# zhuduowang/Change3D

Hardware: AMD Instinct MI355X
Metric: train images/sec (256x256 pairs, X3D-L BCD) (higher is better)
Workload: dtype bf16

## Files before the change

change3d_amd/csrc/dw_bwd_fused.hip:

```cpp
#include "pw_common.h"
#include "dw_common.h"
#include "bn_fin.h"
#include "launch_hints.h"
#include "../../include/change3d_hip.h"
#include <cstdlib>
#include <type_traits>

#ifdef C3D_PW_CLOCK
constexpr int FCLK_WAVES = 16384;
__device__ unsigned long long c3d_fb_clk[FCLK_WAVES][10];
#define FCLK_DECL unsigned long long fclk_[10] = {0, 0, 0, 0, 0, 0, 0, 0, 0, 0}; unsigned long long fclk_last_ = __builtin_amdgcn_s_memtime();
#define FCLK(i) { const unsigned long long t_ = __builtin_amdgcn_s_memtime(); fclk_[i] += t_ - fclk_last_; fclk_last_ = t_; }
#define FCLK_FLUSH if ((threadIdx.x & 63) == 0) { const int w_ = (blockIdx.x * 8 + (threadIdx.x >> 6)) % FCLK_WAVES; for (int i_ = 0; i_ < 9; ++i_) c3d_fb_clk[w_][i_] += fclk_[i_]; c3d_fb_clk[w_][9] += 1ull; }
#else
#define FCLK_DECL
#define FCLK(i)
#define FCLK_FLUSH
#endif

namespace {

#ifndef C3D_FB_ROWS
#define C3D_FB_ROWS 8
#endif
constexpr int FB_TH = C3D_FB_ROWS, FB_TW = 8, FB_DH = FB_TH + 2, FB_DW = FB_TW + 2, FB_NTHR = FB_TH * FB_TW * 8;
#if C3D_FB_ROWS == 8
#define FB_KATTR __launch_bounds__(FB_NTHR)
#else
#define FB_KATTR __launch_bounds__(FB_NTHR) __attribute__((amdgpu_waves_per_eu(2, 2)))
#endif

template <typename T> struct Raw8;
template <> struct Raw8<bf16_t> {
  typedef uint4 type;
  static __device__ __forceinline__ type load(const bf16_t* p) { return *reinterpret_cast<const uint4*>(p); }
  static __device__ __forceinline__ void cvt(const type& v, float (&f)[8]) {
    f[0] = __uint_as_float(v.x << 16); f[1] = __uint_as_float(v.x & 0xffff0000u);
    f[2] = __uint_as_float(v.y << 16); f[3] = __uint_as_float(v.y & 0xffff0000u);
    f[4] = __uint_as_float(v.z << 16); f[5] = __uint_as_float(v.z & 0xffff0000u);
    f[6] = __uint_as_float(v.w << 16); f[7] = __uint_as_float(v.w & 0xffff0000u);
  }
};
template <> struct Raw8<float> {
  struct type { float4 a, b; };
  static __device__ __forceinline__ type load(const float* p) {
    type t; t.a = *reinterpret_cast<const float4*>(p); t.b = *reinterpret_cast<const float4*>(p + 4); return t;
  }
  static __device__ __forceinline__ void cvt(const type& v, float (&f)[8]) {
    f[0] = v.a.x; f[1] = v.a.y; f[2] = v.a.z; f[3] = v.a.w; f[4] = v.b.x; f[5] = v.b.y; f[6] = v.b.z; f[7] = v.b.w;
  }
};
template <typename T> struct Raw4;
template <> struct Raw4<bf16_t> {
  typedef uint2 type;
  static __device__ __forceinline__ type load(const bf16_t* p) { return *reinterpret_cast<const uint2*>(p); }
  static __device__ __forceinline__ void cvt(const type& v, float (&f)[4]) {
    f[0] = __uint_as_float(v.x << 16); f[1] = __uint_as_float(v.x & 0xffff0000u);
    f[2] = __uint_as_float(v.y << 16); f[3] = __uint_as_float(v.y & 0xffff0000u);
  }
  static __device__ __forceinline__ void store(bf16_t* p, const float (&f)[4]) {
    *reinterpret_cast<uint2*>(p) = make_uint2(pack_bf16x2(f[0], f[1]), pack_bf16x2(f[2], f[3]));
  }
};
template <> struct Raw4<float> {
  typedef float4 type;
  static __device__ __forceinline__ type load(const float* p) { return *reinterpret_cast<const float4*>(p); }
  static __device__ __forceinline__ void cvt(const type& v, float (&f)[4]) { f[0] = v.x; f[1] = v.y; f[2] = v.z; f[3] = v.w; }
  static __device__ __forceinline__ void store(float* p, const float (&f)[4]) {
    *reinterpret_cast<float4*>(p) = make_float4(f[0], f[1], f[2], f[3]);
  }
};

__device__ __forceinline__ void lds4(const float* p, float (&f)[4]) {
  const float4 a = *reinterpret_cast<const float4*>(p);
  f[0] = a.x; f[1] = a.y; f[2] = a.z; f[3] = a.w;
}

__device__ __forceinline__ void lds8(const float* p, float (&f)[8]) {
  const float4 a = *reinterpret_cast<const float4*>(p);
  const float4 b = *reinterpret_cast<const float4*>(p + 4);
  f[0] = a.x; f[1] = a.y; f[2] = a.z; f[3] = a.w; f[4] = b.x; f[5] = b.y; f[6] = b.z; f[7] = b.w;
}

template <int TT> __device__ __forceinline__ void pin_acc(f32x2_t (&a)[TT][2]);
template <> __device__ __forceinline__ void pin_acc<3>(f32x2_t (&a)[3][2]) {
  asm volatile("" : "+v"(a[0][0]), "+v"(a[0][1]), "+v"(a[1][0]), "+v"(a[1][1]), "+v"(a[2][0]), "+v"(a[2][1]) : : "memory");
}
template <> __device__ __forceinline__ void pin_acc<4>(f32x2_t (&a)[4][2]) {
  asm volatile("" : "+v"(a[0][0]), "+v"(a[0][1]), "+v"(a[1][0]), "+v"(a[1][1]), "+v"(a[2][0]), "+v"(a[2][1]), "+v"(a[3][0]),
               "+v"(a[3][1]) : : "memory");
}
template <> __device__ __forceinline__ void pin_acc<5>(f32x2_t (&a)[5][2]) {
  asm volatile("" : "+v"(a[0][0]), "+v"(a[0][1]), "+v"(a[1][0]), "+v"(a[1][1]), "+v"(a[2][0]), "+v"(a[2][1]), "+v"(a[3][0]),
               "+v"(a[3][1]), "+v"(a[4][0]), "+v"(a[4][1]) : : "memory");
}
__device__ __forceinline__ void pin_dw(f32x2_t (&a0)[2], f32x2_t (&a1)[2], f32x2_t (&a2)[2]) {
  asm volatile("" : "+v"(a0[0]), "+v"(a0[1]), "+v"(a1[0]), "+v"(a1[1]), "+v"(a2[0]), "+v"(a2[1]));
}

template <int TT, int CY, int CX>
__device__ __forceinline__ void fb_taps_s2(const float4* tp, const float* wlp, f32x2_t (&acc)[TT][2], f32x2_t (&dwa)[27][2],
                                           const f32x2_t (&ain)[TT][2]) {
#pragma unroll
  for (int ky = CY ? 0 : 1; ky < 3; ky += 2) {
#pragma unroll
    for (int kx = CX ? 0 : 1; kx < 3; kx += 2) {
      const int lyo = (CY + 1 - ky) / 2 + 1, lxo = (CX + 1 - kx) / 2 + 1;
      f32x2_t wk[3][2];
#pragma unroll
      for (int kt = 0; kt < 3; ++kt) {
        const float4 wv = *reinterpret_cast<const float4*>(wlp + (kt * 9 + ky * 3 + kx) * 32);
        wk[kt][0] = f32x2_t{wv.x, wv.y}; wk[kt][1] = f32x2_t{wv.z, wv.w};
      }
#pragma unroll
      for (int to = 0; to < TT; ++to) {
        const float4 hv = tp[((to * FB_DH + lyo) * FB_DW + lxo) * DW_CV];
        const f32x2_t v0 = {hv.x, hv.y}, v1 = {hv.z, hv.w};
#pragma unroll
        for (int kt = 0; kt < 3; ++kt) {
          const int ti = to + kt - 1;
          if (ti >= 0 && ti < TT) {
            const int k = kt * 9 + ky * 3 + kx;
            acc[ti][0] = __builtin_elementwise_fma(v0, wk[kt][0], acc[ti][0]);
            acc[ti][1] = __builtin_elementwise_fma(v1, wk[kt][1], acc[ti][1]);
            dwa[k][0] = __builtin_elementwise_fma(v0, ain[ti][0], dwa[k][0]);
            dwa[k][1] = __builtin_elementwise_fma(v1, ain[ti][1], dwa[k][1]);
          }
        }
      }
      pin_acc<TT>(acc);
      pin_dw(dwa[ky * 3 + kx], dwa[9 + ky * 3 + kx], dwa[18 + ky * 3 + kx]);
      if (CX == 0) break;
    }
    if (CY == 0) break;
  }
}

template <int TT>
__device__ __forceinline__ void fb_taps_s1(const float4* tp, const float* wlp, f32x2_t (&acc)[TT][2], f32x2_t (&dwa)[27][2],
                                           const f32x2_t (&ain)[TT][2]) {
#pragma unroll
  for (int ky = 0; ky < 3; ++ky) {
#pragma unroll
    for (int kx = 0; kx < 3; ++kx) {
      f32x2_t wk[3][2];
#pragma unroll
      for (int kt = 0; kt < 3; ++kt) {
        const float4 wv = *reinterpret_cast<const float4*>(wlp + (kt * 9 + ky * 3 + kx) * 32);
        wk[kt][0] = f32x2_t{wv.x, wv.y}; wk[kt][1] = f32x2_t{wv.z, wv.w};
      }
#pragma unroll
      for (int to = 0; to < TT; ++to) {
        const float4 hv = tp[((to * FB_DH + (2 - ky)) * FB_DW + (2 - kx)) * DW_CV];
        const f32x2_t v0 = {hv.x, hv.y}, v1 = {hv.z, hv.w};
#pragma unroll
        for (int kt = 0; kt < 3; ++kt) {
          const int ti = to + kt - 1;
          if (ti >= 0 && ti < TT) {
            const int k = kt * 9 + ky * 3 + kx;
            acc[ti][0] = __builtin_elementwise_fma(v0, wk[kt][0], acc[ti][0]);
            acc[ti][1] = __builtin_elementwise_fma(v1, wk[kt][1], acc[ti][1]);
            dwa[k][0] = __builtin_elementwise_fma(v0, ain[ti][0], dwa[k][0]);
            dwa[k][1] = __builtin_elementwise_fma(v1, ain[ti][1], dwa[k][1]);
          }
        }
      }
      pin_acc<TT>(acc);
      pin_dw(dwa[ky * 3 + kx], dwa[9 + ky * 3 + kx], dwa[18 + ky * 3 + kx]);
    }
  }
}

__device__ __forceinline__ void fb_flush(void* scratch, const float (&S1)[4], const float (&S2)[4], const f32x2_t (&dwa)[27][2],
                                         double* __restrict__ dsums, float* __restrict__ dw, const DwGeom& g, const int c0) {
  const int tid = threadIdx.x;
  const int lane = tid & 63, wave = tid >> 6;
  double* red64 = reinterpret_cast<double*>(scratch);
  __syncthreads();
  double D1[4], D2[4];
#pragma unroll
  for (int j = 0; j < 4; ++j) {
    D1[j] = (double)S1[j]; D2[j] = (double)S2[j];
#pragma unroll
    for (int o = 2 * DW_CV; o < 64; o <<= 1) {
      D1[j] += __shfl_xor(D1[j], o, 64);
      D2[j] += __shfl_xor(D2[j], o, 64);
    }
  }
  if (lane < 2 * DW_CV) {
#pragma unroll
    for (int j = 0; j < 4; ++j) {
      red64[(wave * 2 * DW_CV + lane) * 8 + j] = D1[j];
      red64[(wave * 2 * DW_CV + lane) * 8 + 4 + j] = D2[j];
    }
  }
  __syncthreads();
  if (tid < 64) {
    const int v = tid >> 4, r = tid & 15;
    const int hh = r >> 3, which = (r >> 2) & 1, j = r & 3;
    double sacc = 0.0;
    for (int wv = 0; wv < FB_NTHR / 64; ++wv) sacc += red64[(wv * 2 * DW_CV + hh * DW_CV + v) * 8 + which * 4 + j];
    const int c = c0 + v * 8 + hh * 4 + j;
    if (c < g.C) atomicAdd(dsums + (size_t)which * g.C + c, sacc);
  }
  if (dw == nullptr) return;
  constexpr int FB_DUMP_LD = FB_NTHR + 48, FB_DUMP_PT = FB_NTHR / 2 + 8;
  float* dump = reinterpret_cast<float*>(scratch);
  const int dslot = tid + (FB_DUMP_PT - FB_NTHR / 2) * (tid / (FB_NTHR / 2));
#pragma unroll
  for (int j = 0; j < 4; ++j) {
    __syncthreads();
#pragma unroll
    for (int k = 0; k < 27; ++k) dump[k * FB_DUMP_LD + dslot] = dwa[k][j >> 1][j & 1];
    __syncthreads();
    for (int t2 = tid; t2 < 27 * 8 * 2; t2 += FB_NTHR) {
      const int o = t2 >> 1, part = t2 & 1;
      const int tap = o >> 3, v = o & 3, hh = (o >> 2) & 1;
      const float* src = dump + tap * FB_DUMP_LD + part * FB_DUMP_PT + hh * DW_CV + v;
      float s = 0.f;
#pragma unroll 8
      for (int k = 0; k < FB_NTHR / 16; ++k) s += src[k * 2 * DW_CV];
      s += __shfl_xor(s, 1, 64);
      const int c = c0 + v * 8 + hh * 4 + j;
      if (part == 0 && c < g.C) atomicAdd(dw + (size_t)c * 27 + tap, s);
    }
  }
}

template <typename T, int TT, int S>
__global__ FB_KATTR void dw_bwd_fused_kernel(
    const T* __restrict__ t1, const T* __restrict__ bb, const float* __restrict__ coefA,
    const float* __restrict__ coefB, const float* __restrict__ coefC, const float* __restrict__ w,
    const T* __restrict__ a, const float* __restrict__ ss_a, const float* __restrict__ mr_a, T* __restrict__ t2,
    double* __restrict__ dsums, float* __restrict__ dw, const DwGeom g, const int tiles_per_wg, const c3d_bn_fin fin) {
  typedef Raw8<T> R8;
  typedef Raw4<T> R4;
  constexpr int NI = TT * FB_DH * FB_DW * DW_CV;
  constexpr int SL = (NI + FB_NTHR - 1) / FB_NTHR;
  extern __shared__ __attribute__((aligned(16))) unsigned char smem[];
  float* wl = reinterpret_cast<float*>(smem);
  float* cf = wl + 27 * 32;
  float4* tile = reinterpret_cast<float4*>(cf + 7 * 32);

  const int tid = threadIdx.x;
  FCLK_DECL
  const int h = (tid >> 2) & 1;
  const int cv = tid & (DW_CV - 1);
  const int pix = tid >> 3;
  const int px = pix & (FB_TW - 1), py = pix >> 3;

  const int tiles_x = (g.W + FB_TW * S - 1) / (FB_TW * S), tiles_y = (g.H + FB_TH * S - 1) / (FB_TH * S);
  const int ntiles = tiles_x * tiles_y;
  const int gx = (ntiles + tiles_per_wg - 1) / tiles_per_wg;
  const ChunkOrder co = chunk_order((g.Cp + DW_CV * 8 - 1) / (DW_CV * 8), gx * g.B);
  if (co.group < 0) return;
  const int b = co.group / gx, tg = co.group % gx;
  const int c0 = co.chunk * DW_CV * 8;
  const int cb8 = c0 + cv * 8;
  const int cb4 = cb8 + h * 4;
  const bool c_ok = cb8 < g.Cp;

  for (int i = tid; i < 27 * 32; i += FB_NTHR) {
    const int tap = i >> 5, c = c0 + (i & 31);
    wl[i] = (c < g.C) ? w[(size_t)c * 27 + tap] : 0.f;
  }
  if (fin.sums) {
    if (tid < 128) {
      float cA, cB, cC;
      c3dfin::bn_b_bwd_coef_nc(fin, g.C, g.Cp, c0 + (tid >> 2), tid & 3, co.group == 0, cA, cB, cC);
      if ((tid & 3) == 0) { cf[tid >> 2] = cA; cf[32 + (tid >> 2)] = cB; cf[64 + (tid >> 2)] = cC; }
    }
  }
  for (int i = tid + (fin.sums ? 3 * 32 : 0); i < 7 * 32; i += FB_NTHR) {
    const int k = i >> 5, c = c0 + (i & 31);
    float v = 0.f;
    if (c < g.Cp) {
      v = k == 0 ? coefA[c] : k == 1 ? coefB[(size_t)b * g.Cp + c] : k == 2 ? coefC[c] : k == 3 ? ss_a[c]
        : k == 4 ? ss_a[g.Cp + c] : k == 5 ? mr_a[c] : mr_a[g.Cp + c];
    }
    cf[i] = v;
  }

  float S1[4], S2[4];
#pragma unroll
  for (int j = 0; j < 4; ++j) { S1[j] = 0.f; S2[j] = 0.f; }
  f32x2_t dwa[27][2];
#pragma unroll
  for (int k = 0; k < 27; ++k) { dwa[k][0] = f32x2_t{0.f, 0.f}; dwa[k][1] = f32x2_t{0.f, 0.f}; }

  typename R8::type r1[SL], r2[SL];
  typename R4::type ar[TT];
  unsigned vmask = 0;
  int rel[SL], yx[SL];
#pragma unroll
  for (int sl = 0; sl < SL; ++sl) {
    const int i_ = tid + sl * FB_NTHR;
    const int p_ = i_ / DW_CV;
    const int ix_ = p_ % FB_DW, q_ = p_ / FB_DW;
    const int iy_ = q_ % FB_DH, t_ = q_ / FB_DH;
    const bool use_ = i_ < NI && c_ok && t_ < g.T;
    rel[sl] = ((t_ * g.Ho + iy_) * g.Wo + ix_) * g.Cp + cb8;
    yx[sl] = use_ ? (iy_ | (ix_ << 16)) : 0x7fff7fff;
  }
  const int orel = (S * py * g.W + S * px) * g.Cp + cb4, ofr = g.H * g.W * g.Cp;
#define FB_ISSUE_RAW(TL)                                                                          \
  {                                                                                               \
    const int tx_ = (TL) % tiles_x, ty_ = (TL) / tiles_x;                                         \
    const int dy0_ = ty_ * FB_TH - 1, dx0_ = tx_ * FB_TW - 1;                                     \
    const int64_t tb_ = ((((int64_t)b * g.T) * g.Ho + dy0_) * g.Wo + dx0_) * g.Cp;   \
    const T* t1b_ = t1 + tb_;                                                                     \
    const T* bbb_ = bb + tb_;                                                                     \
    vmask = 0;                                                                                    \
    _Pragma("unroll") for (int sl = 0; sl < SL; ++sl) {                                           \
      const unsigned gy_ = (unsigned)(dy0_ + (yx[sl] & 0xffff));                                  \
      const unsigned gx_ = (unsigned)(dx0_ + (yx[sl] >> 16));                                     \
      if (gy_ < (unsigned)g.Ho && gx_ < (unsigned)g.Wo) {                                         \
        r1[sl] = R8::load(t1b_ + rel[sl]);                                                        \
        r2[sl] = R8::load(bbb_ + rel[sl]);                                                        \
        vmask |= 1u << sl;                                                                        \
      }                                                                                           \
    }                                                                                             \
  }
#define FB_ISSUE_A(TL, CY, CX)                                                                    \
  {                                                                                               \
    const int tx_ = (TL) % tiles_x, ty_ = (TL) / tiles_x;                                         \
    if (c_ok && ty_ * FB_TH * S + S * py + (CY) < g.H && tx_ * FB_TW * S + S * px + (CX) < g.W) { \
      const T* ab_ = a + ((((int64_t)b * g.T) * g.H + ty_ * FB_TH * S + (CY)) * g.W + tx_ * FB_TW * S + (CX)) * g.Cp; \
      _Pragma("unroll") for (int t = 0; t < TT; ++t)                                              \
        if (t < g.T) ar[t] = R4::load(ab_ + (orel + t * ofr));                                    \
    }                                                                                             \
  }
#define FB_ISSUE(TL) { FB_ISSUE_RAW(TL) FB_ISSUE_A(TL, 0, 0) }

  const int tl0 = tg * tiles_per_wg;
  int tl1 = tl0 + tiles_per_wg;
  if (tl1 > ntiles) tl1 = ntiles;
  if (tl0 < tl1) FB_ISSUE(tl0)
  __syncthreads();
  FCLK(0)

  for (int tl = tl0; tl < tl1; ++tl) {
    const int tx = tl % tiles_x, ty = tl / tiles_x;
    const int y0 = ty * FB_TH * S, x0 = tx * FB_TW * S;
    float4* tb = tile + (size_t)((tl - tl0) & 1) * 2 * NI;
    {
      float cA[8], cB[8], cC[8];
      lds8(cf + 0 * 32 + cv * 8, cA);
      lds8(cf + 1 * 32 + cv * 8, cB);
      lds8(cf + 2 * 32 + cv * 8, cC);
#pragma unroll
      for (int sl = 0; sl < SL; ++sl) {
        const int i = tid + sl * FB_NTHR;
        if (i < NI) {
          float f[8];
          if ((vmask >> sl) & 1u) {
            float f2[8];
            R8::cvt(r1[sl], f);
            R8::cvt(r2[sl], f2);
#pragma unroll
            for (int j = 0; j < 8; ++j) f[j] = fmaf(cA[j], f[j], fmaf(cC[j], f2[j], cB[j]));
          } else {
#pragma unroll
            for (int j = 0; j < 8; ++j) f[j] = 0.f;
          }
          tb[i] = make_float4(f[0], f[1], f[2], f[3]);
          tb[NI + i] = make_float4(f[4], f[5], f[6], f[7]);
        }
      }
    }
    FCLK(1)
    typename R4::type arc[TT];
    f32x2_t ain[TT][2];
    f32x2_t acc[TT][2];
    bool p_ok;
    float sa[4], sb[4];
    lds4(cf + 3 * 32 + cv * 8 + h * 4, sa);
    lds4(cf + 4 * 32 + cv * 8 + h * 4, sb);
#define FB_PRE(CY, CX)                                                                                            \
  {                                                                                                               \
    p_ok = c_ok && y0 + S * py + (CY) < g.H && x0 + S * px + (CX) < g.W;                                          \
    _Pragma("unroll") for (int t = 0; t < TT; ++t) {                                                             \
      if (p_ok && t < g.T) {                                                                                      \
        arc[t] = ar[t];                                                                                           \
        float av[4];                                                                                              \
        R4::cvt(arc[t], av);                                                                                      \
        ain[t][0] = f32x2_t{fmaxf(fmaf(av[0], sa[0], sb[0]), 0.f), fmaxf(fmaf(av[1], sa[1], sb[1]), 0.f)};        \
        ain[t][1] = f32x2_t{fmaxf(fmaf(av[2], sa[2], sb[2]), 0.f), fmaxf(fmaf(av[3], sa[3], sb[3]), 0.f)};        \
      } else {                                                                                                    \
        ain[t][0] = f32x2_t{0.f, 0.f}; ain[t][1] = f32x2_t{0.f, 0.f};                                             \
      }                                                                                                           \
      acc[t][0] = f32x2_t{0.f, 0.f}; acc[t][1] = f32x2_t{0.f, 0.f};                                               \
    }                                                                                                             \
  }
#define FB_EPI(CY, CX)                                                                                            \
  if (p_ok) {                                                                                                     \
    float ma[4], ra[4];                                                                                           \
    lds4(cf + 5 * 32 + cv * 8 + h * 4, ma);                                                                       \
    lds4(cf + 6 * 32 + cv * 8 + h * 4, ra);                                                                       \
    T* ob = t2 + ((((int64_t)b * g.T) * g.H + y0 + (CY)) * g.W + x0 + (CX)) * g.Cp;                               \
    _Pragma("unroll") for (int t = 0; t < TT; ++t) {                                                             \
      if (t < g.T) {                                                                                              \
        float av[4], o[4];                                                                                        \
        R4::cvt(arc[t], av);                                                                                      \
        _Pragma("unroll") for (int j = 0; j < 4; ++j) {                                                          \
          const float d = round_as<T>(ain[t][j >> 1][j & 1] > 0.f ? acc[t][j >> 1][j & 1] : 0.f);                 \
          o[j] = d;                                                                                               \
          S1[j] += d; S2[j] += d * ((av[j] - ma[j]) * ra[j]);                                                     \
        }                                                                                                         \
        R4::store(ob + (orel + t * ofr), o);                                                                      \
      }                                                                                                           \
    }                                                                                                             \
  }
    FB_PRE(0, 0)
    if constexpr (S == 2) {
      FB_ISSUE_A(tl, 1, 0)
      if (tl + 1 < tl1) FB_ISSUE_RAW(tl + 1)
      FCLK(2)
      __syncthreads();
      FCLK(3)
      const float4* tp = tb + (size_t)h * NI + (py * FB_DW + px) * DW_CV + cv;
      const float* wlp = wl + cv * 8 + h * 4;
      fb_taps_s2<TT, 0, 0>(tp, wlp, acc, dwa, ain);
      FCLK(4)
      FB_EPI(0, 0)
      FCLK(5)
      FB_PRE(1, 0)
      FB_ISSUE_A(tl, 0, 1)
      FCLK(2)
      fb_taps_s2<TT, 1, 0>(tp, wlp, acc, dwa, ain);
      FCLK(4)
      FB_EPI(1, 0)
      FCLK(5)
      FB_PRE(0, 1)
      FB_ISSUE_A(tl, 1, 1)
      FCLK(2)
      fb_taps_s2<TT, 0, 1>(tp, wlp, acc, dwa, ain);
      FCLK(4)
      FB_EPI(0, 1)
      FCLK(5)
      FB_PRE(1, 1)
      if (tl + 1 < tl1) FB_ISSUE_A(tl + 1, 0, 0)
      FCLK(2)
      fb_taps_s2<TT, 1, 1>(tp, wlp, acc, dwa, ain);
      FCLK(4)
      FB_EPI(1, 1)
      FCLK(5)
      continue;
    }
    if (tl + 1 < tl1) FB_ISSUE(tl + 1)
    FCLK(2)
    __syncthreads();
    FCLK(3)

    const float4* tp = tb + (size_t)h * NI + (py * FB_DW + px) * DW_CV + cv;
    float4 wq[2][3], hq[2][TT];
#define FB_LOAD(S, SLOT)                                                                                          \
  {                                                                                                               \
    constexpr int ky_ = (S) / 3, kx_ = (S) % 3;                                                                   \
    _Pragma("unroll") for (int kt = 0; kt < 3; ++kt)                                                             \
      wq[SLOT][kt] = *reinterpret_cast<const float4*>(wl + (kt * 9 + (S)) * 32 + cv * 8 + h * 4);                \
    _Pragma("unroll") for (int to = 0; to < TT; ++to)                                                            \
      hq[SLOT][to] = tp[((to * FB_DH + (2 - ky_)) * FB_DW + (2 - kx_)) * DW_CV];                                 \
  }
#define FB_STEP(S, SLOT)                                                                                          \
  {                                                                                                               \
    _Pragma("unroll") for (int to = 0; to < TT; ++to) {                                                          \
      const f32x2_t v0 = {hq[SLOT][to].x, hq[SLOT][to].y}, v1 = {hq[SLOT][to].z, hq[SLOT][to].w};                 \
      _Pragma("unroll") for (int kt = 0; kt < 3; ++kt) {                                                         \
        const int ti = to + kt - 1;                               \
        if (ti >= 0 && ti < TT) {                                                                                 \
          const f32x2_t w0 = {wq[SLOT][kt].x, wq[SLOT][kt].y}, w1 = {wq[SLOT][kt].z, wq[SLOT][kt].w};             \
          acc[ti][0] = __builtin_elementwise_fma(v0, w0, acc[ti][0]);                                             \
          acc[ti][1] = __builtin_elementwise_fma(v1, w1, acc[ti][1]);                                             \
          dwa[kt * 9 + (S)][0] = __builtin_elementwise_fma(v0, ain[ti][0], dwa[kt * 9 + (S)][0]);                 \
          dwa[kt * 9 + (S)][1] = __builtin_elementwise_fma(v1, ain[ti][1], dwa[kt * 9 + (S)][1]);                 \
        }                                                                                                         \
      }                                                                                                           \
    }                                                                                                             \
                                                          \
    pin_acc<TT>(acc);                                                                                             \
    pin_dw(dwa[(S)], dwa[9 + (S)], dwa[18 + (S)]);                                                                \
  }
    if constexpr (TT <= 3) {
      FB_LOAD(0, 0)
      FB_LOAD(1, 1) FB_STEP(0, 0)
      FB_LOAD(2, 0) FB_STEP(1, 1)
      FB_LOAD(3, 1) FB_STEP(2, 0)
      FB_LOAD(4, 0) FB_STEP(3, 1)
      FB_LOAD(5, 1) FB_STEP(4, 0)
      FB_LOAD(6, 0) FB_STEP(5, 1)
      FB_LOAD(7, 1) FB_STEP(6, 0)
      FB_LOAD(8, 0) FB_STEP(7, 1)
      FB_STEP(8, 0)
    } else {
      fb_taps_s1<TT>(tp, wl + cv * 8 + h * 4, acc, dwa, ain);
    }
#undef FB_LOAD
#undef FB_STEP
    FCLK(4)
    FB_EPI(0, 0)
    FCLK(5)
  }
#undef FB_PRE
#undef FB_EPI
#undef FB_ISSUE
#undef FB_ISSUE_RAW
#undef FB_ISSUE_A

  fb_flush(tile, S1, S2, dwa, dsums, dw, g, c0);
  FCLK(7)
  FCLK_FLUSH
}

__device__ __forceinline__ void fb_glds16(const void* gsrc, const uint32_t lds_dst) {
  unsigned keep;
  asm volatile("s_mov_b32 %0, m0\n\ts_mov_b32 m0, %2\n\ts_nop 0\n\tglobal_load_lds_dwordx4 %1, off\n\ts_mov_b32 m0, %0"
               : "=&s"(keep) : "v"(gsrc), "s"(lds_dst) : "memory");
}
__device__ __forceinline__ void fb_wait_vm(const int n) {
  switch (n) {
    case 0: asm volatile("s_waitcnt vmcnt(0)" ::: "memory"); break;
    case 1: asm volatile("s_waitcnt vmcnt(1)" ::: "memory"); break;
    case 2: asm volatile("s_waitcnt vmcnt(2)" ::: "memory"); break;
    case 3: asm volatile("s_waitcnt vmcnt(3)" ::: "memory"); break;
    case 4: asm volatile("s_waitcnt vmcnt(4)" ::: "memory"); break;
    case 5: asm volatile("s_waitcnt vmcnt(5)" ::: "memory"); break;
    case 6: asm volatile("s_waitcnt vmcnt(6)" ::: "memory"); break;
    case 7: asm volatile("s_waitcnt vmcnt(7)" ::: "memory"); break;
    case 8: asm volatile("s_waitcnt vmcnt(8)" ::: "memory"); break;
    case 9: asm volatile("s_waitcnt vmcnt(9)" ::: "memory"); break;
    case 10: asm volatile("s_waitcnt vmcnt(10)" ::: "memory"); break;
    case 11: asm volatile("s_waitcnt vmcnt(11)" ::: "memory"); break;
    case 12: asm volatile("s_waitcnt vmcnt(12)" ::: "memory"); break;
    default: asm volatile("s_waitcnt vmcnt(0)" ::: "memory"); break;
  }
}
typedef __attribute__((address_space(3))) unsigned char* fb_lds_ptr_t;

template <int TT>
struct RingPlan {
  static constexpr int NI = TT * FB_DH * FB_DW * DW_CV;
  static constexpr int NP = (NI + 63) / 64;
  static constexpr int NPL = NP * 64;
  static constexpr int SL = (NP + 7) / 8;
  static constexpr bool A_LDS = TT <= 4;
  static constexpr int NA = A_LDS ? (TT * 8 * DW_CV + 63) / 64 : 0;
  static constexpr int A_WAVE_BYTES = TT * 8 * DW_CV * 16;
  static constexpr int A_BYTES = A_LDS ? 8 * A_WAVE_BYTES : 0;
  static constexpr int SLOT_BYTES = 2 * NPL * 16 + A_BYTES;
  static constexpr int R = TT <= 3 ? 3 : 2;
  static constexpr int AHEAD = R - 1;
  static constexpr int HEAD_BYTES = (27 * 32 + 7 * 32) * 4;
  static constexpr int LDS_BYTES = HEAD_BYTES + R * SLOT_BYTES;
};

template <int TT, bool SPREAD>
__global__ __launch_bounds__(FB_NTHR) void dw_bwd_ring_kernel(
    const bf16_t* __restrict__ t1, const bf16_t* __restrict__ bb, const float* __restrict__ coefA,
    const float* __restrict__ coefB, const float* __restrict__ coefC, const float* __restrict__ w,
    const bf16_t* __restrict__ a, const float* __restrict__ ss_a, const float* __restrict__ mr_a, bf16_t* __restrict__ t2,
    double* __restrict__ dsums, float* __restrict__ dw, const DwGeom g, const int tiles_per_wg, const c3d_bn_fin fin) {
  typedef bf16_t T;
  typedef Raw4<T> R4;
  typedef RingPlan<TT> P;
  constexpr int NI = P::NI, NP = P::NP, NPL = P::NPL, SL = P::SL, NA = P::NA, AHEAD = P::AHEAD;
  constexpr bool A_LDS = P::A_LDS;
  extern __shared__ __attribute__((aligned(16))) unsigned char smem[];
  float* wl = reinterpret_cast<float*>(smem);
  float* cf = wl + 27 * 32;
  unsigned char* ring = smem + P::HEAD_BYTES;
  const uint32_t ring_lds = (uint32_t)(uintptr_t)(fb_lds_ptr_t)ring;

  const int tid = threadIdx.x;
  FCLK_DECL
  const int lane = tid & 63;
  const int wave = __builtin_amdgcn_readfirstlane(tid >> 6);
  const int h = (tid >> 2) & 1;
  const int cv = tid & (DW_CV - 1);
  const int pix = tid >> 3;
  const int px = pix & (FB_TW - 1), py = pix >> 3;

  const int tiles_x = (g.W + FB_TW - 1) / FB_TW, tiles_y = (g.H + FB_TH - 1) / FB_TH;
  const int ntiles = tiles_x * tiles_y;
  const int gx = (ntiles + tiles_per_wg - 1) / tiles_per_wg;
  const ChunkOrder co = chunk_order((g.Cp + DW_CV * 8 - 1) / (DW_CV * 8), gx * g.B);
  if (co.group < 0) return;
  const int b = co.group / gx, tg = co.group % gx;
  const int c0 = co.chunk * DW_CV * 8;
  const int cb8 = c0 + cv * 8;
  const int cb4 = cb8 + h * 4;
  const bool c_ok = cb8 < g.Cp;

  for (int i = tid; i < 27 * 32; i += FB_NTHR) {
    const int tap = i >> 5, c = c0 + (i & 31);
    wl[i] = (c < g.C) ? w[(size_t)c * 27 + tap] : 0.f;
  }
  if (fin.sums) {
    if (tid < 128) {
      float cA, cB, cC;
      c3dfin::bn_b_bwd_coef_nc(fin, g.C, g.Cp, c0 + (tid >> 2), tid & 3, co.group == 0, cA, cB, cC);
      if ((tid & 3) == 0) { cf[tid >> 2] = cA; cf[32 + (tid >> 2)] = cB; cf[64 + (tid >> 2)] = cC; }
    }
  }
  for (int i = tid + (fin.sums ? 3 * 32 : 0); i < 7 * 32; i += FB_NTHR) {
    const int k = i >> 5, c = c0 + (i & 31);
    float v = 0.f;
    if (c < g.Cp) {
      v = k == 0 ? coefA[c] : k == 1 ? coefB[(size_t)b * g.Cp + c] : k == 2 ? coefC[c] : k == 3 ? ss_a[c]
        : k == 4 ? ss_a[g.Cp + c] : k == 5 ? mr_a[c] : mr_a[g.Cp + c];
    }
    cf[i] = v;
  }

  float S1[4], S2[4];
#pragma unroll
  for (int j = 0; j < 4; ++j) { S1[j] = 0.f; S2[j] = 0.f; }
  f32x2_t dwa[27][2];
#pragma unroll
  for (int k = 0; k < 27; ++k) { dwa[k][0] = f32x2_t{0.f, 0.f}; dwa[k][1] = f32x2_t{0.f, 0.f}; }

  int rel[SL], yx[SL];
#pragma unroll
  for (int sl = 0; sl < SL; ++sl) {
    const int i_ = tid + sl * FB_NTHR;
    const int p_ = i_ / DW_CV;
    const int ix_ = p_ % FB_DW, q_ = p_ / FB_DW;
    const int iy_ = q_ % FB_DH, t_ = q_ / FB_DH;
    const bool use_ = i_ < NI && c_ok && t_ < g.T;
    rel[sl] = ((t_ * g.Ho + iy_) * g.Wo + ix_) * g.Cp + cb8;
    yx[sl] = use_ ? (iy_ | (ix_ << 16)) : 0x7fff7fff;
  }
  const int rel_safe = (g.Wo + 1) * g.Cp + c0;
  int arel[NA > 0 ? NA : 1];
  unsigned aok = 0;
  int apx[NA > 0 ? NA : 1];
#pragma unroll
  for (int j = 0; j < NA; ++j) {
    const int idx = j * 64 + lane;
    const int vec = idx & (DW_CV - 1), combo = idx >> 2;
    const int p_ = combo & 7, t_ = combo >> 3;
    arel[j] = ((t_ * g.H + wave) * g.W + p_) * g.Cp + c0 + vec * 8;
    apx[j] = p_;
    if (t_ < TT && t_ < g.T && c0 + vec * 8 < g.Cp) aok |= 1u << j;
  }
  typename R4::type ar[A_LDS ? 1 : TT];
  const int orel = (py * g.W + px) * g.Cp + cb4, ofr = g.H * g.W * g.Cp;
  const int n_raw = (NP - 1 - wave) / 8 + 1;
  const int n_dma = 2 * n_raw + NA;

  int64_t ri_tb = 0, ri_ab = 0;
  uint32_t ri_sb = 0;
  int ri_dy0 = 0, ri_dx0 = 0;
  bool ri_row_ok = false, ri_on = false;
#define RB_BASES(TL, SIDX)                                                                        \
  {                                                                                               \
    const int tx_ = (TL) % tiles_x, ty_ = (TL) / tiles_x;                                         \
    ri_dy0 = ty_ * FB_TH - 1; ri_dx0 = tx_ * FB_TW - 1;                                           \
    ri_tb = ((((int64_t)b * g.T) * g.Ho + ri_dy0) * g.Wo + ri_dx0) * g.Cp;      \
    ri_sb = ring_lds + (uint32_t)(SIDX) * P::SLOT_BYTES;                                          \
    ri_ab = ((((int64_t)b * g.T) * g.H + ty_ * FB_TH) * g.W + tx_ * FB_TW) * g.Cp;                \
    ri_row_ok = ty_ * FB_TH + wave < g.H;                                                         \
  }
#define RB_ISSUE_Q(Q)                                                                             \
  if (ri_on) {                                                                                    \
    if constexpr ((Q) < 2 * SL) {                                                                 \
      constexpr int sl_ = (Q) >> 1;                                                               \
      if (wave + 8 * sl_ < NP) {                                                                  \
        const unsigned gy_ = (unsigned)(ri_dy0 + (yx[sl_] & 0xffff));                             \
        const unsigned gx_ = (unsigned)(ri_dx0 + (yx[sl_] >> 16));                                \
        const int off_ = (gy_ < (unsigned)g.Ho && gx_ < (unsigned)g.Wo) ? rel[sl_] : rel_safe;    \
        fb_glds16((((Q) & 1) ? bb : t1) + ri_tb + off_,                                           \
                  ri_sb + (uint32_t)(((Q) & 1) * NPL * 16) + (uint32_t)(wave + 8 * sl_) * 1024u); \
      }                                                                                           \
    } else if constexpr ((Q) < 2 * SL + NA) {                                                     \
      constexpr int j_ = (Q) - 2 * SL;                                                            \
      if (j_ * 64 + lane < TT * 8 * DW_CV) {                                                      \
        const int ax0_ = ri_dx0 + 1;                                                              \
        const int off_ = (ri_row_ok && ((aok >> j_) & 1u) && ax0_ + apx[j_] < g.W) ? arel[j_] : c0; \
        fb_glds16(a + ri_ab + off_, ri_sb + (uint32_t)(2 * NPL * 16) + (uint32_t)wave * (uint32_t)P::A_WAVE_BYTES + (uint32_t)j_ * 1024u); \
      }                                                                                           \
    }                                                                                             \
  }
#define RB_ISSUE_ALL                                                                              \
  { RB_ISSUE_Q(0) RB_ISSUE_Q(1) RB_ISSUE_Q(2) RB_ISSUE_Q(3) RB_ISSUE_Q(4) RB_ISSUE_Q(5) RB_ISSUE_Q(6) RB_ISSUE_Q(7) RB_ISSUE_Q(8) RB_ISSUE_Q(9) }
  static_assert(2 * SL + NA <= 10, "RB_ISSUE_ALL covers ten request indices");
#define RB_ISSUE_A(TL)                                                                            \
  if constexpr (!A_LDS) {                                                                         \
    const int tx_ = (TL) % tiles_x, ty_ = (TL) / tiles_x;                                         \
    if (c_ok && ty_ * FB_TH + py < g.H && tx_ * FB_TW + px < g.W) {                               \
      const T* ab_ = a + ((((int64_t)b * g.T) * g.H + ty_ * FB_TH) * g.W + tx_ * FB_TW) * g.Cp;   \
      _Pragma("unroll") for (int t = 0; t < TT; ++t)                                              \
        if (t < g.T) ar[t] = R4::load(ab_ + (orel + t * ofr));                                    \
    }                                                                                             \
  }
#define RB_CONVERT(TL, SIDX)                                                                      \
  {                                                                                               \
    const int tx_ = (TL) % tiles_x, ty_ = (TL) / tiles_x;                                         \
    const int dy0_ = ty_ * FB_TH - 1, dx0_ = tx_ * FB_TW - 1;                                     \
    uint4* p0_ = reinterpret_cast<uint4*>(ring + (size_t)(SIDX) * P::SLOT_BYTES);                 \
    float cA[8], cB[8], cC[8];                                                                    \
    lds8(cf + 0 * 32 + cv * 8, cA);                                                               \
    lds8(cf + 1 * 32 + cv * 8, cB);                                                               \
    lds8(cf + 2 * 32 + cv * 8, cC);                                                               \
    _Pragma("unroll") for (int sl = 0; sl < SL; ++sl) {                                           \
      if (wave + 8 * sl < NP) {                                                                   \
        const int i = tid + sl * FB_NTHR;                                                         \
        const unsigned gy_ = (unsigned)(dy0_ + (yx[sl] & 0xffff));                                \
        const unsigned gx_ = (unsigned)(dx0_ + (yx[sl] >> 16));                                   \
        float f[8];                                                                               \
        if (gy_ < (unsigned)g.Ho && gx_ < (unsigned)g.Wo) {                                       \
          float f2[8];                                                                            \
          Raw8<T>::cvt(p0_[i], f);                                                                \
          Raw8<T>::cvt(p0_[NPL + i], f2);                                                         \
          _Pragma("unroll") for (int j = 0; j < 8; ++j) f[j] = fmaf(cA[j], f[j], fmaf(cC[j], f2[j], cB[j])); \
        } else {                                                                                  \
          _Pragma("unroll") for (int j = 0; j < 8; ++j) f[j] = 0.f;                               \
        }                                                                                         \
        reinterpret_cast<float4*>(p0_)[i] = make_float4(f[0], f[1], f[2], f[3]);                  \
        reinterpret_cast<float4*>(p0_)[NPL + i] = make_float4(f[4], f[5], f[6], f[7]);            \
      }                                                                                           \
    }                                                                                             \
  }

  const int tl0 = tg * tiles_per_wg;
  int tl1 = tl0 + tiles_per_wg;
  if (tl1 > ntiles) tl1 = ntiles;
  ri_on = true;
#pragma unroll
  for (int d = 0; d < AHEAD; ++d)
    if (tl0 + d < tl1) { RB_BASES(tl0 + d, d) RB_ISSUE_ALL }
  if (tl0 < tl1) RB_ISSUE_A(tl0)
  __syncthreads();
  if (tl0 < tl1) {
    const int younger = tl1 - tl0 - 1 < AHEAD - 1 ? tl1 - tl0 - 1 : AHEAD - 1;
    fb_wait_vm(A_LDS ? younger * n_dma : 0);
    RB_CONVERT(tl0, 0)
  }
  FCLK(0)

  int slot = 0;
  for (int tl = tl0; tl < tl1; ++tl) {
    const int tx = tl % tiles_x, ty = tl / tiles_x;
    const int y0 = ty * FB_TH, x0 = tx * FB_TW;
    const int slot1 = slot + 1 == P::R ? 0 : slot + 1;
    const int slotn = slot + AHEAD >= P::R ? slot + AHEAD - P::R : slot + AHEAD;
    const float4* tb = reinterpret_cast<const float4*>(ring + (size_t)slot * P::SLOT_BYTES);
    typename R4::type arc[TT];
    f32x2_t ain[TT][2];
    f32x2_t acc[TT][2];
    float sa[4], sb[4];
    const bool p_ok = c_ok && y0 + py < g.H && x0 + px < g.W;
    if constexpr (A_LDS) {
      const uint2* ab = reinterpret_cast<const uint2*>(ring + (size_t)slot * P::SLOT_BYTES + 2 * NPL * 16 + wave * P::A_WAVE_BYTES) + (px * DW_CV + cv) * 2 + h;
#pragma unroll
      for (int t = 0; t < TT; ++t) arc[t] = ab[t * 8 * DW_CV * 2];
    } else {
#pragma unroll
      for (int t = 0; t < TT; ++t) arc[t] = ar[t];
    }
    lds4(cf + 3 * 32 + cv * 8 + h * 4, sa);
    lds4(cf + 4 * 32 + cv * 8 + h * 4, sb);
    __syncthreads();
    FCLK(3)
    ri_on = tl + AHEAD < tl1;
    if (ri_on) RB_BASES(tl + AHEAD, slotn)
    if constexpr (!SPREAD) RB_ISSUE_ALL
    if (tl + 1 < tl1) RB_ISSUE_A(tl + 1)
    FCLK(2)
#pragma unroll
    for (int t = 0; t < TT; ++t) {
      if (p_ok && t < g.T) {
        float av[4];
        R4::cvt(arc[t], av);
        ain[t][0] = f32x2_t{fmaxf(fmaf(av[0], sa[0], sb[0]), 0.f), fmaxf(fmaf(av[1], sa[1], sb[1]), 0.f)};
        ain[t][1] = f32x2_t{fmaxf(fmaf(av[2], sa[2], sb[2]), 0.f), fmaxf(fmaf(av[3], sa[3], sb[3]), 0.f)};
      } else {
        ain[t][0] = f32x2_t{0.f, 0.f}; ain[t][1] = f32x2_t{0.f, 0.f};
      }
      acc[t][0] = f32x2_t{0.f, 0.f}; acc[t][1] = f32x2_t{0.f, 0.f};
    }
    FCLK(1)
    const float4* tp = tb + (size_t)h * NPL + (py * FB_DW + px) * DW_CV + cv;
    if constexpr (TT <= 3) {
      float4 wq[2][3], hq[2][TT];
#define FB_LOAD(S, SLOT)                                                                                          \
  {                                                                                                               \
    constexpr int ky_ = (S) / 3, kx_ = (S) % 3;                                                                   \
    _Pragma("unroll") for (int kt = 0; kt < 3; ++kt)                                                             \
      wq[SLOT][kt] = *reinterpret_cast<const float4*>(wl + (kt * 9 + (S)) * 32 + cv * 8 + h * 4);                \
    _Pragma("unroll") for (int to = 0; to < TT; ++to)                                                            \
      hq[SLOT][to] = tp[((to * FB_DH + (2 - ky_)) * FB_DW + (2 - kx_)) * DW_CV];                                 \
  }
#define FB_STEP(S, SLOT)                                                                                          \
  {                                                                                                               \
    _Pragma("unroll") for (int to = 0; to < TT; ++to) {                                                          \
      const f32x2_t v0 = {hq[SLOT][to].x, hq[SLOT][to].y}, v1 = {hq[SLOT][to].z, hq[SLOT][to].w};                 \
      _Pragma("unroll") for (int kt = 0; kt < 3; ++kt) {                                                         \
        const int ti = to + kt - 1;                                                                               \
        if (ti >= 0 && ti < TT) {                                                                                 \
          const f32x2_t w0 = {wq[SLOT][kt].x, wq[SLOT][kt].y}, w1 = {wq[SLOT][kt].z, wq[SLOT][kt].w};             \
          acc[ti][0] = __builtin_elementwise_fma(v0, w0, acc[ti][0]);                                             \
          acc[ti][1] = __builtin_elementwise_fma(v1, w1, acc[ti][1]);                                             \
          dwa[kt * 9 + (S)][0] = __builtin_elementwise_fma(v0, ain[ti][0], dwa[kt * 9 + (S)][0]);                 \
          dwa[kt * 9 + (S)][1] = __builtin_elementwise_fma(v1, ain[ti][1], dwa[kt * 9 + (S)][1]);                 \
        }                                                                                                         \
      }                                                                                                           \
    }                                                                                                             \
    pin_acc<TT>(acc);                                                                                             \
    pin_dw(dwa[(S)], dwa[9 + (S)], dwa[18 + (S)]);                                                                \
    if constexpr (SPREAD) { RB_ISSUE_Q(S) if constexpr ((S) == 8) { RB_ISSUE_Q(9) } }                             \
  }
      FB_LOAD(0, 0)
      FB_LOAD(1, 1) FB_STEP(0, 0)
      FB_LOAD(2, 0) FB_STEP(1, 1)
      FB_LOAD(3, 1) FB_STEP(2, 0)
      FB_LOAD(4, 0) FB_STEP(3, 1)
      FB_LOAD(5, 1) FB_STEP(4, 0)
      FB_LOAD(6, 0) FB_STEP(5, 1)
      FB_LOAD(7, 1) FB_STEP(6, 0)
      FB_LOAD(8, 0) FB_STEP(7, 1)
      FB_STEP(8, 0)
#undef FB_LOAD
#undef FB_STEP
    } else {
      fb_taps_s1<TT>(tp, wl + cv * 8 + h * 4, acc, dwa, ain);
      if constexpr (SPREAD) RB_ISSUE_ALL
    }
    FCLK(4)
    if (tl + 1 < tl1) {
      const int younger = tl1 - tl - 2 < AHEAD - 1 ? tl1 - tl - 2 : AHEAD - 1;
      fb_wait_vm(A_LDS ? younger * n_dma : 0);
    }
    FCLK(6)
    if (p_ok) {
      float ma[4], ra[4];
      lds4(cf + 5 * 32 + cv * 8 + h * 4, ma);
      lds4(cf + 6 * 32 + cv * 8 + h * 4, ra);
      T* ob = t2 + ((((int64_t)b * g.T) * g.H + y0) * g.W + x0) * g.Cp;
#pragma unroll
      for (int t = 0; t < TT; ++t) {
        if (t < g.T) {
          float av[4], o[4];
          R4::cvt(arc[t], av);
#pragma unroll
          for (int j = 0; j < 4; ++j) {
            const float d = round_as<T>(ain[t][j >> 1][j & 1] > 0.f ? acc[t][j >> 1][j & 1] : 0.f);
            o[j] = d;
            S1[j] += d; S2[j] += d * ((av[j] - ma[j]) * ra[j]);
          }
          R4::store(ob + (orel + t * ofr), o);
        }
      }
    }
    FCLK(5)
    if (tl + 1 < tl1) RB_CONVERT(tl + 1, slot1)
    FCLK(8)
    slot = slot1;
  }
#undef RB_BASES
#undef RB_ISSUE_Q
#undef RB_ISSUE_ALL
#undef RB_ISSUE_A
#undef RB_CONVERT

  fb_flush(ring, S1, S2, dwa, dsums, dw, g, c0);
  FCLK(7)
  FCLK_FLUSH
}

template <int TT, bool SPREAD>
int launch_ring_t(const void* t1, const void* bb, const float* cA, const float* cB, const float* cC, const float* w,
                  const void* a, const float* ss_a, const float* mr_a, void* t2, double* dsums, float* dw,
                  const DwGeom& g, hipStream_t stream, const c3d_bn_fin& fin) {
  typedef RingPlan<TT> P;
  static_assert(P::LDS_BYTES <= 160 * 1024, "ring does not fit");
  static_assert((size_t)P::R * P::SLOT_BYTES >= (size_t)27 * (FB_NTHR + 48) * sizeof(float), "dump region");
  static_assert((P::AHEAD - 1) * (2 * P::SL + P::NA) <= 12, "fb_wait_vm covers counts up to 12");
  static bool attr_set = false;
  if (!attr_set) {
    hipError_t e = hipFuncSetAttribute(reinterpret_cast<const void*>(&dw_bwd_ring_kernel<TT, SPREAD>),
                                       hipFuncAttributeMaxDynamicSharedMemorySize, 160 * 1024);
    if (e != hipSuccess) return (int)e;
    attr_set = true;
  }
  const int ntiles = ((g.W + FB_TW - 1) / FB_TW) * ((g.H + FB_TH - 1) / FB_TH);
  const int chunks = (g.Cp + DW_CV * 8 - 1) / (DW_CV * 8);
  static const int env_tpw = c3d_env("C3D_DWBF_TPW") ? atoi(c3d_env("C3D_DWBF_TPW")) : 0;
  static const int env_max = c3d_env("C3D_DWBF_MAX") ? atoi(c3d_env("C3D_DWBF_MAX")) : 64;
  int tpw = env_max;
  while (tpw > 4 && (long)((ntiles + tpw - 1) / tpw) * chunks * g.B < 85L * device_cus() / 100) tpw >>= 1;
  if (env_tpw > 0) tpw = env_tpw;
  if (tpw > ntiles) tpw = ntiles;
  dim3 grid(chunk_order_grid(chunks, (long)((ntiles + tpw - 1) / tpw) * g.B));
  dw_bwd_ring_kernel<TT, SPREAD><<<grid, dim3(FB_NTHR), P::LDS_BYTES, stream>>>(
      reinterpret_cast<const bf16_t*>(t1), reinterpret_cast<const bf16_t*>(bb), cA, cB, cC, w, reinterpret_cast<const bf16_t*>(a),
      ss_a, mr_a, reinterpret_cast<bf16_t*>(t2), dsums, dw, g, tpw, fin);
  C3D_CHECK_LAUNCH();
  return 0;
}

template <typename T, int TT, int S>
int launch_fused_t(const void* t1, const void* bb, const float* cA, const float* cB, const float* cC, const float* w,
                   const void* a, const float* ss_a, const float* mr_a, void* t2, double* dsums, float* dw,
                   const DwGeom& g, hipStream_t stream, const c3d_bn_fin& fin) {
  constexpr int NI = TT * FB_DH * FB_DW * DW_CV;
  const size_t lds = (27 * 32 + 7 * 32) * sizeof(float) + (size_t)2 * 2 * NI * sizeof(float4);
  static_assert((size_t)2 * 2 * NI * sizeof(float4) >= (size_t)27 * (FB_NTHR + 48) * sizeof(float), "dump region");
  if (lds > 160 * 1024) return C3D_E_UNSUPPORTED;
  static bool attr_set = false;
  if (!attr_set) {
    hipError_t e = hipFuncSetAttribute(reinterpret_cast<const void*>(&dw_bwd_fused_kernel<T, TT, S>),
                                       hipFuncAttributeMaxDynamicSharedMemorySize, 160 * 1024);
    if (e != hipSuccess) return (int)e;
    attr_set = true;
  }
  const int ntiles = ((g.W + FB_TW * S - 1) / (FB_TW * S)) * ((g.H + FB_TH * S - 1) / (FB_TH * S));
  const int chunks = (g.Cp + DW_CV * 8 - 1) / (DW_CV * 8);
  static const int env_tpw = c3d_env("C3D_DWBF_TPW") ? atoi(c3d_env("C3D_DWBF_TPW")) : 0;
  static const int env_max = c3d_env("C3D_DWBF_MAX") ? atoi(c3d_env("C3D_DWBF_MAX")) : 64;
  int tpw = env_max / (S * S) * (8 / FB_TH);
  constexpr int WGC = 512 / FB_NTHR;
  while (tpw > 4 && (long)((ntiles + tpw - 1) / tpw) * chunks * g.B < 85L * WGC * device_cus() / 100) tpw >>= 1;
  if (env_tpw > 0) tpw = env_tpw;
  if (tpw > ntiles) tpw = ntiles;
  dim3 grid(chunk_order_grid(chunks, (long)((ntiles + tpw - 1) / tpw) * g.B));
  dw_bwd_fused_kernel<T, TT, S><<<grid, dim3(FB_NTHR), lds, stream>>>(
      reinterpret_cast<const T*>(t1), reinterpret_cast<const T*>(bb), cA, cB, cC, w, reinterpret_cast<const T*>(a),
      ss_a, mr_a, reinterpret_cast<T*>(t2), dsums, dw, g, tpw, fin);
  C3D_CHECK_LAUNCH();
  return 0;
}

}

namespace {
int dispatch_fused(const void* t1, const void* b, const float* coefA, const float* coefB, const float* coefC, const float* w,
                   const void* a, const float* ss_a, const float* mr_a, void* t2, double* dsums, float* dw, const DwGeom& g,
                   int dtype, hipStream_t s, const c3d_bn_fin& fin) {
  const int tt = dw_frames(g.T);
#define FB_DISPATCH(TY, S_)                                                                                         \
  return tt == 3 ? launch_fused_t<TY, 3, S_>(t1, b, coefA, coefB, coefC, w, a, ss_a, mr_a, t2, dsums, dw, g, s, fin)   \
       : tt == 4 ? launch_fused_t<TY, 4, S_>(t1, b, coefA, coefB, coefC, w, a, ss_a, mr_a, t2, dsums, dw, g, s, fin)   \
                 : launch_fused_t<TY, 5, S_>(t1, b, coefA, coefB, coefC, w, a, ss_a, mr_a, t2, dsums, dw, g, s, fin);
  if (dtype == C3D_DT_F32) {
    if (g.stride == 1) { FB_DISPATCH(float, 1) }
    FB_DISPATCH(float, 2)
  }
  if (dtype == C3D_DT_BF16) {
    if (C3D_FB_ROWS == 8 && g.stride == 1 && (c3d_option_dw_ring & 1) && ((c3d_option_dw_ring & 8) || g.T > 3 || (long)g.H * g.W >= 64 * 64)) {
      if (tt == 3) {
        if (c3d_option_dw_ring & 4) return launch_ring_t<3, true>(t1, b, coefA, coefB, coefC, w, a, ss_a, mr_a, t2, dsums, dw, g, s, fin);
        return launch_ring_t<3, false>(t1, b, coefA, coefB, coefC, w, a, ss_a, mr_a, t2, dsums, dw, g, s, fin);
      }
      if (tt == 4) {
        if (c3d_option_dw_ring & 4) return launch_ring_t<4, true>(t1, b, coefA, coefB, coefC, w, a, ss_a, mr_a, t2, dsums, dw, g, s, fin);
        return launch_ring_t<4, false>(t1, b, coefA, coefB, coefC, w, a, ss_a, mr_a, t2, dsums, dw, g, s, fin);
      }
      if (c3d_option_dw_ring & 4) return launch_ring_t<5, true>(t1, b, coefA, coefB, coefC, w, a, ss_a, mr_a, t2, dsums, dw, g, s, fin);
      return launch_ring_t<5, false>(t1, b, coefA, coefB, coefC, w, a, ss_a, mr_a, t2, dsums, dw, g, s, fin);
    }
    if (g.stride == 1) { FB_DISPATCH(bf16_t, 1) }
    FB_DISPATCH(bf16_t, 2)
  }
#undef FB_DISPATCH
  return C3D_E_BADARG;
}
}

extern "C" int c3d_dw333_bwd_fused(const void* t1, const void* b, const float* coefA, const float* coefB,
                                   const float* coefC, const float* w, const void* a, const float* ss_a,
                                   const float* mr_a, void* t2, double* dsums, float* dw, int32_t B, int32_t T,
                                   int32_t H, int32_t W, int32_t C, int32_t Cp, int32_t stride, int32_t dtype, void* stream) {
  if (stride != 1 && stride != 2) return C3D_E_UNSUPPORTED;
  DwGeom g{B, T, H, W, (H - 1) / stride + 1, (W - 1) / stride + 1, C, Cp, stride};
  if (!t1 || !b || !coefA || !coefB || !coefC || !w || !a || !ss_a || !mr_a || !t2 || !dsums || !dw || !geom_ok(g))
    return C3D_E_BADARG;
  return dispatch_fused(t1, b, coefA, coefB, coefC, w, a, ss_a, mr_a, t2, dsums, dw, g, dtype,
                        reinterpret_cast<hipStream_t>(stream), c3d_bn_fin{});
}

extern "C" int c3d_dw333_bwd_fused_fin(const void* t1, const void* b, const c3d_bn_fin* fin_b, const float* w, const void* a,
                                       const float* ss_a, const float* mr_a, void* t2, double* dsums, float* dw, int32_t B,
                                       int32_t T, int32_t H, int32_t W, int32_t C, int32_t Cp, int32_t stride, int32_t dtype,
                                       void* stream) {
  if (stride != 1 && stride != 2) return C3D_E_UNSUPPORTED;
  DwGeom g{B, T, H, W, (H - 1) / stride + 1, (W - 1) / stride + 1, C, Cp, stride};
  if (!t1 || !b || !w || !a || !ss_a || !mr_a || !t2 || !dsums || !dw || !geom_ok(g)) return C3D_E_BADARG;
  if (!fin_b || !fin_b->sums || fin_b->batch != B || !fin_b->gamma || !fin_b->mr || !(fin_b->count > 0)) return C3D_E_BADARG;
  return dispatch_fused(t1, b, nullptr, nullptr, nullptr, w, a, ss_a, mr_a, t2, dsums, dw, g, dtype,
                        reinterpret_cast<hipStream_t>(stream), *fin_b);
}

#ifdef C3D_PW_CLOCK
extern "C" int c3d_debug_fb_clock(unsigned long long* out, int reset) {
  hipError_t e = hipMemcpyFromSymbol(out, HIP_SYMBOL(c3d_fb_clk), sizeof(unsigned long long) * FCLK_WAVES * 10);
  if (e != hipSuccess) return (int)e;
  if (reset) {
    void* p = nullptr;
    e = hipGetSymbolAddress(&p, HIP_SYMBOL(c3d_fb_clk));
    if (e == hipSuccess) e = hipMemset(p, 0, sizeof(unsigned long long) * FCLK_WAVES * 10);
  }
  return (int)e;
}
#endif
```

change3d_amd/csrc/launch_hints.h:

```cpp
#pragma once
#include <cstdint>
#include <hip/hip_runtime.h>
#include "../../include/change3d_hip.h"

extern thread_local int c3d_side_launch;

extern int c3d_option_stem_mfma;
extern int c3d_option_convt_mfma;
extern int c3d_option_dw_ring;
extern int c3d_option_dw_fwd_hv;
extern int c3d_option_dw_t4;
extern int c3d_option_pw_cfwd;
extern int c3d_option_pw_cdg;
int c3d_detail_pw_cdg_a(const c3d_pw_args* args, void* stream);
bool c3d_detail_pw_cdg_a_supported(int Kp, int Np, int64_t M);
int c3d_detail_pw_cdg_c(const c3d_pw_args* args, void* stream);
bool c3d_detail_pw_cdg_c_supported(int Kp, int Np, int64_t M, int64_t rows_per_sample);
extern thread_local int c3d_cdg_defer_reduce, c3d_cdg_parts;
int c3d_detail_pw_wgrad_reduce(const float* ws, float* dw, int N, int K, int parts, int sn, int sk, hipStream_t stream);
extern int c3d_option_pw_wgrad_v2;
void c3d_detail_pw_wgrad_v2_drop();
```

change3d_amd/csrc/pw_cdgrad.hip:

```cpp
#include "common.h"
#include "../../include/change3d_hip.h"
#include "pw_common.h"
#include "launch_hints.h"
#include "bn_fin.h"
#include <cstdlib>
#include <cstring>

thread_local int c3d_cdg_defer_reduce = 0, c3d_cdg_parts = 0;

#ifdef C3D_CD_CLOCK
__device__ unsigned long long c3d_cd_clk[1024][8];
#define CDCLK(i) { if (threadIdx.x == 0) c3d_cd_clk[blockIdx.x & 1023][i] = __builtin_amdgcn_s_memtime(); }
extern "C" int c3d_debug_cd_clock(unsigned long long* out) {
  return (int)hipMemcpyFromSymbol(out, HIP_SYMBOL(c3d_cd_clk), sizeof(c3d_cd_clk));
}
#else
#define CDCLK(i)
#endif

namespace {

constexpr int CD_THREADS = 512;
constexpr uint32_t CD_OOB = 0x80000000u;
constexpr int CD_MAX_PARTS = 512;

struct CdPlan {
  int MT, WR, WC;
  int QG;
  int tiles_per_wg;
  int KL, QL;
  int img_rows;
  int w_off, a_off, a_bytes, q_off, q_bytes;
  int os_off, os_wave;
  int par_off, dump_off;
};

typedef uint32_t cd_u32x4_t __attribute__((ext_vector_type(4)));
typedef __attribute__((address_space(3))) void* cd_lds_ptr_t;
typedef const __attribute__((address_space(1))) void* cd_glb_ptr_t;
typedef short cd_s16x4_t __attribute__((ext_vector_type(4)));
typedef __attribute__((address_space(3))) cd_s16x4_t* cd_lds_s16x4_ptr_t;

__device__ __forceinline__ __amdgpu_buffer_rsrc_t cd_rsrc(const void* p, uint32_t bytes) {
  return __builtin_amdgcn_make_buffer_rsrc(const_cast<void*>(p), 0, p ? (int)bytes : 0, 0x00020000);
}
__device__ __forceinline__ uint4 cd_load(__amdgpu_buffer_rsrc_t r, uint32_t off) {
  const cd_u32x4_t v = __builtin_amdgcn_raw_buffer_load_b128(r, off, 0, 0);
  return make_uint4(v[0], v[1], v[2], v[3]);
}
__device__ __forceinline__ void cd_cvt(const uint4& v, float (&f)[8]) {
  f[0] = __uint_as_float(v.x << 16); f[1] = __uint_as_float(v.x & 0xffff0000u);
  f[2] = __uint_as_float(v.y << 16); f[3] = __uint_as_float(v.y & 0xffff0000u);
  f[4] = __uint_as_float(v.z << 16); f[5] = __uint_as_float(v.z & 0xffff0000u);
  f[6] = __uint_as_float(v.w << 16); f[7] = __uint_as_float(v.w & 0xffff0000u);
}
__device__ __forceinline__ void cd_ld8(const float* p, float (&f)[8]) {
  const float4 a = *reinterpret_cast<const float4*>(p);
  const float4 b = *reinterpret_cast<const float4*>(p + 4);
  f[0] = a.x; f[1] = a.y; f[2] = a.z; f[3] = a.w; f[4] = b.x; f[5] = b.y; f[6] = b.z; f[7] = b.w;
}

template <int KS, int NTW, int NPW, int NQW, int RP, int RQ, int K2>
__global__ __launch_bounds__(CD_THREADS) void pw_cdg_a_kernel(const c3d_pw_args a, const CdPlan L) {
  extern __shared__ __attribute__((aligned(16))) unsigned char smem[];
  const int tid = threadIdx.x, lane = tid & 63;
  const int wave = __builtin_amdgcn_readfirstlane(tid >> 6);
  const int Kp = a.Kp, Np = a.Np, Gq = Kp >> 3, Gn = Np >> 3, MT = L.MT, KL = L.KL, QL = L.QL;
  bf16_t* const Ws = reinterpret_cast<bf16_t*>(smem + L.w_off);
  float* const Pp = reinterpret_cast<float*>(smem + L.par_off);
  float* const Ep = Pp + 3 * Kp;
  bf16_t* const dump = reinterpret_cast<bf16_t*>(smem + L.dump_off) + tid * 8;

  const int M32 = (int)a.M;
  const int tiles = (M32 + MT - 1) / MT;
  int t0 = (int)blockIdx.x * L.tiles_per_wg;
  if (t0 > tiles) t0 = tiles;
  int t1 = t0 + L.tiles_per_wg;
  if (t1 > tiles) t1 = tiles;
  const uint32_t row_hi = (uint32_t)(t1 * MT < M32 ? t1 * MT : M32);
  const __amdgpu_buffer_rsrc_t rX = cd_rsrc(a.x, row_hi * (uint32_t)Kp * 2u);
  const __amdgpu_buffer_rsrc_t rX2 = cd_rsrc(a.x2, row_hi * (uint32_t)Kp * 2u);
  const __amdgpu_buffer_rsrc_t rQ = cd_rsrc(a.wg_x3, row_hi * (uint32_t)Np * 2u);
  const __amdgpu_buffer_rsrc_t rE1 = cd_rsrc(a.e1, (uint32_t)M32 * (uint32_t)Np * 2u);
  const __amdgpu_buffer_rsrc_t rC1 = cd_rsrc(a.add_sums ? a.add_c : nullptr, (uint32_t)M32 * (uint32_t)Np * 2u);
  const __amdgpu_buffer_rsrc_t rY = cd_rsrc(a.y, (uint32_t)M32 * (uint32_t)Np * 2u);

  int p_desc[RP], q_desc[RQ];
  uint32_t p_go[RP], q_go[RQ];
  {
    const float invG = 1.0f / (float)Gq, invN = 1.0f / (float)Gn;
#pragma unroll
    for (int r = 0; r < RP; ++r) {
      const int i = tid + CD_THREADS * r;
      const int row = __float2int_rz(((float)i + 0.5f) * invG);
      const bool ok = i < MT * Gq;
      p_desc[r] = ok ? (row << 5) | (i - row * Gq) : 0;
      p_go[r] = ok ? (uint32_t)i * 16u : CD_OOB;
    }
#pragma unroll
    for (int r = 0; r < RQ; ++r) {
      const int i = tid + CD_THREADS * r;
      const int row = __float2int_rz(((float)i + 0.5f) * invN);
      const bool ok = i < MT * Gn;
      q_desc[r] = ok ? (row << 5) | (i - row * Gn) : 0;
      q_go[r] = ok ? (uint32_t)i * 16u : CD_OOB;
    }
  }
  const bool p_last = (wave * 64 + CD_THREADS * (RP - 1)) < MT * Gq;
  const bool q_last = (wave * 64 + CD_THREADS * (RQ - 1)) < MT * Gn;
  uint4 rawp[RP], rawp2[RP], rawq[RQ];
  const uint32_t tbp = (uint32_t)(MT * Kp * 2), tbq = (uint32_t)(MT * Np * 2);
  {
    const uint32_t bp = (uint32_t)t0 * tbp, bq = (uint32_t)t0 * tbq;
#pragma unroll
    for (int r = 0; r < RP; ++r) { rawp[r] = cd_load(rX, p_go[r] + bp); rawp2[r] = cd_load(rX2, p_go[r] + bp); }
#pragma unroll
    for (int r = 0; r < RQ; ++r) rawq[r] = cd_load(rQ, q_go[r] + bq);
  }

  const int wr = wave % L.WR, wc = wave / L.WR;
  const int nt0 = wc * NTW;
  constexpr int NLW = NTW * 16 + 8;
  bf16_t* const Os = reinterpret_cast<bf16_t*>(smem + L.os_off + wave * L.os_wave);
  constexpr int GOW = NTW * 2, RPO = 64 / GOW, NPASS = (16 + RPO - 1) / RPO;
  const int rr_o = lane / GOW, v_o = lane - rr_o * GOW;
  const int cvec = nt0 * 2 + v_o;
  const bool act_o = lane < GOW * RPO && cvec * 8 < Np;
  uint4 e1r[NPASS], c1r[NPASS];
#define CD_EOFF(TILE, P) ((act_o && (P) * RPO + rr_o < 16 && (TILE) * MT + wr * 16 + (P) * RPO + rr_o < M32)                        \
                              ? ((uint32_t)((TILE) * MT + wr * 16 + (P) * RPO + rr_o) * (uint32_t)Np + (uint32_t)cvec * 8u) * 2u : CD_OOB)
#pragma unroll
  for (int p = 0; p < NPASS; ++p) { const uint32_t o = t0 < t1 ? CD_EOFF(t0, p) : CD_OOB; e1r[p] = cd_load(rE1, o); c1r[p] = cd_load(rC1, o); }

  {
    const int wbytes = (KS * 4) * L.img_rows * 16;
    const int nchunk = (wbytes + 1023) >> 10;
    const unsigned char* src = reinterpret_cast<const unsigned char*>(a.w_img);
    const int rot = (int)blockIdx.x % nchunk;
    for (int c = wave; c < nchunk; c += 8) {
      int r = c + rot;
      if (r >= nchunk) r -= nchunk;
      const int off = r * 1024 + lane * 16;
      if (off < wbytes)
        __builtin_amdgcn_global_load_lds((cd_glb_ptr_t)(src + off), (cd_lds_ptr_t)(smem + L.w_off + r * 1024), 16, 0, 0);
    }
  }
  for (int i = tid * 16; i < 2 * L.a_bytes; i += CD_THREADS * 16) *reinterpret_cast<uint4*>(smem + L.a_off + i) = make_uint4(0u, 0u, 0u, 0u);
  for (int i = tid * 16; i < 2 * L.q_bytes; i += CD_THREADS * 16) *reinterpret_cast<uint4*>(smem + L.q_off + i) = make_uint4(0u, 0u, 0u, 0u);

  if (a.fin.sums) {
    for (int c = tid; c < Kp; c += CD_THREADS) {
      float cA, cB, cC;
      c3dfin::bn_bwd_coef_consume(a.fin, a.K, Kp, c, blockIdx.x == 0, cA, cB, cC);
      Pp[c] = cA; Pp[Kp + c] = cB; Pp[2 * Kp + c] = cC;
    }
  } else {
    for (int i = tid; i < 3 * Kp; i += CD_THREADS) Pp[i] = a.pro_p[i];
  }
  for (int i = tid; i < 2 * Np; i += CD_THREADS) Ep[i] = a.add_sums ? a.add_mr[i] : 0.f;
  asm volatile("s_waitcnt vmcnt(0)" ::: "memory");
  __syncthreads();

  float s0[8], s1[8];
#pragma unroll
  for (int j = 0; j < 8; ++j) { s0[j] = 0.f; s1[j] = 0.f; }
  const uint32_t mask_on = a.wg_mask_out ? 0xffffffffu : 0u;
  const uint32_t sums_on = a.add_sums ? 0xffffffffu : 0u;
  const bf16_t* const wfrag = Ws + ((size_t)(lane >> 4) * L.img_rows + nt0 * 16 + (lane & 15)) * 8;
  const int xfrag = (wr * 16 + (lane & 15)) * KL + (lane >> 4) * 8;

  const int qg = wave % L.QG, pg = wave / L.QG;
  const int g4 = lane >> 4, li = lane & 15;
  const int pl = (4 * g4 + (li >> 2)) * KL + 4 * (li & 3) + pg * NPW * 16;
  const int ql = (4 * g4 + (li >> 2)) * QL + 4 * (li & 3) + qg * NQW * 16;
  f32x4_t dacc[NPW][NQW];
#pragma unroll
  for (int i = 0; i < NPW; ++i)
#pragma unroll
    for (int j = 0; j < NQW; ++j) dacc[i][j] = f32x4_t{0.f, 0.f, 0.f, 0.f};

#define CD_CONVERT(TILE, CP, CQ)                                                                                    \
  {                                                                                                                 \
    const int rowg0_ = (TILE) * MT;                                                                                 \
    const uint32_t bpn_ = (uint32_t)((TILE) + 1) * tbp, bqn_ = (uint32_t)((TILE) + 1) * tbq;                        \
    _Pragma("unroll") for (int r = 0; r < RP; ++r) {                                                                \
      if (r == RP - 1 && !p_last) continue;                                                                         \
      const int row = p_desc[r] >> 5, v = p_desc[r] & 31;                                                           \
      bf16_t* dst = p_go[r] != CD_OOB ? (CP) + row * KL + v * 8 : dump;                                             \
      float f[8], f2[8], cA[8], cB[8], cC[8];                                                                       \
      cd_cvt(rawp[r], f); cd_cvt(rawp2[r], f2);                                                                     \
      cd_ld8(Pp + v * 8, cA); cd_ld8(Pp + Kp + v * 8, cB); cd_ld8(Pp + 2 * Kp + v * 8, cC);                         \
       \
      const uint32_t keep = rowg0_ + row < M32 ? 0xffffffffu : 0u;                                                  \
      _Pragma("unroll") for (int e = 0; e < 8; ++e)                                                                 \
        f[e] = __uint_as_float(__float_as_uint(fmaf(cA[e], f[e], fmaf(cC[e], f2[e], cB[e]))) & keep);               \
      Vec8<bf16_t>::store(dst, f);                                                                                  \
      rawp[r] = cd_load(rX, p_go[r] + bpn_);          \
      rawp2[r] = cd_load(rX2, p_go[r] + bpn_);                                                                      \
    }                                                                                                               \
    _Pragma("unroll") for (int r = 0; r < RQ; ++r) {                                                                \
      if (r == RQ - 1 && !q_last) continue;                                                                         \
      const int row = q_desc[r] >> 5, v = q_desc[r] & 31;                                                           \
      bf16_t* dst = q_go[r] != CD_OOB ? (CQ) + row * QL + v * 8 : dump;                                             \
      *reinterpret_cast<uint4*>(dst) = rawq[r];                                                                     \
      rawq[r] = cd_load(rQ, q_go[r] + bqn_);                                                                        \
    }                                                                                                               \
  }
#define CD_MULT(CA)                                                                                                 \
  {                                                                                                                 \
    _Pragma("unroll") for (int ks = 0; ks < KS; ++ks) {                                                             \
      const uint4 xb = *reinterpret_cast<const uint4*>((CA) + xfrag + ks * 32);                                     \
      _Pragma("unroll") for (int t = 0; t < NTW; ++t) {                                                             \
        const uint4 wa = *reinterpret_cast<const uint4*>(wfrag + ((size_t)ks * 4 * L.img_rows + t * 16) * 8);       \
        acc[t] = __builtin_amdgcn_mfma_f32_16x16x32_bf16(__builtin_bit_cast(bf16x8_t, wa), __builtin_bit_cast(bf16x8_t, xb), acc[t], 0, 0, 0); \
      }                                                                                                             \
    }                                                                                                               \
  }
#define CD_WGRAD(CA, CQ)                                                                                            \
  {                                                                                                                 \
    _Pragma("unroll") for (int k2 = 0; k2 < K2; ++k2) {                                                             \
      uint4 pa[NPW], qb[NQW];                                                                                       \
      const bf16_t* pb_ = (CA) + k2 * 32 * KL + pl;                                                                 \
      const bf16_t* qb_ = (CQ) + k2 * 32 * QL + ql;                                                                 \
      _Pragma("unroll") for (int i = 0; i < NPW; ++i) {                                                             \
        const cd_s16x4_t lo_ = __builtin_amdgcn_ds_read_tr16_b64_v4i16((cd_lds_s16x4_ptr_t)(pb_ + i * 16));        \
        const cd_s16x4_t hi_ = __builtin_amdgcn_ds_read_tr16_b64_v4i16((cd_lds_s16x4_ptr_t)(pb_ + 16 * KL + i * 16)); \
        pa[i] = __builtin_bit_cast(uint4, __builtin_shufflevector(lo_, hi_, 0, 1, 2, 3, 4, 5, 6, 7));               \
      }                                                                                                             \
      _Pragma("unroll") for (int j = 0; j < NQW; ++j) {                                                             \
        const cd_s16x4_t lo_ = __builtin_amdgcn_ds_read_tr16_b64_v4i16((cd_lds_s16x4_ptr_t)(qb_ + j * 16));        \
        const cd_s16x4_t hi_ = __builtin_amdgcn_ds_read_tr16_b64_v4i16((cd_lds_s16x4_ptr_t)(qb_ + 16 * QL + j * 16)); \
        qb[j] = __builtin_bit_cast(uint4, __builtin_shufflevector(lo_, hi_, 0, 1, 2, 3, 4, 5, 6, 7));               \
      }                                                                                                             \
      _Pragma("unroll") for (int i = 0; i < NPW; ++i)                                                               \
        _Pragma("unroll") for (int j = 0; j < NQW; ++j)                                                             \
          dacc[i][j] = __builtin_amdgcn_mfma_f32_16x16x32_bf16(__builtin_bit_cast(bf16x8_t, pa[i]), __builtin_bit_cast(bf16x8_t, qb[j]), \
                                                               dacc[i][j], 0, 0, 0);                               \
    }                                                                                                               \
  }
#define CD_EPI(TILE, CQ, NEXT_ON)                                                                                   \
  {                                                                                                                 \
    _Pragma("unroll") for (int t = 0; t < NTW; ++t)                                                                 \
      *reinterpret_cast<uint2*>(Os + (lane & 15) * NLW + t * 16 + (lane >> 4) * 4) =                                \
          make_uint2(pack_bf16x2(acc[t][0], acc[t][1]), pack_bf16x2(acc[t][2], acc[t][3]));                         \
    const int row0_ = (TILE) * MT + wr * 16;                                                                        \
    _Pragma("unroll") for (int p = 0; p < NPASS; ++p) {                                                             \
      const int row = p * RPO + rr_o;                                                                               \
      const int rowc = row < 16 ? row : 0;                                                                          \
      const int m = row0_ + row;                                                                                    \
      const bool ok = act_o && row < 16 && m < M32;                                                                 \
      const uint32_t keep = ok ? 0xffffffffu : 0u;                                                                  \
      const uint4 rawo = *reinterpret_cast<const uint4*>(Os + rowc * NLW + v_o * 8);                                \
      const uint4 x3 = *reinterpret_cast<const uint4*>((CQ) + (wr * 16 + rowc) * QL + (act_o ? cvec : 0) * 8);      \
      float f[8], rv[8], cv[8], eM[8], eR[8];                                                                       \
      cd_cvt(rawo, f); cd_cvt(e1r[p], rv); cd_cvt(c1r[p], cv);                                                      \
      cd_ld8(Ep + (act_o ? cvec : 0) * 8, eM); cd_ld8(Ep + Np + (act_o ? cvec : 0) * 8, eR);                        \
      const uint32_t xw[4] = {x3.x, x3.y, x3.z, x3.w};                                                              \
      _Pragma("unroll") for (int j = 0; j < 8; ++j) {                                                               \
        const uint32_t hx = (xw[j >> 1] >> ((j & 1) * 16)) & 0xffffu;                                               \
              \
        const uint32_t pass = ((hx & 0x7fffu) != 0u && !(hx & 0x8000u)) ? 0xffffffffu : ~mask_on;                   \
        const float d = __uint_as_float(__float_as_uint(f[j] + rv[j]) & pass);                                      \
        f[j] = d;                                                                                                   \
        const float gq = __uint_as_float(__float_as_uint(round_as<bf16_t>(d)) & keep & sums_on);                    \
        s0[j] += gq; s1[j] = fmaf(gq, (cv[j] - eM[j]) * eR[j], s1[j]);                                              \
      }                                                                                                             \
      const uint4 pk = make_uint4(pack_bf16x2(f[0], f[1]), pack_bf16x2(f[2], f[3]), pack_bf16x2(f[4], f[5]), pack_bf16x2(f[6], f[7])); \
      __builtin_amdgcn_raw_buffer_store_b128(cd_u32x4_t{pk.x, pk.y, pk.z, pk.w}, rY,                                \
                                             ok ? ((uint32_t)m * (uint32_t)Np + (uint32_t)cvec * 8u) * 2u : CD_OOB, 0, 0); \
      const uint32_t no_ = (NEXT_ON) ? CD_EOFF((TILE) + 1, p) : CD_OOB;                                             \
      e1r[p] = cd_load(rE1, no_); c1r[p] = cd_load(rC1, no_);                                                       \
    }                                                                                                               \
  }

  bf16_t* const bufP0 = reinterpret_cast<bf16_t*>(smem + L.a_off);
  bf16_t* const bufP1 = reinterpret_cast<bf16_t*>(smem + L.a_off + L.a_bytes);
  bf16_t* const bufQ0 = reinterpret_cast<bf16_t*>(smem + L.q_off);
  bf16_t* const bufQ1 = reinterpret_cast<bf16_t*>(smem + L.q_off + L.q_bytes);
  if (t0 < t1) CD_CONVERT(t0, bufP0, bufQ0)
  int cur = 0;
  for (int tile = t0; tile < t1; ++tile, cur ^= 1) {
    bf16_t* const curP = cur ? bufP1 : bufP0;
    bf16_t* const nxtP = cur ? bufP0 : bufP1;
    bf16_t* const curQ = cur ? bufQ1 : bufQ0;
    bf16_t* const nxtQ = cur ? bufQ0 : bufQ1;
    __syncthreads();
    f32x4_t acc[NTW];
#pragma unroll
    for (int t = 0; t < NTW; ++t) acc[t] = f32x4_t{0.f, 0.f, 0.f, 0.f};
    if (tile + 1 < t1) {
      CD_MULT(curP)
      CD_WGRAD(curP, curQ)
      CD_CONVERT(tile + 1, nxtP, nxtQ)
      CD_EPI(tile, curQ, true)
#ifndef CD_VPM
#define CD_VPM 10
#endif
#ifndef CD_SCHED
#define CD_SCHED 0
#endif
#pragma unroll
      for (int i = 0; i < (CD_SCHED ? NTW * KS + K2 * NPW * NQW : 0); ++i) {
        __builtin_amdgcn_sched_group_barrier(0x008, 1, 0);
        __builtin_amdgcn_sched_group_barrier(0x002, CD_VPM, 0);
        if (i & 1) __builtin_amdgcn_sched_group_barrier(0x020, 1, 0);
      }
    } else {
      CD_MULT(curP)
      CD_WGRAD(curP, curQ)
      CD_EPI(tile, curQ, false)
    }
  }
#undef CD_CONVERT
#undef CD_MULT
#undef CD_WGRAD
#undef CD_EPI
#undef CD_EOFF

  {
    float* wsb = a.wg_ws + (size_t)blockIdx.x * a.K * a.N;
#pragma unroll
    for (int i = 0; i < NPW; ++i) {
#pragma unroll
      for (int j = 0; j < NQW; ++j) {
        const int n = (qg * NQW + j) * 16 + (lane & 15);
#pragma unroll
        for (int r = 0; r < 4; ++r) {
          const int k = (pg * NPW + i) * 16 + (lane >> 4) * 4 + r;
          if (k < a.K && n < a.N) wsb[(size_t)k * a.N + n] = dacc[i][j][r];
        }
      }
    }
  }

  if (a.add_sums) {
    __syncthreads();
    float* mine = reinterpret_cast<float*>(smem + L.a_off) + (size_t)wave * 16 * 64;
#pragma unroll
    for (int j = 0; j < 8; ++j) { mine[j * 64 + lane] = s0[j]; mine[(8 + j) * 64 + lane] = s1[j]; }
    __syncthreads();
    for (int i = tid; i < 2 * a.N; i += CD_THREADS) {
      const int which = i / a.N, c = i - which * a.N;
      const int cv = c >> 3, j = c & 7;
      const int wcg = cv / GOW, vo = cv - wcg * GOW;
      float accv = 0.f;
      for (int w_ = 0; w_ < L.WR; ++w_) {
        const float* base = reinterpret_cast<const float*>(smem + L.a_off) + (size_t)(wcg * L.WR + w_) * 16 * 64 + (which * 8 + j) * 64;
        for (int rr = 0; rr < RPO; ++rr) accv += base[rr * GOW + vo];
      }
      atomicAdd(a.add_sums + which * a.N + c, (double)accv);
    }
  }
}

template <int KS, int NTW, int NPW, int NQW, int RP, int RQ, int K2>
int cd_launch(const c3d_pw_args& a, const CdPlan& L, dim3 grid, size_t lds, hipStream_t s) {
  static bool attr_set = false;
  if (!attr_set) {
    hipError_t e = hipFuncSetAttribute(reinterpret_cast<const void*>(&pw_cdg_a_kernel<KS, NTW, NPW, NQW, RP, RQ, K2>),
                                       hipFuncAttributeMaxDynamicSharedMemorySize, 160 * 1024);
    if (e != hipSuccess) return (int)e;
    attr_set = true;
  }
  pw_cdg_a_kernel<KS, NTW, NPW, NQW, RP, RQ, K2><<<grid, dim3(CD_THREADS), lds, s>>>(a, L);
  return 0;
}

int cd_variant(int Kp, int Np) {
  const int KS = (Kp + 31) / 32, ntn = (Np + 15) >> 4, ntp = (Kp + 15) >> 4;
  if (KS == 7 && ntn >= 5 && ntn <= 6 && ntp <= 16) return 1;
  if (KS == 4 && ntn == 3 && ntp <= 8) return 2;
  if (KS == 2 && ntn == 2 && ntp <= 4) return 3;
  return 0;
}

int cd_plan(const c3d_pw_args& a, CdPlan& L, int64_t& blocks, size_t& lds) {
  const int var = cd_variant(a.Kp, a.Np);
  if (!var) return 0;
  const int Kpad = (a.Kp + 31) / 32 * 32, KS = Kpad / 32, ntn = (a.Np + 15) >> 4;
  L.img_rows = (ntn <= 2 ? 2 : ntn <= 4 ? 4 : ntn <= 7 ? 7 : 14) * 16;
  int NTW;
  if (var == 1) { L.WR = 2; L.WC = 4; NTW = 2; L.QG = 2; }
  else if (var == 2) { L.WR = 8; L.WC = 1; NTW = 3; L.QG = 1; }
  else { L.WR = 8; L.WC = 1; NTW = 2; L.QG = 2; }
  L.MT = 16 * L.WR;
  L.KL = Kpad + 8;
  L.QL = ntn * 16 + 8;
  const int64_t tiles = (a.M + L.MT - 1) / L.MT;
  blocks = device_cus();
  if (blocks > (tiles + 1) / 2) blocks = (tiles + 1) / 2;
  if (blocks > CD_MAX_PARTS) blocks = CD_MAX_PARTS;
  if (blocks < 1) blocks = 1;
  const int tpw = (int)((tiles + blocks - 1) / blocks);
  blocks = (tiles + tpw - 1) / tpw;
  L.tiles_per_wg = tpw;
  auto al = [](size_t v) { return (v + 1023) / 1024 * 1024; };
  size_t off = 0;
  L.w_off = 0; off += al((size_t)KS * 4 * L.img_rows * 16);
  L.a_off = (int)off; L.a_bytes = (int)al((size_t)L.MT * L.KL * 2); off += 2 * (size_t)L.a_bytes;
  L.q_off = (int)off; L.q_bytes = (int)al((size_t)L.MT * L.QL * 2); off += 2 * (size_t)L.q_bytes;
  if (2 * (size_t)L.a_bytes + 2 * (size_t)L.q_bytes < (size_t)8 * 16 * 64 * 4) return 0;
  L.os_wave = 16 * (NTW * 16 + 8) * 2; L.os_off = (int)off; off += al((size_t)8 * L.os_wave);
  L.par_off = (int)off; off += al(((size_t)3 * a.Kp + 2 * a.Np) * 4);
  L.dump_off = (int)off; off += (size_t)CD_THREADS * 16;
  if (off > 160 * 1024) return 0;
  lds = off;
  return var;
}


struct CcPlan {
  int MT, WR, WC, QG;
  int tiles_per_wg;
  int KL, QL;
  int img_rows;
  int w_off, a_off, a_bytes, q_off, q_bytes, os_off, os_wave, par_off, red_off, dump_off;
};

template <int KS, int NPW, int NQW, int K2>
__global__ __launch_bounds__(CD_THREADS) void pw_cdg_c_kernel(const c3d_pw_args a, const CcPlan L) {
  constexpr int NTW = 4;
  extern __shared__ __attribute__((aligned(16))) unsigned char smem[];
  CDCLK(0)
  const int tid = threadIdx.x, lane = tid & 63;
  const int wave = __builtin_amdgcn_readfirstlane(tid >> 6);
  const int Kp = a.Kp, Np = a.Np, Gq = Kp >> 3, MT = L.MT, KL = L.KL, QL = L.QL;
  bf16_t* const Ws = reinterpret_cast<bf16_t*>(smem + L.w_off);
  float* const Pp = reinterpret_cast<float*>(smem + L.par_off);
  float* const Ep = Pp + 3 * Kp;
  float* const red = reinterpret_cast<float*>(smem + L.red_off);
  float* const Gs = Ep + 4 * Np;
  bf16_t* const dump = reinterpret_cast<bf16_t*>(smem + L.dump_off) + tid * 8;

  const int M32 = (int)a.M;
  const int tiles = (M32 + MT - 1) / MT;
  int t0 = (int)blockIdx.x * L.tiles_per_wg;
  if (t0 > tiles) t0 = tiles;
  int t1 = t0 + L.tiles_per_wg;
  if (t1 > tiles) t1 = tiles;
  const uint32_t row_hi = (uint32_t)(t1 * MT < M32 ? t1 * MT : M32);
  const __amdgpu_buffer_rsrc_t rX = cd_rsrc(a.x, row_hi * (uint32_t)Kp * 2u);
  const __amdgpu_buffer_rsrc_t rX2 = cd_rsrc(a.x2, row_hi * (uint32_t)Kp * 2u);
  const __amdgpu_buffer_rsrc_t rE1 = cd_rsrc(a.e1, (uint32_t)M32 * (uint32_t)Np * 2u);
  const __amdgpu_buffer_rsrc_t rY = cd_rsrc(a.y, (uint32_t)M32 * (uint32_t)Np * 2u);
  const uint32_t rps = (uint32_t)a.rows_per_sample;

  int p_desc;
  uint32_t p_go;
  {
    const int row = __float2int_rz(((float)tid + 0.5f) * (1.0f / (float)Gq));
    const bool ok = tid < MT * Gq;
    p_desc = ok ? (row << 5) | (tid - row * Gq) : 0;
    p_go = ok ? (uint32_t)tid * 16u : CD_OOB;
  }
  const uint32_t tbp = (uint32_t)(MT * Kp * 2);
  uint4 rawp[2], rawp2[2];
#pragma unroll
  for (int s_ = 0; s_ < 2; ++s_) { rawp[s_] = cd_load(rX, p_go + (uint32_t)(t0 + s_) * tbp); rawp2[s_] = cd_load(rX2, p_go + (uint32_t)(t0 + s_) * tbp); }

  const int wr = wave % L.WR, wc = wave / L.WR;
  const int nt0 = wc * NTW;
  constexpr int NLW = NTW * 16 + 8;
  bf16_t* const Os = reinterpret_cast<bf16_t*>(smem + L.os_off + wave * L.os_wave);
  constexpr int GOW = NTW * 2, RPO = 64 / GOW, NPASS = 16 / RPO;
  const int rr_o = lane >> 3, v_o = lane & 7;
  const int cvec = nt0 * 2 + v_o;
  const bool act_o = cvec * 8 < Np;
  const int cve = act_o ? cvec : 0;
  uint4 e1r[2][NPASS];
#define CC_EOFF(TILE, P) ((act_o && (TILE) < t1 && (TILE) * MT + wr * 16 + (P) * RPO + rr_o < M32)                                                \
                              ? ((uint32_t)((TILE) * MT + wr * 16 + (P) * RPO + rr_o) * (uint32_t)Np + (uint32_t)cvec * 8u) * 2u : CD_OOB)
#pragma unroll
  for (int s_ = 0; s_ < 2; ++s_)
#pragma unroll
    for (int p = 0; p < NPASS; ++p) e1r[s_][p] = cd_load(rE1, CC_EOFF(t0 + s_, p));

  {
    const int wbytes = (KS * 4) * L.img_rows * 16;
    const int nchunk = (wbytes + 1023) >> 10;
    const unsigned char* src = reinterpret_cast<const unsigned char*>(a.w_img);
    const int rot = (int)blockIdx.x % nchunk;
    for (int c = wave; c < nchunk; c += 8) {
      int r = c + rot;
      if (r >= nchunk) r -= nchunk;
      const int off = r * 1024 + lane * 16;
      if (off < wbytes)
        __builtin_amdgcn_global_load_lds((cd_glb_ptr_t)(src + off), (cd_lds_ptr_t)(smem + L.w_off + r * 1024), 16, 0, 0);
    }
  }
  for (int i = tid * 16; i < 3 * L.a_bytes; i += CD_THREADS * 16) *reinterpret_cast<uint4*>(smem + L.a_off + i) = make_uint4(0u, 0u, 0u, 0u);
  for (int i = tid * 16; i < 2 * L.q_bytes; i += CD_THREADS * 16) *reinterpret_cast<uint4*>(smem + L.q_off + i) = make_uint4(0u, 0u, 0u, 0u);
  if (a.fin.sums) {
    for (int c = tid; c < Kp; c += CD_THREADS) {
      float cA, cB, cC;
      c3dfin::bn_bwd_coef_consume(a.fin, a.K, Kp, c, blockIdx.x == 0, cA, cB, cC);
      Pp[c] = cA; Pp[Kp + c] = cB; Pp[2 * Kp + c] = cC;
    }
  } else {
    for (int i = tid; i < 3 * Kp; i += CD_THREADS) Pp[i] = a.pro_p[i];
  }
  for (int i = tid; i < 2 * Np; i += CD_THREADS) { Ep[i] = a.epi_p[i]; Ep[2 * Np + i] = a.epi_q[i]; }
  asm volatile("s_waitcnt vmcnt(0)" ::: "memory");
  __syncthreads();
  CDCLK(1)

  float s0[8], s1[8], s2[8];
#pragma unroll
  for (int j = 0; j < 8; ++j) { s0[j] = 0.f; s1[j] = 0.f; s2[j] = 0.f; }
  int cur_n = -1;
  const bf16_t* const wfrag = Ws + ((size_t)(lane >> 4) * L.img_rows + nt0 * 16 + (lane & 15)) * 8;
  const int xfrag = (wr * 16 + (lane & 15)) * KL + (lane >> 4) * 8;
  const int qg = wave % L.QG, pg = wave / L.QG;
  const int g4 = lane >> 4, li = lane & 15;
  const int pl = (4 * g4 + (li >> 2)) * KL + 4 * (li & 3) + pg * NPW * 16;
  const int ql = (4 * g4 + (li >> 2)) * QL + 4 * (li & 3) + qg * NQW * 16;
  f32x4_t dacc[NPW][NQW];
#pragma unroll
  for (int i = 0; i < NPW; ++i)
#pragma unroll
    for (int j = 0; j < NQW; ++j) dacc[i][j] = f32x4_t{0.f, 0.f, 0.f, 0.f};

  auto flush = [&]() {
#pragma unroll
    for (int j = 0; j < 8; ++j) {
      float r0 = s0[j], r1 = s1[j], r2 = s2[j];
#pragma unroll
      for (int o = 8; o < 64; o <<= 1) { r0 += __shfl_xor(r0, o, 64); r1 += __shfl_xor(r1, o, 64); r2 += __shfl_xor(r2, o, 64); }
      if (lane < 8) { red[(wave * 24 + j) * 8 + lane] = r0; red[(wave * 24 + 8 + j) * 8 + lane] = r1; red[(wave * 24 + 16 + j) * 8 + lane] = r2; }
      s0[j] = 0.f; s1[j] = 0.f; s2[j] = 0.f;
    }
    __syncthreads();
    for (int i = tid; i < 3 * Np; i += CD_THREADS) {
      const int which = i / Np, c = i - which * Np;
      const int cv = c >> 3, j = c & 7;
      const int wcg = cv >> 3, vo = cv & 7;
      float accv = 0.f;
      for (int w_ = 0; w_ < L.WR; ++w_) accv += red[((wcg * L.WR + w_) * 24 + which * 8 + j) * 8 + vo];
      atomicAdd(a.stats + ((int64_t)cur_n * Np + c) * 3 + which, (double)accv);
    }
    __syncthreads();
  };

#define CC_CONVERT(TILE, CP, S)                                                                                      \
  {                                                                                                                 \
    const int rowg0_ = (TILE) * MT;                                                                                 \
    const uint32_t bpn_ = (uint32_t)((TILE) + 2) * tbp;     \
    const int row = p_desc >> 5, v = p_desc & 31;                                                                   \
    bf16_t* dst = p_go != CD_OOB ? (CP) + row * KL + v * 8 : dump;                                                  \
    float f[8], f2[8], cA[8], cB[8], cC[8];                                                                         \
    cd_cvt(rawp[S], f); cd_cvt(rawp2[S], f2);                                                                       \
    cd_ld8(Pp + v * 8, cA); cd_ld8(Pp + Kp + v * 8, cB); cd_ld8(Pp + 2 * Kp + v * 8, cC);                           \
    const uint32_t keep = rowg0_ + row < M32 ? 0xffffffffu : 0u;                                                    \
    _Pragma("unroll") for (int e = 0; e < 8; ++e)                                                                   \
      f[e] = __uint_as_float(__float_as_uint(fmaf(cA[e], f[e], fmaf(cC[e], f2[e], cB[e]))) & keep);                 \
    Vec8<bf16_t>::store(dst, f);                                                                                    \
    rawp[S] = cd_load(rX, p_go + bpn_);                                                                             \
    rawp2[S] = cd_load(rX2, p_go + bpn_);                                                                           \
  }
#define CC_MULT(CA)                                                                                                 \
  {                                                                                                                 \
     \
    _Pragma("unroll") for (int th = 0; th < NTW; th += 2) {                                                         \
      f32x4_t acc[2] = {f32x4_t{0.f, 0.f, 0.f, 0.f}, f32x4_t{0.f, 0.f, 0.f, 0.f}};                                  \
      _Pragma("unroll") for (int ks = 0; ks < KS; ++ks) {                                                           \
        const uint4 xb = *reinterpret_cast<const uint4*>((CA) + xfrag + ks * 32);                                   \
        _Pragma("unroll") for (int t = 0; t < 2; ++t) {                                                             \
          const uint4 wa = *reinterpret_cast<const uint4*>(wfrag + ((size_t)ks * 4 * L.img_rows + (th + t) * 16) * 8); \
          acc[t] = __builtin_amdgcn_mfma_f32_16x16x32_bf16(__builtin_bit_cast(bf16x8_t, wa), __builtin_bit_cast(bf16x8_t, xb), acc[t], 0, 0, 0); \
        }                                                                                                           \
      }                                                                                                             \
      _Pragma("unroll") for (int t = 0; t < 2; ++t)                                                                 \
        *reinterpret_cast<uint2*>(Os + (lane & 15) * NLW + (th + t) * 16 + (lane >> 4) * 4) =                       \
            make_uint2(pack_bf16x2(acc[t][0], acc[t][1]), pack_bf16x2(acc[t][2], acc[t][3]));                       \
    }                                                                                                               \
  }
#define CC_WGRAD(CA, CQ)                                                                                            \
  {                                                                                                                 \
    _Pragma("unroll") for (int k2 = 0; k2 < K2; ++k2) {                                                             \
      uint4 pa[NPW], qb[NQW];                                                                                       \
      const bf16_t* pb_ = (CA) + k2 * 32 * KL + pl;                                                                 \
      const bf16_t* qb_ = (CQ) + k2 * 32 * QL + ql;                                                                 \
      _Pragma("unroll") for (int i = 0; i < NPW; ++i) {                                                             \
        const cd_s16x4_t lo_ = __builtin_amdgcn_ds_read_tr16_b64_v4i16((cd_lds_s16x4_ptr_t)(pb_ + i * 16));        \
        const cd_s16x4_t hi_ = __builtin_amdgcn_ds_read_tr16_b64_v4i16((cd_lds_s16x4_ptr_t)(pb_ + 16 * KL + i * 16)); \
        pa[i] = __builtin_bit_cast(uint4, __builtin_shufflevector(lo_, hi_, 0, 1, 2, 3, 4, 5, 6, 7));               \
      }                                                                                                             \
      _Pragma("unroll") for (int j = 0; j < NQW; ++j) {                                                             \
        const cd_s16x4_t lo_ = __builtin_amdgcn_ds_read_tr16_b64_v4i16((cd_lds_s16x4_ptr_t)(qb_ + j * 16));        \
        const cd_s16x4_t hi_ = __builtin_amdgcn_ds_read_tr16_b64_v4i16((cd_lds_s16x4_ptr_t)(qb_ + 16 * QL + j * 16)); \
        qb[j] = __builtin_bit_cast(uint4, __builtin_shufflevector(lo_, hi_, 0, 1, 2, 3, 4, 5, 6, 7));               \
      }                                                                                                             \
      _Pragma("unroll") for (int i = 0; i < NPW; ++i)                                                               \
        _Pragma("unroll") for (int j = 0; j < NQW; ++j)                                                             \
          dacc[i][j] = __builtin_amdgcn_mfma_f32_16x16x32_bf16(__builtin_bit_cast(bf16x8_t, pa[i]), __builtin_bit_cast(bf16x8_t, qb[j]), \
                                                               dacc[i][j], 0, 0, 0);                               \
    }                                                                                                               \
  }
#define CC_EPI(TILE, CQ, S)                                                                                         \
  {                                                                                                                 \
    const int row0_ = (TILE) * MT + wr * 16;                                                                        \
    _Pragma("unroll") for (int p = 0; p < NPASS; ++p) {                                                             \
      const int row = p * RPO + rr_o;                                                                               \
      const int m = row0_ + row;                                                                                    \
      const bool ok = act_o && m < M32;                                                                             \
      const uint32_t keep = ok ? 0xffffffffu : 0u;                                                                  \
      const uint4 rawo = *reinterpret_cast<const uint4*>(Os + row * NLW + v_o * 8);                                 \
      float f[8], bv[8], qs[8];                                                                                     \
      cd_cvt(rawo, f); cd_cvt(e1r[S][p], bv);                                                                       \
                             \
      _Pragma("unroll") for (int h = 0; h < 8; h += 4) {                                                            \
        const float4 eS = *reinterpret_cast<const float4*>(Ep + cve * 8 + h), eB = *reinterpret_cast<const float4*>(Ep + Np + cve * 8 + h); \
        const float4 eM = *reinterpret_cast<const float4*>(Ep + 2 * Np + cve * 8 + h), eR = *reinterpret_cast<const float4*>(Ep + 3 * Np + cve * 8 + h); \
        const float eS_[4] = {eS.x, eS.y, eS.z, eS.w}, eB_[4] = {eB.x, eB.y, eB.z, eB.w};                           \
        const float eM_[4] = {eM.x, eM.y, eM.z, eM.w}, eR_[4] = {eR.x, eR.y, eR.z, eR.w};                           \
        const float4 eGv = *reinterpret_cast<const float4*>(Gs + cve * 8 + h);                                      \
        const float eG_[4] = {eGv.x, eGv.y, eGv.z, eGv.w};                                                          \
        _Pragma("unroll") for (int u = 0; u < 4; ++u) {                                                             \
          const int j = h + u;                                                                                      \
          const float pb = fmaf(bv[j], eS_[u], eB_[u]);                                                             \
          const float q = eG_[u] * pb;                                                                              \
          const float sg = sigmoid_t<bf16_t>(q);                                                                    \
          const float dq = __uint_as_float(__float_as_uint(f[j] * sg * (1.f + q * (1.f - sg))) & keep);             \
          const float t = round_as<bf16_t>(dq * eG_[u]);                                                            \
          s0[j] += dq * pb;                                                                                         \
          s1[j] += t;                                                                                               \
          s2[j] += t * ((bv[j] - eM_[u]) * eR_[u]);                                                                 \
          f[j] = t;                                                                                                 \
          qs[j] = __uint_as_float(__float_as_uint(q * sg) & keep);                                                  \
        }                                                                                                           \
        __builtin_amdgcn_sched_barrier(0);                                                                          \
      }                                                                                                             \
      const uint4 pk = make_uint4(pack_bf16x2(f[0], f[1]), pack_bf16x2(f[2], f[3]), pack_bf16x2(f[4], f[5]), pack_bf16x2(f[6], f[7])); \
      __builtin_amdgcn_raw_buffer_store_b128(cd_u32x4_t{pk.x, pk.y, pk.z, pk.w}, rY,                                \
                                             ok ? ((uint32_t)m * (uint32_t)Np + (uint32_t)cvec * 8u) * 2u : CD_OOB, 0, 0); \
      Vec8<bf16_t>::store((CQ) + (wr * 16 + row) * QL + cvec * 8, qs);                                              \
      e1r[S][p] = cd_load(rE1, CC_EOFF((TILE) + 2, p));                                                             \
    }                                                                                                               \
  }

#ifndef CC_SECTIONS
#define CC_SECTIONS 1
#endif
#if CC_SECTIONS
#define CC_SECTION __builtin_amdgcn_sched_barrier(0);
#else
#define CC_SECTION
#endif
  bf16_t* pP = reinterpret_cast<bf16_t*>(smem + L.a_off);
  bf16_t* cP = reinterpret_cast<bf16_t*>(smem + L.a_off + L.a_bytes);
  bf16_t* nP = reinterpret_cast<bf16_t*>(smem + L.a_off + 2 * L.a_bytes);
  bf16_t* const bufQ0 = reinterpret_cast<bf16_t*>(smem + L.q_off);
  bf16_t* const bufQ1 = reinterpret_cast<bf16_t*>(smem + L.q_off + L.q_bytes);
  bf16_t* lastQ = bufQ0;
  if (t0 < t1) CC_CONVERT(t0, cP, 0)
  CDCLK(2)
#define CC_ITER(TILE, S, CURQ, PRVQ)                                                                                \
  {                                                                                                                 \
    const int n_tile = (int)((uint32_t)((TILE) * MT) / rps);                                                        \
    if (n_tile != cur_n) {                                                \
      if (cur_n >= 0) flush();                                                                                      \
      cur_n = n_tile;                                                                                               \
       \
      for (int i = tid; i < Np; i += CD_THREADS) Gs[i] = a.epi_gate ? a.epi_gate[(int64_t)cur_n * Np + i] : 1.f;    \
    }                                                                                                               \
    __syncthreads();    \
    CC_MULT(cP)                                                                                                     \
    CC_SECTION                                                                                                      \
    CC_WGRAD(pP, PRVQ)                                                                                              \
    CC_SECTION                                                                                                      \
    CC_CONVERT((TILE) + 1, nP, 1 - (S))                                                                             \
    CC_SECTION                                                                                                      \
    CC_EPI(TILE, CURQ, S)                                                                                           \
    bf16_t* const tmp = pP; pP = cP; cP = nP; nP = tmp;                                                             \
    lastQ = (CURQ);                                                                                                 \
  }
  for (int tile = t0; tile < t1; tile += 2) {
    CC_ITER(tile, 0, bufQ0, bufQ1)
    if (tile + 1 < t1) CC_ITER(tile + 1, 1, bufQ1, bufQ0)
  }
#undef CC_ITER
  CDCLK(3)
  if (t0 < t1) {
    __syncthreads();
    CC_WGRAD(pP, lastQ)
  }
#undef CC_CONVERT
#undef CC_MULT
#undef CC_WGRAD
#undef CC_EPI
#undef CC_EOFF

  {
    float* wsb = a.wg_ws + (size_t)blockIdx.x * a.K * a.N;
#pragma unroll
    for (int i = 0; i < NPW; ++i) {
#pragma unroll
      for (int j = 0; j < NQW; ++j) {
        const int n = (qg * NQW + j) * 16 + (lane & 15);
#pragma unroll
        for (int r = 0; r < 4; ++r) {
          const int k = (pg * NPW + i) * 16 + (lane >> 4) * 4 + r;
          if (k < a.K && n < a.N) wsb[(size_t)k * a.N + n] = dacc[i][j][r];
        }
      }
    }
  }
  CDCLK(4)
  if (cur_n >= 0) flush();
  CDCLK(5)
}

template <int KS, int NPW, int NQW, int K2>
int cc_launch(const c3d_pw_args& a, const CcPlan& L, dim3 grid, size_t lds, hipStream_t s) {
  static bool attr_set = false;
  if (!attr_set) {
    hipError_t e = hipFuncSetAttribute(reinterpret_cast<const void*>(&pw_cdg_c_kernel<KS, NPW, NQW, K2>),
                                       hipFuncAttributeMaxDynamicSharedMemorySize, 160 * 1024);
    if (e != hipSuccess) return (int)e;
    attr_set = true;
  }
  pw_cdg_c_kernel<KS, NPW, NQW, K2><<<grid, dim3(CD_THREADS), lds, s>>>(a, L);
  return 0;
}

int cc_variant(int Kp, int Np) {
  const int KS = (Kp + 31) / 32, ntn = (Np + 15) >> 4, ntp = (Kp + 15) >> 4;
  if (KS == 3 && ntn >= 13 && ntn <= 14 && ntp <= 6) return 1;
  if (KS == 2 && ntn == 7 && ntp <= 3) return 2;
  if (KS == 1 && ntn == 4 && ntp <= 2) return 3;
  return 0;
}

int cc_plan(const c3d_pw_args& a, CcPlan& L, int64_t& blocks, size_t& lds) {
  const int var = cc_variant(a.Kp, a.Np);
  if (!var) return 0;
  const int Kpad = (a.Kp + 31) / 32 * 32, KS = Kpad / 32, ntn = (a.Np + 15) >> 4;
  L.img_rows = (ntn <= 2 ? 2 : ntn <= 4 ? 4 : ntn <= 7 ? 7 : 14) * 16;
  if (var == 1) { L.WR = 2; L.WC = 4; L.QG = 4; }
  else if (var == 2) { L.WR = 4; L.WC = 2; L.QG = 8; }
  else { L.WR = 8; L.WC = 1; L.QG = 4; }
  L.MT = 16 * L.WR;
  if ((L.MT * (a.Kp >> 3)) > CD_THREADS) return 0;
  if (a.rows_per_sample <= 0 || a.rows_per_sample % L.MT) return 0;
  L.KL = Kpad + 8;
  L.QL = L.WC * 4 * 16 + 8;
  const int64_t tiles = (a.M + L.MT - 1) / L.MT;
  blocks = device_cus();
  if (blocks > (tiles + 1) / 2) blocks = (tiles + 1) / 2;
  if (blocks > CD_MAX_PARTS) blocks = CD_MAX_PARTS;
  if (blocks < 1) blocks = 1;
  const int tpw = (int)((tiles + blocks - 1) / blocks);
  blocks = (tiles + tpw - 1) / tpw;
  L.tiles_per_wg = tpw;
  auto al = [](size_t v) { return (v + 1023) / 1024 * 1024; };
  size_t off = 0;
  L.w_off = 0; off += al((size_t)KS * 4 * L.img_rows * 16);
  L.a_off = (int)off; L.a_bytes = (int)al((size_t)L.MT * L.KL * 2); off += 3 * (size_t)L.a_bytes;
  L.q_off = (int)off; L.q_bytes = (int)al((size_t)L.MT * L.QL * 2); off += 2 * (size_t)L.q_bytes;
  L.os_wave = 16 * (4 * 16 + 8) * 2; L.os_off = (int)off; off += al((size_t)8 * L.os_wave);
  L.par_off = (int)off; off += al(((size_t)3 * a.Kp + 5 * a.Np) * 4);
  L.red_off = (int)off; off += al((size_t)8 * 24 * 8 * 4);
  L.dump_off = (int)off; off += (size_t)CD_THREADS * 16;
  if (off > 160 * 1024) return 0;
  lds = off;
  return var;
}

}

__attribute__((visibility("hidden"))) bool c3d_detail_pw_cdg_a_supported(int Kp, int Np, int64_t M) {
  if (Kp <= 0 || Np <= 0 || (Kp & 7) || (Np & 7)) return false;
  if (M < 1024 || (M + 512) * (int64_t)(Kp > Np ? Kp : Np) * 2 >= ((int64_t)1 << 31)) return false;
  c3d_pw_args a;
  std::memset(&a, 0, sizeof(a));
  a.M = M; a.K = a.Kp = Kp; a.N = a.Np = Np;
  CdPlan L;
  int64_t blocks = 0;
  size_t lds = 0;
  return cd_plan(a, L, blocks, lds) != 0;
}

__attribute__((visibility("hidden"))) int c3d_detail_pw_cdg_a(const c3d_pw_args* args, void* stream) {
  const c3d_pw_args& a = *args;
  if (a.dtype != C3D_DT_BF16 || a.row_mode != C3D_ROWS_DENSE || a.pro_mode != C3D_PRO_AFFINE2 || a.epi_mode != C3D_EPI_ADD ||
      a.wg_mode != C3D_WG_ROWS || a.res_mode != 0)
    return C3D_E_UNSUPPORTED;
  if (!a.w_img || !a.x2 || !a.e1 || !a.wg_x3 || !a.wg_dw || !a.wg_ws || a.pro_out || a.bias || a.fin.ticket) return C3D_E_UNSUPPORTED;
  if (a.fin.sums ? (a.fin.training != 0 || !a.fin.mr || !a.fin.gamma) : !a.pro_p) return C3D_E_UNSUPPORTED;
  if (a.add_sums && (!a.add_c || !a.add_mr || !a.wg_mask_out)) return C3D_E_UNSUPPORTED;
  if (a.M < 1024 || (a.M + 512) * (int64_t)(a.Kp > a.Np ? a.Kp : a.Np) * 2 >= ((int64_t)1 << 31)) return C3D_E_UNSUPPORTED;
  CdPlan L;
  int64_t blocks = 0;
  size_t lds = 0;
  const int var = cd_plan(a, L, blocks, lds);
  if (!var) return C3D_E_UNSUPPORTED;
  hipStream_t s = reinterpret_cast<hipStream_t>(stream);
  const dim3 grid((unsigned)blocks);
  int rc = C3D_E_UNSUPPORTED;
  if (var == 1) rc = cd_launch<7, 2, 4, 3, 2, 1, 1>(a, L, grid, lds, s);
  else if (var == 2) rc = cd_launch<4, 3, 1, 3, 4, 2, 4>(a, L, grid, lds, s);
  else if (var == 3) rc = cd_launch<2, 2, 1, 1, 2, 1, 4>(a, L, grid, lds, s);
  if (rc != 0) return rc;
  C3D_CHECK_LAUNCH();
  if (c3d_cdg_defer_reduce) { c3d_cdg_parts = (int)blocks; return 0; }
  return c3d_detail_pw_wgrad_reduce(a.wg_ws, a.wg_dw, a.K, a.N, (int)blocks, a.w_sk, a.w_sn, s);
}

__attribute__((visibility("hidden"))) bool c3d_detail_pw_cdg_c_supported(int Kp, int Np, int64_t M, int64_t rows_per_sample) {
  if (Kp <= 0 || Np <= 0 || (Kp & 7) || (Np & 7)) return false;
  if (M < 1024 || (M + 512) * (int64_t)(Kp > Np ? Kp : Np) * 2 >= ((int64_t)1 << 31)) return false;
  c3d_pw_args a;
  std::memset(&a, 0, sizeof(a));
  a.M = M; a.K = a.Kp = Kp; a.N = a.Np = Np; a.rows_per_sample = rows_per_sample;
  CcPlan L;
  int64_t blocks = 0;
  size_t lds = 0;
  return cc_plan(a, L, blocks, lds) != 0;
}

__attribute__((visibility("hidden"))) int c3d_detail_pw_cdg_c(const c3d_pw_args* args, void* stream) {
  const c3d_pw_args& a = *args;
  if (a.dtype != C3D_DT_BF16 || a.row_mode != C3D_ROWS_DENSE || a.pro_mode != C3D_PRO_AFFINE2 || a.epi_mode != C3D_EPI_SWISH_SE_BWD ||
      a.wg_mode != C3D_WG_SWISH)
    return C3D_E_UNSUPPORTED;
  if (!a.w_img || !a.x2 || !a.e1 || !a.epi_p || !a.epi_q || !a.stats || !a.wg_dw || !a.wg_ws || a.pro_out || a.bias || a.fin.ticket ||
      a.add_sums)
    return C3D_E_UNSUPPORTED;
  if (a.fin.sums ? (a.fin.training != 0 || !a.fin.mr || !a.fin.gamma) : !a.pro_p) return C3D_E_UNSUPPORTED;
  if (a.M < 1024 || (a.M + 512) * (int64_t)(a.Kp > a.Np ? a.Kp : a.Np) * 2 >= ((int64_t)1 << 31)) return C3D_E_UNSUPPORTED;
  CcPlan L;
  int64_t blocks = 0;
  size_t lds = 0;
  const int var = cc_plan(a, L, blocks, lds);
  if (!var) return C3D_E_UNSUPPORTED;
  hipStream_t s = reinterpret_cast<hipStream_t>(stream);
  const dim3 grid((unsigned)blocks);
  int rc = C3D_E_UNSUPPORTED;
  if (var == 1) rc = cc_launch<3, 3, 4, 1>(a, L, grid, lds, s);
  else if (var == 2) rc = cc_launch<2, 3, 1, 2>(a, L, grid, lds, s);
  else if (var == 3) rc = cc_launch<1, 1, 1, 4>(a, L, grid, lds, s);
  if (rc != 0) return rc;
  C3D_CHECK_LAUNCH();
  if (c3d_cdg_defer_reduce) { c3d_cdg_parts = (int)blocks; return 0; }
  return c3d_detail_pw_wgrad_reduce(a.wg_ws, a.wg_dw, a.K, a.N, (int)blocks, a.w_sk, a.w_sn, s);
}
```

change3d_amd/csrc/stage_driver.hip:

```cpp
#include "../../include/change3d_hip.h"
#include <hip/hip_runtime.h>
#include <cstdlib>
#include "common.h"
#include "launch_hints.h"
#include <cstdio>
#include <cstring>
#include <deque>
#include <mutex>
#include <vector>

bool c3d_detail_pw_gemm_wg_supported(int Kp, int Np, int wg_mode);
bool c3d_detail_pw_gemm_masksum_supported(int Kp, int Np);

namespace {

inline int cpad(int c) { return (c + 7) / 8 * 8; }
inline size_t al(size_t v) { return (v + 255) / 256 * 256; }
inline size_t es(int dtype) { return dtype == C3D_DT_F32 ? 4 : 2; }
constexpr int S = C3D_STAT_STRIPES;
enum { SC_NONE = 0, SC_IDENTITY = 1, SC_BN = 2, SC_RAW = 3 };

#define RC(call)              \
  do {                        \
    const int rc_ = (call);   \
    if (rc_ != 0) return rc_; \
  } while (0)
#define HIPRC(call)                            \
  do {                                         \
    const hipError_t e_ = (call);              \
    if (e_ != hipSuccess) return (int)e_;      \
  } while (0)

struct BlkGeom {
  int H, W, Ho, Wo;
  int64_t M, Mo;
  int Cin, Ci, Co, Cinp, Cip, Cop, s, Cr;
  bool se, sc_conv, sc_bn;
};

struct BlkFwd {
  size_t a, b, c, sc, y;
  size_t ss_a, mr_a, ss_b, mr_b, gate, hid, ss_c, mr_c, ss_1, mr_1;
  size_t sums_a, nc_b, sums_c, sums_1;
  size_t tick;
  size_t img_a, img_at, img_c, img_ct, img_s, img_st;
};

#ifndef C3D_BWD_RING_DEFAULT
#define C3D_BWD_RING_DEFAULT 3
#endif
constexpr int BWD_RING_MAX = 8;
int bwd_ring() {
  static const int r = [] {
    const char* s = c3d_env("C3D_BWD_RING");
    const int v = s ? atoi(s) : C3D_BWD_RING_DEFAULT;
    return v < 2 ? 2 : (v > BWD_RING_MAX ? BWD_RING_MAX : v);
  }();
  return r;
}

struct BlkBwd {
  size_t g, t1, t2, dxs, dx;
  size_t coef_c, coef_1, coef_a, cA, cC, cB;
  size_t dsums_c, dsums_1, nc3, dsums_a;
  size_t tick;
};

struct Plan {
  std::vector<BlkGeom> g;
  std::vector<BlkFwd> f;
  std::vector<BlkBwd> b;
  size_t fwd_acc_off = 0, fwd_acc_bytes = 0, fwd_total = 0;
  size_t bwd_acc_off = 0, bwd_acc_bytes = 0, bwd_total = 0, wgrad_ws = 0, wgrad_ws2 = 0, wgrad_ws_fused = 0, wgrad_ws_fused_slot = 0;
  size_t y_bytes = 0, dx_bytes = 0;
};

struct Carver {
  size_t off = 0;
  size_t take(size_t bytes) { const size_t o = off; off += al(bytes); return o; }
};

inline bool fuse_wgrad(const c3d_stage_desc* d, int Kp, int Np, int wg_mode) {
  return !(d->flags & C3D_STAGE_SEPARATE_WGRAD) && d->dtype == C3D_DT_BF16 && Kp <= 112 && Np <= 112 && c3d_knob("C3D_PW_WG", 1) &&
         c3d_detail_pw_gemm_wg_supported(Kp, Np, wg_mode);
}

int g_mask_in_dgrad = 3;
int g_fold_se = 1;
int g_fuse_wgrad = 3;
int g_wgrad_chain = 1;

int make_plan(const c3d_stage_desc* d, Plan& P) {
  if (!d || d->n_blocks <= 0 || !d->blocks || d->B <= 0 || d->T <= 0 || d->H <= 0 || d->W <= 0) return C3D_E_BADARG;
  if (d->dtype != C3D_DT_F32 && d->dtype != C3D_DT_BF16) return C3D_E_BADARG;
  const size_t e = es(d->dtype);
  const int n = d->n_blocks;
  P.g.resize(n); P.f.resize(n); P.b.resize(n);
  int H = d->H, W = d->W;
  for (int i = 0; i < n; ++i) {
    const c3d_block_desc& k = d->blocks[i];
    if (k.cin <= 0 || k.cinner <= 0 || k.cout <= 0 || (k.stride != 1 && k.stride != 2)) return C3D_E_BADARG;
    if (i > 0 && k.cin != d->blocks[i - 1].cout) return C3D_E_BADARG;
    if (!k.has_sc_conv && (k.cin != k.cout || k.stride != 1)) return C3D_E_BADARG;
    if (k.has_sc_bn && !k.has_sc_conv) return C3D_E_BADARG;
    BlkGeom& G = P.g[i];
    G.H = H; G.W = W; G.s = k.stride;
    G.Ho = (H - 1) / k.stride + 1; G.Wo = (W - 1) / k.stride + 1;
    G.M = (int64_t)d->B * d->T * H * W; G.Mo = (int64_t)d->B * d->T * G.Ho * G.Wo;
    G.Cin = k.cin; G.Ci = k.cinner; G.Co = k.cout;
    G.Cinp = cpad(k.cin); G.Cip = cpad(k.cinner); G.Cop = cpad(k.cout);
    G.se = k.se_width > 0; G.Cr = k.se_width; G.sc_conv = k.has_sc_conv != 0; G.sc_bn = k.has_sc_bn != 0;
    {
      const int cmax = std::max(std::max(G.Cinp, G.Cip), G.Cop);
      if (cmax <= 224 && (int64_t)std::max(G.M, G.Mo) * cmax * (int64_t)e >= ((int64_t)1 << 31)) return C3D_E_UNSUPPORTED;
    }
    H = G.Ho; W = G.Wo;
  }
  Carver cf;
  for (int i = 0; i < n; ++i) {
    const BlkGeom& G = P.g[i];
    BlkFwd& F = P.f[i];
    F.a = cf.take((size_t)G.M * G.Cip * e);
    F.b = cf.take((size_t)G.Mo * G.Cip * e);
    F.c = cf.take((size_t)G.Mo * G.Cop * e);
    F.sc = G.sc_conv ? cf.take((size_t)G.Mo * G.Cop * e) : SIZE_MAX;
    F.y = i + 1 < n ? cf.take((size_t)G.Mo * G.Cop * e) : SIZE_MAX;
  }
  for (int i = 0; i < n; ++i) {
    const BlkGeom& G = P.g[i];
    BlkFwd& F = P.f[i];
    F.ss_a = cf.take(2 * G.Cip * 4); F.mr_a = cf.take(2 * G.Cip * 4);
    F.ss_b = cf.take(2 * G.Cip * 4); F.mr_b = cf.take(2 * G.Cip * 4);
    F.gate = G.se ? cf.take((size_t)d->B * G.Cip * 4) : SIZE_MAX;
    F.hid = G.se ? cf.take((size_t)d->B * G.Cr * 4) : SIZE_MAX;
    F.ss_c = cf.take(2 * G.Cop * 4); F.mr_c = cf.take(2 * G.Cop * 4);
    F.ss_1 = G.sc_bn ? cf.take(2 * G.Cop * 4) : SIZE_MAX;
    F.mr_1 = G.sc_bn ? cf.take(2 * G.Cop * 4) : SIZE_MAX;
  }
  P.fwd_acc_off = cf.off;
  for (int i = 0; i < n; ++i) {
    const BlkGeom& G = P.g[i];
    BlkFwd& F = P.f[i];
    F.sums_a = cf.take((size_t)S * 2 * G.Ci * 8);
    F.nc_b = cf.take((size_t)d->B * G.Cip * 2 * 8);
    F.sums_c = cf.take((size_t)S * 2 * G.Co * 8);
    F.sums_1 = G.sc_bn ? cf.take((size_t)S * 2 * G.Co * 8) : SIZE_MAX;
    F.tick = cf.take(16);
  }
  P.fwd_acc_bytes = cf.off - P.fwd_acc_off;
  for (int i = 0; i < n; ++i) {
    const BlkGeom& G = P.g[i];
    BlkFwd& F = P.f[i];
    auto img = [&](int Np, int Kp) -> size_t {
      const int64_t b = c3d_pw_weight_image_bytes(Np, Kp, d->dtype);
      return b > 0 ? cf.take((size_t)b) : SIZE_MAX;
    };
    F.img_a = img(G.Cip, G.Cinp); F.img_at = img(G.Cinp, G.Cip);
    F.img_c = img(G.Cop, G.Cip); F.img_ct = img(G.Cip, G.Cop);
    F.img_s = G.sc_conv ? img(G.Cop, G.Cinp) : SIZE_MAX;
    F.img_st = G.sc_conv ? img(G.Cinp, G.Cop) : SIZE_MAX;
  }
  P.fwd_total = cf.off;
  size_t mx_g = 0, mx_t1 = 0, mx_t2 = 0, mx_dxs = 0, mx_dx = 0;
  int64_t wsf = 0, wsf_fused = 0;
  for (int i = 0; i < n; ++i) {
    const BlkGeom& G = P.g[i];
    if (fuse_wgrad(d, G.Cop, G.Cip, C3D_WG_SWISH)) wsf_fused = std::max(wsf_fused, c3d_pw_gemm_wg_ws_floats(G.Co, G.Ci));
    if (fuse_wgrad(d, G.Cip, G.Cinp, C3D_WG_ROWS)) wsf_fused = std::max(wsf_fused, c3d_pw_gemm_wg_ws_floats(G.Ci, G.Cin));
    if (d->dtype == C3D_DT_BF16 && c3d_detail_pw_cdg_a_supported(G.Cip, G.Cinp, G.M)) wsf_fused = std::max(wsf_fused, c3d_pw_gemm_wg_ws_floats(G.Ci, G.Cin));
    if (d->dtype == C3D_DT_BF16 && c3d_detail_pw_cdg_c_supported(G.Cop, G.Cip, G.Mo, (int64_t)d->T * G.Ho * G.Wo))
      wsf_fused = std::max(wsf_fused, c3d_pw_gemm_wg_ws_floats(G.Co, G.Ci));
    mx_g = std::max(mx_g, (size_t)G.Mo * G.Cop * e);
    mx_t1 = std::max(mx_t1, (size_t)G.Mo * G.Cip * e);
    mx_t2 = std::max(mx_t2, (size_t)G.M * G.Cip * e);
    if (G.sc_conv) mx_dxs = std::max(mx_dxs, (size_t)G.Mo * G.Cinp * e);
    if (i > 0) mx_dx = std::max(mx_dx, (size_t)G.M * G.Cinp * e);
    wsf = std::max(wsf, c3d_pw_wgrad_ws_floats(G.Co, G.Ci));
    wsf = std::max(wsf, c3d_pw_wgrad_ws_floats(G.Ci, G.Cin));
    wsf = std::max(wsf, c3d_pw_wgrad_ws_floats(G.Co, G.Cin));
  }
  Carver cb;
  const int R = bwd_ring();
  size_t ring[BWD_RING_MAX][4];
  for (int r = 0; r < R; ++r) {
    ring[r][0] = cb.take(mx_g); ring[r][1] = cb.take(mx_t1); ring[r][2] = cb.take(mx_t2);
    ring[r][3] = mx_dxs ? cb.take(mx_dxs) : SIZE_MAX;
  }
  size_t ring_dx[BWD_RING_MAX + 1];
  for (int r = 0; r < R + 1; ++r) ring_dx[r] = mx_dx ? cb.take(mx_dx) : SIZE_MAX;
  P.wgrad_ws = cb.take((size_t)wsf * 4);
  P.wgrad_ws2 = cb.take((size_t)wsf * 4);
  P.wgrad_ws_fused = wsf_fused ? cb.take((size_t)wsf_fused * 4 * (1 + 2 * (size_t)n)) : SIZE_MAX;
  P.wgrad_ws_fused_slot = (size_t)wsf_fused * 4;
  for (int i = 0; i < n; ++i) {
    const BlkGeom& G = P.g[i];
    BlkBwd& Bk = P.b[i];
    const int r = i % R;
    Bk.g = ring[r][0]; Bk.t1 = ring[r][1]; Bk.t2 = ring[r][2]; Bk.dxs = ring[r][3];
    Bk.dx = i > 0 ? ring_dx[i % (R + 1)] : SIZE_MAX;
    Bk.coef_c = cb.take(3 * G.Cop * 4);
    Bk.coef_1 = G.sc_bn ? cb.take(3 * G.Cop * 4) : SIZE_MAX;
    Bk.coef_a = cb.take(3 * G.Cip * 4);
    Bk.cA = cb.take(G.Cip * 4); Bk.cC = cb.take(G.Cip * 4); Bk.cB = cb.take((size_t)d->B * G.Cip * 4);
  }
  P.bwd_acc_off = cb.off;
  for (int i = 0; i < n; ++i) {
    const BlkGeom& G = P.g[i];
    BlkBwd& Bk = P.b[i];
    Bk.dsums_c = cb.take(2 * G.Co * 8);
    Bk.dsums_1 = G.sc_bn ? cb.take(2 * G.Co * 8) : SIZE_MAX;
    Bk.nc3 = cb.take((size_t)d->B * G.Cip * 3 * 8);
    Bk.dsums_a = cb.take(2 * G.Ci * 8);
    Bk.tick = cb.take(16);
  }
  P.bwd_acc_bytes = cb.off - P.bwd_acc_off;
  P.bwd_total = cb.off;
  P.y_bytes = (size_t)P.g[n - 1].Mo * P.g[n - 1].Cop * e;
  P.dx_bytes = (size_t)P.g[0].M * P.g[0].Cinp * e;
  return 0;
}

struct ProfRec { char name[64]; hipEvent_t e0, e1; double bytes; };
std::vector<ProfRec> g_prof;
int g_prof_flags = -1;
char g_prof_tag[32] = "";

template <typename F>
int prof_call(const char* name, double bytes, hipStream_t s, F&& fn) {
  if (g_prof_flags < 0) return fn();
  ProfRec r;
  if ((g_prof_flags & 2) && g_prof_tag[0] && !std::strchr(name, '['))
    std::snprintf(r.name, sizeof(r.name), "%s[%s]", name, g_prof_tag);
  else
    std::snprintf(r.name, sizeof(r.name), "%s", name);
  r.bytes = bytes;
  HIPRC(hipEventCreate(&r.e0));
  HIPRC(hipEventCreate(&r.e1));
  HIPRC(hipEventRecord(r.e0, s));
  const int rc = fn();
  HIPRC(hipEventRecord(r.e1, s));
  g_prof.push_back(r);
  return rc;
}
inline bool prof_detail() { return g_prof_flags >= 0 && (g_prof_flags & 2); }

struct SideCtx {
  hipStream_t side = nullptr;
  std::vector<hipEvent_t> pool;
  size_t next = 0;
  std::deque<std::pair<uint64_t, hipEvent_t>> marks;
  uint64_t seq = 0;
  hipEvent_t ev() {
    if (pool.size() < 256) {
      hipEvent_t e;
      if (hipEventCreateWithFlags(&e, hipEventDisableTiming | hipEventDisableSystemFence) != hipSuccess) return nullptr;
      pool.push_back(e);
      return e;
    }
    next = (next + 1) % pool.size();
    return pool[next];
  }
};

std::mutex g_mu;
SideCtx g_side[16];

int g_side_on = 1;
bool side_enabled() { return g_side_on != 0 && !(g_prof_flags >= 0 && (g_prof_flags & 1)); }

SideCtx* side_ctx() {
  int dev = 0;
  if (hipGetDevice(&dev) != hipSuccess || dev < 0 || dev >= 16) return nullptr;
  SideCtx& c = g_side[dev];
  if (!c.side) {
    static const bool low = c3d_env("C3D_SIDE_PRIO") && atoi(c3d_env("C3D_SIDE_PRIO")) == 1;
    int lo = 0, hi = 0;
    if (low && hipDeviceGetStreamPriorityRange(&lo, &hi) == hipSuccess) {
      if (hipStreamCreateWithPriority(&c.side, hipStreamNonBlocking, lo) != hipSuccess) return nullptr;
    } else if (hipStreamCreateWithFlags(&c.side, hipStreamNonBlocking) != hipSuccess) {
      return nullptr;
    }
  }
  return &c;
}

template <typename F>
int side_run(hipStream_t main, F&& fn) {
  if (!side_enabled()) return fn(main);
  std::lock_guard<std::mutex> lk(g_mu);
  SideCtx* c = side_ctx();
  if (!c) return fn(main);
  hipEvent_t fork = c->ev();
  if (!fork) return fn(main);
  HIPRC(hipEventRecord(fork, main));
  HIPRC(hipStreamWaitEvent(c->side, fork, 0));
  c3d_side_launch = 1;
  const int rc_fn = fn(c->side);
  c3d_side_launch = 0;
  RC(rc_fn);
  hipEvent_t done = c->ev();
  if (!done) return (int)hipErrorOutOfMemory;
  HIPRC(hipEventRecord(done, c->side));
  c->marks.emplace_back(++c->seq, done);
  while (c->marks.size() > 64) c->marks.pop_front();
  return 0;
}

uint64_t side_mark() {
  std::lock_guard<std::mutex> lk(g_mu);
  SideCtx* c = side_ctx();
  return c ? c->seq : 0;
}

int side_join(hipStream_t main, uint64_t upto) {
  std::lock_guard<std::mutex> lk(g_mu);
  SideCtx* c = side_ctx();
  if (!c) return 0;
  hipEvent_t last = nullptr;
  while (!c->marks.empty() && c->marks.front().first <= upto) {
    last = c->marks.front().second;
    c->marks.pop_front();
  }
  if (last) HIPRC(hipStreamWaitEvent(main, last, 0));
  return 0;
}

struct PwCall {
  c3d_pw_args a;
  PwCall(const void* x, const float* w, void* y, int64_t M, int K, int N, int w_sn, int w_sk, int dtype) {
    std::memset(&a, 0, sizeof(a));
    a.x = x; a.w = w; a.y = y; a.M = M; a.K = K; a.Kp = cpad(K); a.N = N; a.Np = cpad(N);
    a.w_sn = w_sn; a.w_sk = w_sk; a.dtype = dtype;
    a.pro_mode = C3D_PRO_NONE; a.epi_mode = C3D_EPI_STORE; a.row_mode = C3D_ROWS_DENSE;
  }
};

struct WgCall {
  c3d_pw_wgrad_args a;
  WgCall(const void* p, const void* q, float* dw, float* ws, int64_t M, int K, int N, int dw_sn, int dw_sk, int dtype) {
    std::memset(&a, 0, sizeof(a));
    a.p = p; a.q = q; a.dw = dw; a.ws = ws; a.M = M; a.K = K; a.Kp = cpad(K); a.N = N; a.Np = cpad(N);
    a.dw_sn = dw_sn; a.dw_sk = dw_sk; a.dtype = dtype; a.q_mode = C3D_PRO_NONE; a.row_mode = C3D_ROWS_DENSE;
  }
};

inline bool fin_consumer(const c3d_stage_desc* d) { return !(d->flags & C3D_STAGE_SEPARATE_FINALIZE); }
inline bool fuse_residual(const c3d_stage_desc* d) { return !(d->flags & C3D_STAGE_SEPARATE_RESIDUAL); }
inline bool use_pw_img(const c3d_stage_desc* d) { return !(d->flags & C3D_STAGE_NO_WEIGHT_IMAGES); }

inline c3d_bn_fin fin_consume(const double* sums, const c3d_bn_ptrs& bn, double count, float momentum, float eps,
                              float* ss, float* mr) {
  c3d_bn_fin f;
  std::memset(&f, 0, sizeof(f));
  f.gamma = bn.gamma; f.beta = bn.beta; f.running_mean = bn.running_mean; f.running_var = bn.running_var;
  f.nbt = bn.num_batches_tracked; f.ss = ss; f.mr = mr; f.count = count; f.momentum = momentum; f.eps = eps;
  f.training = 1; f.sums = sums;
  return f;
}

inline c3d_bn_fin fin_coef_consume(const double* dsums, const c3d_bn_ptrs& bn, double count, const float* mr,
                                   bool accumulate) {
  c3d_bn_fin f;
  std::memset(&f, 0, sizeof(f));
  f.sums = dsums; f.gamma = bn.gamma; f.mr = const_cast<float*>(mr); f.count = count;
  if (accumulate) { f.running_mean = bn.dgamma; f.running_var = bn.dbeta; }
  return f;
}

inline char* at(void* base, size_t off) { return off == SIZE_MAX ? nullptr : reinterpret_cast<char*>(base) + off; }
template <typename T> inline T* atT(void* base, size_t off) { return reinterpret_cast<T*>(at(base, off)); }


__global__ __launch_bounds__(256) void zero_fill_kernel(uint4* __restrict__ p, size_t n16) {
  for (size_t i = (size_t)blockIdx.x * 256 + threadIdx.x; i < n16; i += (size_t)gridDim.x * 256) p[i] = make_uint4(0, 0, 0, 0);
}
int zero_fill(void* p, size_t bytes, hipStream_t st) {
  if (!bytes) return 0;
  if (((uintptr_t)p & 15) || (bytes & 15)) { HIPRC(hipMemsetAsync(p, 0, bytes, st)); return 0; }
  const size_t n16 = bytes >> 4;
  size_t blocks = (n16 + 255) / 256;
  if (blocks > 1024) blocks = 1024;
  zero_fill_kernel<<<dim3((unsigned)blocks), dim3(256), 0, st>>>(reinterpret_cast<uint4*>(p), n16);
  hipError_t e = hipGetLastError();
  return e == hipSuccess ? 0 : (int)e;
}

__global__ void fold_bn_kernel(const float* __restrict__ w, float* __restrict__ wf, int N, int K, const float* __restrict__ gamma,
                               const float* __restrict__ beta, const float* __restrict__ mean, const float* __restrict__ var,
                               float eps, float* __restrict__ ss, int Cp) {
  const int n = blockIdx.x;
  if (n >= Cp) return;
  float sc = 0.f, sh = 0.f;
  if (n < N) {
    const float rstd = (float)(1.0 / sqrt((double)var[n] + (double)eps));
    sc = gamma[n] * rstd;
    sh = beta[n] - mean[n] * sc;
    for (int k = threadIdx.x; k < K; k += blockDim.x) wf[(size_t)n * K + k] = w[(size_t)n * K + k] * sc;
  }
  if (threadIdx.x == 0) { ss[n] = n < N ? 1.f : 0.f; ss[Cp + n] = sh; }
}

struct BlkFold { size_t w_a, w_b, w_c, w_sc, ss_a, ss_b, ss_c, ss_1; };
struct BlkEval { size_t a, b, c, sc, y, gate, hid, nc_b; };
struct FoldPlan {
  std::vector<BlkFold> f;
  std::vector<BlkEval> e;
  size_t fold_total = 0, ws_total = 0, acc_off = 0, acc_bytes = 0;
};

int make_fold_plan(const c3d_stage_desc* d, const Plan& P, FoldPlan& Q) {
  const int n = d->n_blocks;
  const size_t e = es(d->dtype);
  Q.f.resize(n); Q.e.resize(n);
  Carver cf;
  for (int i = 0; i < n; ++i) {
    const BlkGeom& G = P.g[i];
    BlkFold& F = Q.f[i];
    F.w_a = cf.take((size_t)G.Ci * G.Cin * 4); F.w_b = cf.take((size_t)G.Ci * 27 * 4);
    F.w_c = cf.take((size_t)G.Co * G.Ci * 4);
    F.w_sc = G.sc_conv ? cf.take((size_t)G.Co * G.Cin * 4) : SIZE_MAX;
    F.ss_a = cf.take(2 * G.Cip * 4); F.ss_b = cf.take(2 * G.Cip * 4); F.ss_c = cf.take(2 * G.Cop * 4);
    F.ss_1 = G.sc_bn ? cf.take(2 * G.Cop * 4) : SIZE_MAX;
  }
  Q.fold_total = cf.off;
  size_t mx_a = 0, mx_b = 0, mx_c = 0, mx_y = 0, mx_gate = 0, mx_hid = 0, mx_nc = 0;
  for (int i = 0; i < n; ++i) {
    const BlkGeom& G = P.g[i];
    mx_a = std::max(mx_a, (size_t)G.M * G.Cip * e); mx_b = std::max(mx_b, (size_t)G.Mo * G.Cip * e);
    mx_c = std::max(mx_c, (size_t)G.Mo * G.Cop * e); mx_y = std::max(mx_y, (size_t)G.Mo * G.Cop * e);
    mx_gate = std::max(mx_gate, (size_t)d->B * G.Cip * 4); mx_hid = std::max(mx_hid, (size_t)d->B * std::max(G.Cr, 1) * 4);
    mx_nc = std::max(mx_nc, (size_t)d->B * G.Cip * 2 * 8);
  }
  Carver cw;
  const size_t a = cw.take(mx_a), b = cw.take(mx_b), c = cw.take(mx_c), sc = cw.take(mx_c);
  const size_t y0 = cw.take(mx_y), y1 = cw.take(mx_y), gate = cw.take(mx_gate), hid = cw.take(mx_hid);
  Q.acc_off = cw.off;
  for (int i = 0; i < n; ++i) {
    BlkEval& E = Q.e[i];
    E.a = a; E.b = b; E.c = c; E.sc = sc; E.y = (i & 1) ? y1 : y0; E.gate = gate; E.hid = hid;
    E.nc_b = P.g[i].se ? cw.take((size_t)d->B * P.g[i].Cip * 2 * 8) : SIZE_MAX;
  }
  Q.acc_bytes = cw.off - Q.acc_off;
  Q.ws_total = cw.off;
  return 0;
}

}

extern "C" int c3d_stage_ws_bytes(const c3d_stage_desc* d, int64_t* ws_fwd_bytes, int64_t* ws_bwd_bytes, int64_t* y_bytes,
                                  int64_t* dx_bytes) {
  Plan P;
  RC(make_plan(d, P));
  if (ws_fwd_bytes) *ws_fwd_bytes = (int64_t)P.fwd_total;
  if (ws_bwd_bytes) *ws_bwd_bytes = (int64_t)P.bwd_total;
  if (y_bytes) *y_bytes = (int64_t)P.y_bytes;
  if (dx_bytes) *dx_bytes = (int64_t)P.dx_bytes;
  return 0;
}

extern "C" int c3d_stage_saved(const c3d_stage_desc* d, int32_t blk, const char* name, int64_t* offset, int64_t* bytes) {
  Plan P;
  RC(make_plan(d, P));
  if (blk < 0 || blk >= d->n_blocks || !name || !offset || !bytes) return C3D_E_BADARG;
  const BlkGeom& G = P.g[blk];
  const BlkFwd& F = P.f[blk];
  const size_t e = es(d->dtype);
  size_t off = SIZE_MAX, n = 0;
  if (!strcmp(name, "a")) { off = F.a; n = (size_t)G.M * G.Cip * e; }
  else if (!strcmp(name, "b")) { off = F.b; n = (size_t)G.Mo * G.Cip * e; }
  else if (!strcmp(name, "c")) { off = F.c; n = (size_t)G.Mo * G.Cop * e; }
  else if (!strcmp(name, "sc")) { off = F.sc; n = (size_t)G.Mo * G.Cop * e; }
  else if (!strcmp(name, "mr_a")) { off = F.mr_a; n = 2 * G.Cip * 4; }
  else if (!strcmp(name, "mr_b")) { off = F.mr_b; n = 2 * G.Cip * 4; }
  else if (!strcmp(name, "mr_c")) { off = F.mr_c; n = 2 * G.Cop * 4; }
  else if (!strcmp(name, "mr_sc")) { off = F.mr_1; n = 2 * G.Cop * 4; }
  else if (!strcmp(name, "ss_a")) { off = F.ss_a; n = 2 * G.Cip * 4; }
  else if (!strcmp(name, "ss_b")) { off = F.ss_b; n = 2 * G.Cip * 4; }
  else if (!strcmp(name, "ss_c")) { off = F.ss_c; n = 2 * G.Cop * 4; }
  else if (!strcmp(name, "ss_sc")) { off = F.ss_1; n = 2 * G.Cop * 4; }
  else if (!strcmp(name, "gate")) { off = F.gate; n = (size_t)d->B * G.Cip * 4; }
  if (off == SIZE_MAX) return C3D_E_BADARG;
  *offset = (int64_t)off; *bytes = (int64_t)n;
  return 0;
}

extern "C" int c3d_side_join(void* stream) { return side_join(reinterpret_cast<hipStream_t>(stream), UINT64_MAX); }

namespace {

int pw_launch(const c3d_pw_args& a, hipStream_t st) {
  const double bytes = (double)a.M * ((double)a.Kp * (a.x2 ? 2 : 1) + (double)a.Np * (a.e1 ? 2 : 1) + (a.pro_out ? a.Kp : 0) +
                                     ((a.wg_mode == C3D_WG_ROWS || a.wg_mode == C3D_WG_MASKSUM) ? a.Np : 0) + (a.add_sums ? a.Np : 0)) * (double)es(a.dtype);
  char nm[64];
  if (prof_detail())
    std::snprintf(nm, sizeof(nm), "c3d_pw_gemm[M=%lld K=%d N=%d pro=%d epi=%d rows=%d%s]", (long long)a.M, a.K, a.N, a.pro_mode,
                  a.epi_mode, a.row_mode, a.wg_mode == C3D_WG_MASKSUM ? " +bob" : a.wg_mode ? (a.add_sums ? " +dW +bob" : " +dW") : "");
  else
    std::snprintf(nm, sizeof(nm), "c3d_pw_gemm");
  return prof_call(nm, bytes, st, [&] { return c3d_pw_gemm(&a, st); });
}

int wg_launch(const c3d_pw_wgrad_args& a, hipStream_t st) {
  const double bytes = (double)a.M * ((double)a.Np * (a.p2 ? 2 : 1) + (double)a.Kp) * (double)es(a.dtype);
  char nm[64];
  if (prof_detail())
    std::snprintf(nm, sizeof(nm), "c3d_pw_wgrad[M=%lld K=%d N=%d q=%d rows=%d]", (long long)a.M, a.K, a.N, a.q_mode, a.row_mode);
  else
    std::snprintf(nm, sizeof(nm), "c3d_pw_wgrad");
  return prof_call(nm, bytes, st, [&] { return c3d_pw_wgrad(&a, st); });
}

}

extern "C" int c3d_stage_fwd(const c3d_stage_desc* d, const void* x, void* ws, void* y_out, void* stream) {
  Plan P;
  RC(make_plan(d, P));
  if (!x || !ws || !y_out) return C3D_E_BADARG;
  hipStream_t st = reinterpret_cast<hipStream_t>(stream);
  const int dt = d->dtype, tr = d->training ? 1 : 0, B = d->B, T = d->T;
  const double e = (double)es(dt);
  RC(zero_fill(at(ws, P.fwd_acc_off), P.fwd_acc_bytes, st));
  const bool wimg = use_pw_img(d);
  auto imgp = [&](size_t off) -> const void* { return wimg && off != SIZE_MAX ? at(ws, off) : nullptr; };
  if (wimg) {
    std::vector<c3d_pw_pack_desc> pk;
    auto add = [&](const float* w, size_t off, int N, int K, int sn, int sk) {
      if (off != SIZE_MAX) pk.push_back(c3d_pw_pack_desc{w, at(ws, off), N, cpad(N), K, cpad(K), sn, sk});
    };
    for (int i = 0; i < d->n_blocks; ++i) {
      const c3d_block_desc& k = d->blocks[i];
      const BlkGeom& G = P.g[i];
      const BlkFwd& F = P.f[i];
      add(k.w_a, F.img_a, G.Ci, G.Cin, G.Cin, 1);
      add(k.w_c, F.img_c, G.Co, G.Ci, G.Ci, 1);
      if (G.sc_conv) add(k.w_sc, F.img_s, G.Co, G.Cin, G.Cin, 1);
      add(k.w_a, F.img_at, G.Cin, G.Ci, 1, G.Cin);
      add(k.w_c, F.img_ct, G.Ci, G.Co, 1, G.Ci);
      if (G.sc_conv) add(k.w_sc, F.img_st, G.Cin, G.Co, 1, G.Cin);
    }
    RC(prof_call("c3d_pw_pack_weights", 0.0, st, [&] { return c3d_pw_pack_weights(pk.data(), (int32_t)pk.size(), dt, st); }));
  }
  const int epi = tr ? C3D_EPI_STATS : C3D_EPI_STORE;
  const void* cur = x;
  struct Pending { const void* c; const void* sc; c3d_bn_fin fin; void* y; bool on; } pend;
  std::memset(&pend, 0, sizeof(pend));
  for (int i = 0; i < d->n_blocks; ++i) {
    const c3d_block_desc& k = d->blocks[i];
    const BlkGeom& G = P.g[i];
    if (prof_detail()) std::snprintf(g_prof_tag, sizeof(g_prof_tag), "H=%d Ci=%d s=%d se=%d", G.H, G.Ci, G.s, (int)G.se);
    const BlkFwd& F = P.f[i];
    void* a = at(ws, F.a); void* b = at(ws, F.b); void* c = at(ws, F.c); void* sc = at(ws, F.sc);
    void* y = F.y == SIZE_MAX ? y_out : at(ws, F.y);
    float* ss_a = atT<float>(ws, F.ss_a); float* mr_a = atT<float>(ws, F.mr_a);
    float* ss_b = atT<float>(ws, F.ss_b); float* mr_b = atT<float>(ws, F.mr_b);
    float* ss_c = atT<float>(ws, F.ss_c); float* mr_c = atT<float>(ws, F.mr_c);
    float* ss_1 = atT<float>(ws, F.ss_1); float* mr_1 = atT<float>(ws, F.mr_1);
    float* gate = atT<float>(ws, F.gate); float* hid = atT<float>(ws, F.hid);
    double* sums_a = atT<double>(ws, F.sums_a); double* nc_b = atT<double>(ws, F.nc_b);
    double* sums_c = atT<double>(ws, F.sums_c); double* sums_1 = atT<double>(ws, F.sums_1);
    const int64_t rps = (int64_t)T * G.Ho * G.Wo;
    if (pend.on) {
      PwCall p(pend.c, k.w_a, a, G.M, G.Cin, G.Ci, G.Cin, 1, dt);
      p.a.x2 = pend.sc; p.a.pro_mode = C3D_PRO_AFFINE2; p.a.fin = pend.fin; p.a.pro_p = pend.fin.ss; p.a.pro_out = pend.y;
      p.a.epi_mode = epi; p.a.stats = sums_a; p.a.w_img = imgp(F.img_a);
      RC(pw_launch(p.a, st));
      pend.on = false;
    } else {
      PwCall p(cur, k.w_a, a, G.M, G.Cin, G.Ci, G.Cin, 1, dt);
      p.a.epi_mode = epi; p.a.stats = sums_a; p.a.w_img = imgp(F.img_a);
      RC(pw_launch(p.a, st));
    }
    const bool cons = tr && fin_consumer(d);
    const double dw_bytes = ((double)G.M + (double)G.Mo) * G.Cip * e;
    if (cons) {
      const c3d_bn_fin fa = fin_consume(sums_a, k.bn_a, (double)G.M, d->momentum, d->eps, ss_a, mr_a);
      RC(prof_call("c3d_dw333_fwd", dw_bytes, st, [&] {
        return c3d_dw333_fwd_fin(a, &fa, k.w_b, b, nc_b, B, T, G.H, G.W, G.Ci, G.Cip, G.s, dt, st); }));
    } else {
      RC(prof_call("c3d_bn_finalize", 0.0, st, [&] {
        return c3d_bn_finalize(sums_a, S, (double)G.M, k.bn_a.gamma, k.bn_a.beta, k.bn_a.running_mean, k.bn_a.running_var,
                               tr ? k.bn_a.num_batches_tracked : nullptr, d->momentum, d->eps, G.Ci, G.Cip, tr, ss_a, mr_a, st); }));
      RC(prof_call("c3d_dw333_fwd", dw_bytes, st, [&] {
        return c3d_dw333_fwd(a, ss_a, k.w_b, b, nc_b, B, T, G.H, G.W, G.Ci, G.Cip, G.s, dt, st); }));
    }
    const bool fold_b = cons && G.Cip <= 224 && G.Cop <= 224 && (!G.se || (g_fold_se && G.Cr <= 32));
    if (!fold_b)
    RC(prof_call("c3d_bn_se_finalize", 0.0, st, [&] {
      return c3d_bn_se_finalize(nc_b, B, (double)rps, k.bn_b.gamma, k.bn_b.beta, k.bn_b.running_mean, k.bn_b.running_var,
                                tr ? k.bn_b.num_batches_tracked : nullptr, d->momentum, d->eps, G.Ci, G.Cip, tr,
                                G.se ? k.se_w1 : nullptr, k.se_b1, k.se_w2, k.se_b2, G.Cr, ss_b, mr_b, gate, hid, st); }));
    {
      PwCall p(b, k.w_c, c, G.Mo, G.Ci, G.Co, G.Ci, 1, dt);
      p.a.pro_mode = C3D_PRO_BN_SE_SWISH; p.a.pro_p = ss_b; p.a.pro_gate = gate; p.a.rows_per_sample = rps;
      if (fold_b) {
        p.a.fin = fin_consume(nc_b, k.bn_b, (double)rps * B, d->momentum, d->eps, ss_b, mr_b);
        p.a.fin.batch = B;
        if (G.se) { p.a.se_w1 = k.se_w1; p.a.se_b1 = k.se_b1; p.a.se_w2 = k.se_w2; p.a.se_b2 = k.se_b2; p.a.se_hid = hid; p.a.se_cr = G.Cr; }
      }
      p.a.epi_mode = epi; p.a.stats = sums_c; p.a.w_img = imgp(F.img_c);
      RC(pw_launch(p.a, st));
    }
    auto finalize = [&](const double* sums, const c3d_bn_ptrs& bn, int C, int Cp, float* ss, float* mr) {
      return prof_call("c3d_bn_finalize", 0.0, st, [&] {
        return c3d_bn_finalize(sums, S, (double)G.Mo, bn.gamma, bn.beta, bn.running_mean, bn.running_var,
                               tr ? bn.num_batches_tracked : nullptr, d->momentum, d->eps, C, Cp, tr, ss, mr, st); });
    };
    if (!cons) RC(finalize(sums_c, k.bn_c, G.Co, G.Cop, ss_c, mr_c));
    int mode = SC_IDENTITY;
    const void* scp = cur;
    if (G.sc_conv) {
      PwCall p(cur, k.w_sc, sc, G.Mo, G.Cin, G.Co, G.Cin, 1, dt);
      p.a.row_mode = G.s == 2 ? C3D_ROWS_STRIDE2 : C3D_ROWS_DENSE; p.a.H = G.H; p.a.W = G.W;
      p.a.epi_mode = G.sc_bn ? epi : C3D_EPI_STORE; p.a.stats = sums_1; p.a.w_img = imgp(F.img_s);
      RC(pw_launch(p.a, st));
      if (G.sc_bn) {
        if (!cons) RC(finalize(sums_1, k.bn_sc, G.Co, G.Cop, ss_1, mr_1));
        mode = SC_BN;
      } else {
        mode = SC_RAW;
      }
      scp = sc;
    }
    const bool fuse_next = cons && fuse_residual(d) && i + 1 < d->n_blocks && mode != SC_BN && dt == C3D_DT_BF16 &&
                           G.Cop <= 224 && P.g[i + 1].Cip <= 224 && d->blocks[i + 1].stride == 1 && !d->blocks[i + 1].has_sc_conv;
    const double bo_bytes = (double)G.Mo * G.Cop * 3 * e;
    if (fuse_next) {
      pend.c = c; pend.sc = scp; pend.y = y; pend.on = true;
      pend.fin = fin_consume(sums_c, k.bn_c, (double)G.Mo, d->momentum, d->eps, ss_c, mr_c);
    } else if (cons) {
      const c3d_bn_fin fc = fin_consume(sums_c, k.bn_c, (double)G.Mo, d->momentum, d->eps, ss_c, mr_c);
      c3d_bn_fin f1;
      if (mode == SC_BN) f1 = fin_consume(sums_1, k.bn_sc, (double)G.Mo, d->momentum, d->eps, ss_1, mr_1);
      RC(prof_call("c3d_block_out_fwd", bo_bytes, st, [&] {
        return c3d_block_out_fwd_fin(c, &fc, scp, mode == SC_BN ? &f1 : nullptr, mode, y, G.Mo, G.Co, G.Cop, dt, st); }));
    } else {
      RC(prof_call("c3d_block_out_fwd", bo_bytes, st, [&] {
        return c3d_block_out_fwd(c, ss_c, scp, ss_1, mode, y, G.Mo, G.Cop, dt, st); }));
    }
    cur = y;
  }
  return 0;
}

extern "C" int c3d_stage_bwd(const c3d_stage_desc* d, const void* x, const void* y_out, const void* dy, void* ws,
                             void* wb, void* dx_out, void* stream) {
  Plan P;
  RC(make_plan(d, P));
  if (!x || !y_out || !dy || !ws || !wb || !dx_out) return C3D_E_BADARG;
  hipStream_t st = reinterpret_cast<hipStream_t>(stream);
  const int dt = d->dtype, B = d->B, T = d->T;
  const double e = (double)es(dt);
  RC(zero_fill(at(wb, P.bwd_acc_off), P.bwd_acc_bytes, st));
  float* const wgws_ab[2] = {atT<float>(wb, P.wgrad_ws), atT<float>(wb, P.wgrad_ws2)};
  int wg_n = 0;
  float* wgws_fused = atT<float>(wb, P.wgrad_ws_fused);
  int cdg_n = 0;
  struct RedJob { const float* ws; float* dw; int K, N, parts, sk, sn; };
  std::vector<RedJob> red_jobs;
  c3d_detail_pw_wgrad_v2_drop();
  const bool wimg = use_pw_img(d);
  auto imgp = [&](size_t off) -> const void* { return wimg && off != SIZE_MAX ? at(ws, off) : nullptr; };
  const void* cur_dy = dy;
  bool premasked = false;
  bool sums_done = false;
  std::deque<uint64_t> lag;
  for (int i = d->n_blocks - 1; i >= 0; --i) {
    const c3d_block_desc& k = d->blocks[i];
    const BlkGeom& G = P.g[i];
    if (prof_detail()) std::snprintf(g_prof_tag, sizeof(g_prof_tag), "H=%d Ci=%d s=%d se=%d", G.H, G.Ci, G.s, (int)G.se);
    const BlkFwd& F = P.f[i];
    const BlkBwd& Bk = P.b[i];
    const void* xin = i == 0 ? x : (P.f[i - 1].y == SIZE_MAX ? y_out : at(ws, P.f[i - 1].y));
    const void* a = at(ws, F.a); const void* b = at(ws, F.b); const void* c = at(ws, F.c); const void* sc = at(ws, F.sc);
    const void* y = F.y == SIZE_MAX ? y_out : at(ws, F.y);
    const float* ss_a = atT<float>(ws, F.ss_a); const float* mr_a = atT<float>(ws, F.mr_a);
    const float* ss_b = atT<float>(ws, F.ss_b); const float* mr_b = atT<float>(ws, F.mr_b);
    const float* mr_c = atT<float>(ws, F.mr_c); const float* mr_1 = atT<float>(ws, F.mr_1);
    const float* gate = atT<float>(ws, F.gate); const float* hid = atT<float>(ws, F.hid);
    const double* nc_b = atT<double>(ws, F.nc_b);
    void* g = at(wb, Bk.g); void* t1 = at(wb, Bk.t1); void* t2 = at(wb, Bk.t2); void* dxs = at(wb, Bk.dxs);
    void* dx = i == 0 ? dx_out : at(wb, Bk.dx);
    float* coef_c = atT<float>(wb, Bk.coef_c); float* coef_1 = atT<float>(wb, Bk.coef_1);
    float* coef_a = atT<float>(wb, Bk.coef_a);
    float* cA = atT<float>(wb, Bk.cA); float* cC = atT<float>(wb, Bk.cC); float* cB = atT<float>(wb, Bk.cB);
    double* dsums_c = atT<double>(wb, Bk.dsums_c); double* dsums_1 = atT<double>(wb, Bk.dsums_1);
    double* nc3 = atT<double>(wb, Bk.nc3); double* dsums_a = atT<double>(wb, Bk.dsums_a);
    const int64_t rps = (int64_t)T * G.Ho * G.Wo;
    const bool scbn = G.sc_bn;
    const bool consb = fin_consumer(d) && dt == C3D_DT_BF16;
    auto coef = [&](const double* dsums, double count, const c3d_bn_ptrs& bn, const float* mr, int C, int Cp, float* out) {
      return prof_call("c3d_bn_bwd_coef", 0.0, st, [&] {
        return c3d_bn_bwd_coef(dsums, 1, count, bn.gamma, mr, C, Cp, out, bn.dgamma, bn.dbeta, st); });
    };
    if (premasked && sums_done) {
      g = const_cast<void*>(cur_dy);
    } else if (premasked) {
      g = const_cast<void*>(cur_dy);
      RC(prof_call("c3d_block_out_bwd", (double)G.Mo * G.Cop * (scbn ? 3 : 2) * e, st, [&] {
        return c3d_block_out_bwd(cur_dy, nullptr, c, scbn ? sc : nullptr, nullptr, mr_c, scbn ? mr_1 : nullptr, dsums_c,
                                 scbn ? dsums_1 : nullptr, G.Mo, G.Co, G.Cop, dt, st); }));
    } else
    RC(prof_call("c3d_block_out_bwd", (double)G.Mo * G.Cop * (scbn ? 5 : 4) * e, st, [&] {
      return c3d_block_out_bwd(cur_dy, y, c, scbn ? sc : nullptr, g, mr_c, scbn ? mr_1 : nullptr, dsums_c,
                               scbn ? dsums_1 : nullptr, G.Mo, G.Co, G.Cop, dt, st); }));
    if (!consb) RC(coef(dsums_c, (double)G.Mo, k.bn_c, mr_c, G.Co, G.Cop, coef_c));
    const bool coop_wc = (c3d_option_pw_cdg & 2) && dt == C3D_DT_BF16 && !(d->flags & C3D_STAGE_SEPARATE_WGRAD) && imgp(F.img_ct) != nullptr &&
                         c3d_detail_pw_cdg_c_supported(G.Cop, G.Cip, G.Mo, rps);
    const bool fuse_wc = coop_wc || ((g_fuse_wgrad & 2) && fuse_wgrad(d, G.Cop, G.Cip, C3D_WG_SWISH) && G.Cop <= 48);
    if (!fuse_wc)
    RC(side_run(st, [&](hipStream_t s2) {
      WgCall w(g, b, k.dw_c, wgws_ab[wg_n++ & 1], G.Mo, G.Ci, G.Co, G.Ci, 1, dt);
      w.a.chain = g_wgrad_chain;
      w.a.p2 = c; w.a.p_coef = coef_c; w.a.q_mode = C3D_PRO_BN_SE_SWISH; w.a.q_ss = ss_b; w.a.q_gate = gate;
      w.a.rows_per_sample = rps;
      if (consb) w.a.p_fin = fin_coef_consume(dsums_c, k.bn_c, (double)G.Mo, mr_c, false);
      return wg_launch(w.a, s2);
    }));
    {
      PwCall p(g, k.w_c, t1, G.Mo, G.Co, G.Ci, 1, G.Ci, dt);
      if (fuse_wc) { p.a.wg_mode = C3D_WG_SWISH; p.a.wg_dw = k.dw_c; p.a.wg_ws = wgws_fused; }
      p.a.x2 = c; p.a.pro_mode = C3D_PRO_AFFINE2; p.a.pro_p = coef_c;
      if (consb) p.a.fin = fin_coef_consume(dsums_c, k.bn_c, (double)G.Mo, mr_c, true);
      p.a.epi_mode = C3D_EPI_SWISH_SE_BWD; p.a.e1 = b; p.a.epi_p = ss_b; p.a.epi_gate = gate; p.a.epi_q = mr_b;
      p.a.stats = nc3; p.a.rows_per_sample = rps; p.a.w_img = imgp(F.img_ct);
      if (coop_wc && side_enabled()) {
        float* const wsk = wgws_fused + (size_t)(1 + cdg_n) * (P.wgrad_ws_fused_slot / 4);
        p.a.wg_ws = wsk;
        c3d_cdg_defer_reduce = 1; c3d_cdg_parts = 0;
        const int rcl = pw_launch(p.a, st);
        c3d_cdg_defer_reduce = 0;
        RC(rcl);
        if (c3d_cdg_parts > 0) { ++cdg_n; red_jobs.push_back({wsk, p.a.wg_dw, p.a.K, p.a.N, c3d_cdg_parts, p.a.w_sk, p.a.w_sn}); }
      } else {
        RC(pw_launch(p.a, st));
      }
    }
    const bool fold_b = fin_consumer(d) && !G.se && G.s == 1;
    if (!fold_b)
    RC(prof_call("c3d_se_bn_bwd_coef", 0.0, st, [&] {
      return c3d_se_bn_bwd_coef(nc3, nc_b, B, (double)rps, k.bn_b.gamma, mr_b, ss_b, G.Ci, G.Cip, G.se ? k.se_w1 : nullptr,
                                k.se_w2, gate, hid, G.Cr, cA, cC, cB, k.bn_b.dgamma, k.bn_b.dbeta, k.dse_w1, k.dse_b1,
                                k.dse_w2, k.dse_b2, st); }));
    if (fold_b) {
      c3d_bn_fin fb;
      std::memset(&fb, 0, sizeof(fb));
      fb.sums = nc3; fb.batch = B; fb.gamma = k.bn_b.gamma; fb.mr = const_cast<float*>(mr_b); fb.count = (double)rps * B;
      fb.running_mean = k.bn_b.dgamma; fb.running_var = k.bn_b.dbeta;
      RC(prof_call("c3d_dw333_bwd_fused", ((double)G.Mo * 2 + (double)G.M * 2) * G.Cip * e, st, [&] {
        return c3d_dw333_bwd_fused_fin(t1, b, &fb, k.w_b, a, ss_a, mr_a, t2, dsums_a, k.dw_b, B, T, G.H, G.W, G.Ci, G.Cip, 1, dt, st); }));
    } else {
      RC(prof_call("c3d_dw333_bwd_fused", ((double)G.Mo * 2 + (double)G.M * 2) * G.Cip * e, st, [&] {
        return c3d_dw333_bwd_fused(t1, b, cA, cB, cC, k.w_b, a, ss_a, mr_a, t2, dsums_a, k.dw_b, B, T, G.H, G.W, G.Ci, G.Cip, G.s, dt, st); }));
    }
    if (!consb) RC(coef(dsums_a, (double)G.M, k.bn_a, mr_a, G.Ci, G.Cip, coef_a));
    const void* res = g;
    int res_mode = 0;
    if (G.sc_conv) {
      const int rm = G.s == 2 ? C3D_ROWS_STRIDE2 : C3D_ROWS_DENSE;
      PwCall p(g, k.w_sc, dxs, G.Mo, G.Co, G.Cin, 1, G.Cin, dt);
      p.a.w_img = imgp(F.img_st);
      if (scbn) {
        if (!consb) RC(coef(dsums_1, (double)G.Mo, k.bn_sc, mr_1, G.Co, G.Cop, coef_1));
        p.a.x2 = sc; p.a.pro_mode = C3D_PRO_AFFINE2; p.a.pro_p = coef_1;
        if (consb) p.a.fin = fin_coef_consume(dsums_1, k.bn_sc, (double)G.Mo, mr_1, true);
      }
      RC(pw_launch(p.a, st));
      RC(side_run(st, [&](hipStream_t s2) {
        WgCall w(g, xin, k.dw_sc, wgws_ab[wg_n++ & 1], G.Mo, G.Cin, G.Co, G.Cin, 1, dt);
        w.a.chain = g_wgrad_chain;
        if (scbn) {
          w.a.p2 = sc; w.a.p_coef = coef_1;
          if (consb) w.a.p_fin = fin_coef_consume(dsums_1, k.bn_sc, (double)G.Mo, mr_1, false);
        }
        w.a.row_mode = rm; w.a.H = G.H; w.a.W = G.W;
        return wg_launch(w.a, s2);
      }));
      res = dxs;
      res_mode = G.s == 2 ? 1 : 0;
    }
    const bool coop_wa = (c3d_option_pw_cdg & 1) && dt == C3D_DT_BF16 && !(d->flags & C3D_STAGE_SEPARATE_WGRAD) && res_mode == 0 &&
                         imgp(F.img_at) != nullptr && c3d_detail_pw_cdg_a_supported(G.Cip, G.Cinp, G.M);
    const bool fuse_wa = coop_wa || ((g_fuse_wgrad & 1) && fuse_wgrad(d, G.Cip, G.Cinp, C3D_WG_ROWS));
    bool mask_next = false, sums_next = false;
    if (!fuse_wa)
    RC(side_run(st, [&](hipStream_t s2) {
      WgCall w(t2, xin, k.dw_a, wgws_ab[wg_n++ & 1], G.M, G.Cin, G.Ci, G.Cin, 1, dt);
      w.a.chain = g_wgrad_chain;
      w.a.p2 = a; w.a.p_coef = coef_a;
      if (consb) w.a.p_fin = fin_coef_consume(dsums_a, k.bn_a, (double)G.M, mr_a, false);
      return wg_launch(w.a, s2);
    }));
    {
      PwCall p(t2, k.w_a, dx, G.M, G.Ci, G.Cin, 1, G.Cin, dt);
      if (fuse_wa) { p.a.wg_mode = C3D_WG_ROWS; p.a.wg_x3 = xin; p.a.wg_dw = k.dw_a; p.a.wg_ws = wgws_fused; }
      const bool masksum = !fuse_wa && dt == C3D_DT_BF16 && c3d_detail_pw_gemm_masksum_supported(G.Cip, G.Cinp);
      mask_next = i > 0 && (g_mask_in_dgrad & 1) && res_mode == 0 && (fuse_wa || (masksum && (g_mask_in_dgrad & 2)));
      sums_next = mask_next && (g_mask_in_dgrad & 2) && !P.g[i - 1].sc_bn;
      if (mask_next && !fuse_wa && !sums_next) mask_next = false;
      p.a.wg_mask_out = mask_next ? 1 : 0;
      if (mask_next && !fuse_wa) { p.a.wg_mode = C3D_WG_MASKSUM; p.a.wg_x3 = xin; }
      if (sums_next) {
        p.a.add_c = at(ws, P.f[i - 1].c); p.a.add_mr = atT<float>(ws, P.f[i - 1].mr_c);
        p.a.add_sums = atT<double>(wb, P.b[i - 1].dsums_c);
      }
      p.a.x2 = a; p.a.pro_mode = C3D_PRO_AFFINE2; p.a.pro_p = coef_a;
      if (consb) p.a.fin = fin_coef_consume(dsums_a, k.bn_a, (double)G.M, mr_a, true);
      p.a.epi_mode = C3D_EPI_ADD; p.a.e1 = res; p.a.res_mode = res_mode; p.a.H = G.H; p.a.W = G.W;
      p.a.w_img = imgp(F.img_at);
      if (coop_wa && side_enabled()) {
        float* const wsk = wgws_fused + (size_t)(1 + cdg_n) * (P.wgrad_ws_fused_slot / 4);
        p.a.wg_ws = wsk;
        c3d_cdg_defer_reduce = 1; c3d_cdg_parts = 0;
        const int rcl = pw_launch(p.a, st);
        c3d_cdg_defer_reduce = 0;
        RC(rcl);
        if (c3d_cdg_parts > 0) { ++cdg_n; red_jobs.push_back({wsk, p.a.wg_dw, p.a.K, p.a.N, c3d_cdg_parts, p.a.w_sk, p.a.w_sn}); }
      } else {
        RC(pw_launch(p.a, st));
      }
    }
    lag.push_back(side_mark());
    if ((int)lag.size() >= bwd_ring()) { RC(side_join(st, lag.front())); lag.pop_front(); }
    cur_dy = dx;
    premasked = mask_next;
    sums_done = sums_next;
  }
  if (wg_n || !red_jobs.empty())
    RC(side_run(st, [&](hipStream_t s2) {
      for (const RedJob& j : red_jobs) RC(c3d_detail_pw_wgrad_reduce(j.ws, j.dw, j.K, j.N, j.parts, j.sk, j.sn, s2));
      return wg_n ? c3d_pw_wgrad_flush(s2) : 0;
    }));
  return 0;
}

int c3d_option_stem_mfma = 2, c3d_option_convt_mfma = 1;
int c3d_option_dw_ring = 13;
int c3d_option_pw_wgrad_v2 = 1;
int c3d_option_pw_cfwd = 3;
int c3d_option_pw_cdg = 3;
int c3d_option_dw_fwd_hv = 5;
int c3d_option_dw_t4 = 1;

extern "C" int c3d_set_option(int32_t option, int32_t value) {
  switch (option) {
    case C3D_OPT_SIDE_STREAM: g_side_on = value ? 1 : 0; return 0;
    case C3D_OPT_STEM_MFMA: c3d_option_stem_mfma = value < 0 ? 0 : (value > 2 ? 2 : value); return 0;
    case C3D_OPT_CONVT_MFMA: c3d_option_convt_mfma = value ? 1 : 0; return 0;
    case C3D_OPT_FUSE_WGRAD: g_fuse_wgrad = value & 3; return 0;
    case C3D_OPT_FOLD_SE: g_fold_se = value ? 1 : 0; return 0;
    case C3D_OPT_MASK_IN_DGRAD: g_mask_in_dgrad = value & 3; return 0;
    case C3D_OPT_DW_RING: c3d_option_dw_ring = value & 15; return 0;
    case C3D_OPT_DW_FWD_HV: c3d_option_dw_fwd_hv = value & 7; return 0;
    case C3D_OPT_DW_T4: c3d_option_dw_t4 = value ? 1 : 0; return 0;
    case C3D_OPT_PW_CFWD: c3d_option_pw_cfwd = value & 3; return 0;
    case C3D_OPT_PW_CDG: c3d_option_pw_cdg = value & 3; return 0;
    case C3D_OPT_PW_WGRAD_V2: c3d_option_pw_wgrad_v2 = value & 1; g_wgrad_chain = (value & 2) ? 0 : 1; return 0;
    default: return C3D_E_BADARG;
  }
}

extern "C" int c3d_prof_begin(int32_t flags) {
  for (ProfRec& r : g_prof) { (void)hipEventDestroy(r.e0); (void)hipEventDestroy(r.e1); }
  g_prof.clear();
  g_prof_flags = flags & 3;
  g_prof_tag[0] = 0;
  return 0;
}

extern "C" int c3d_prof_end(c3d_prof_row* rows, int32_t cap, int32_t* n_rows) {
  g_prof_flags = -1;
  if (!n_rows || (cap > 0 && !rows)) return C3D_E_BADARG;
  HIPRC(hipDeviceSynchronize());
  int n = 0;
  for (ProfRec& r : g_prof) {
    float ms = 0.f;
    HIPRC(hipEventElapsedTime(&ms, r.e0, r.e1));
    (void)hipEventDestroy(r.e0); (void)hipEventDestroy(r.e1);
    int j = 0;
    while (j < n && std::strncmp(rows[j].name, r.name, sizeof(rows[j].name)) != 0) ++j;
    if (j == n) {
      if (n >= cap) continue;
      std::memset(&rows[n], 0, sizeof(rows[n]));
      std::snprintf(rows[n].name, sizeof(rows[n].name), "%s", r.name);
      ++n;
    }
    rows[j].launches += 1; rows[j].ms_total += ms; rows[j].bytes_total += r.bytes;
  }
  g_prof.clear();
  *n_rows = n;
  return 0;
}

extern "C" int c3d_stage_fold_bytes(const c3d_stage_desc* d, int64_t* fold_bytes, int64_t* ws_eval_bytes) {
  Plan P;
  RC(make_plan(d, P));
  FoldPlan Q;
  RC(make_fold_plan(d, P, Q));
  if (fold_bytes) *fold_bytes = (int64_t)Q.fold_total;
  if (ws_eval_bytes) *ws_eval_bytes = (int64_t)Q.ws_total;
  return 0;
}

extern "C" int c3d_stage_fold_bn(const c3d_stage_desc* d, void* fold, void* stream) {
  Plan P;
  RC(make_plan(d, P));
  FoldPlan Q;
  RC(make_fold_plan(d, P, Q));
  if (!fold) return C3D_E_BADARG;
  hipStream_t st = reinterpret_cast<hipStream_t>(stream);
  for (int i = 0; i < d->n_blocks; ++i) {
    const c3d_block_desc& k = d->blocks[i];
    const BlkGeom& G = P.g[i];
    const BlkFold& F = Q.f[i];
    struct Job { const float* w; size_t wf; int N, K; const c3d_bn_ptrs* bn; size_t ss; int Cp; bool on; };
    const Job jobs[4] = {{k.w_a, F.w_a, G.Ci, G.Cin, &k.bn_a, F.ss_a, G.Cip, true},
                         {k.w_b, F.w_b, G.Ci, 27, &k.bn_b, F.ss_b, G.Cip, true},
                         {k.w_c, F.w_c, G.Co, G.Ci, &k.bn_c, F.ss_c, G.Cop, true},
                         {k.w_sc, F.w_sc, G.Co, G.Cin, &k.bn_sc, F.ss_1, G.Cop, G.sc_bn}};
    for (const Job& j : jobs) {
      if (!j.on) continue;
      if (!j.w || !j.bn->gamma || !j.bn->beta || !j.bn->running_mean || !j.bn->running_var) return C3D_E_BADARG;
      fold_bn_kernel<<<dim3(j.Cp), dim3(64), 0, st>>>(j.w, atT<float>(fold, j.wf), j.N, j.K, j.bn->gamma, j.bn->beta,
                                                     j.bn->running_mean, j.bn->running_var, d->eps, atT<float>(fold, j.ss), j.Cp);
    }
    if (G.sc_conv && !G.sc_bn)
      HIPRC(hipMemcpyAsync(at(fold, F.w_sc), k.w_sc, (size_t)G.Co * G.Cin * 4, hipMemcpyDeviceToDevice, st));
  }
  hipError_t e = hipGetLastError();
  return e == hipSuccess ? 0 : (int)e;
}

extern "C" int c3d_stage_fwd_folded(const c3d_stage_desc* d, const void* fold_c, const void* x, void* ws, void* y_out,
                                    void* stream) {
  Plan P;
  RC(make_plan(d, P));
  FoldPlan Q;
  RC(make_fold_plan(d, P, Q));
  if (!fold_c || !x || !ws || !y_out) return C3D_E_BADARG;
  void* fold = const_cast<void*>(fold_c);
  hipStream_t st = reinterpret_cast<hipStream_t>(stream);
  const int dt = d->dtype, B = d->B, T = d->T;
  RC(zero_fill(at(ws, Q.acc_off), Q.acc_bytes, st));
  const void* cur = x;
  for (int i = 0; i < d->n_blocks; ++i) {
    const c3d_block_desc& k = d->blocks[i];
    const BlkGeom& G = P.g[i];
    const BlkFold& F = Q.f[i];
    const BlkEval& E = Q.e[i];
    void* a = at(ws, E.a); void* b = at(ws, E.b); void* c = at(ws, E.c); void* sc = at(ws, E.sc);
    void* y = i + 1 == d->n_blocks ? y_out : at(ws, E.y);
    float* ss_a = atT<float>(fold, F.ss_a); float* ss_b = atT<float>(fold, F.ss_b); float* ss_c = atT<float>(fold, F.ss_c);
    float* ss_1 = atT<float>(fold, F.ss_1);
    float* gate = G.se ? atT<float>(ws, E.gate) : nullptr;
    double* nc_b = atT<double>(ws, E.nc_b);
    const int64_t rps = (int64_t)T * G.Ho * G.Wo;
    {
      PwCall p(cur, atT<float>(fold, F.w_a), a, G.M, G.Cin, G.Ci, G.Cin, 1, dt);
      RC(c3d_pw_gemm(&p.a, st));
    }
    RC(c3d_dw333_fwd(a, ss_a, atT<float>(fold, F.w_b), b, nc_b, B, T, G.H, G.W, G.Ci, G.Cip, G.s, dt, st));
    if (G.se)
      RC(c3d_bn_se_finalize(nc_b, B, (double)rps, k.bn_b.gamma, k.bn_b.beta, k.bn_b.running_mean, k.bn_b.running_var, nullptr,
                            d->momentum, d->eps, G.Ci, G.Cip, 2, k.se_w1, k.se_b1, k.se_w2, k.se_b2, G.Cr, ss_b, nullptr,
                            gate, atT<float>(ws, E.hid), st));
    {
      PwCall p(b, atT<float>(fold, F.w_c), c, G.Mo, G.Ci, G.Co, G.Ci, 1, dt);
      p.a.pro_mode = C3D_PRO_BN_SE_SWISH; p.a.pro_p = ss_b; p.a.pro_gate = gate; p.a.rows_per_sample = rps;
      RC(c3d_pw_gemm(&p.a, st));
    }
    int mode = SC_IDENTITY;
    const void* scp = cur;
    if (G.sc_conv) {
      PwCall p(cur, atT<float>(fold, F.w_sc), sc, G.Mo, G.Cin, G.Co, G.Cin, 1, dt);
      p.a.row_mode = G.s == 2 ? C3D_ROWS_STRIDE2 : C3D_ROWS_DENSE; p.a.H = G.H; p.a.W = G.W;
      RC(c3d_pw_gemm(&p.a, st));
      mode = G.sc_bn ? SC_BN : SC_RAW;
      scp = sc;
    }
    RC(c3d_block_out_fwd(c, ss_c, scp, ss_1, mode, y, G.Mo, G.Cop, dt, st));
    cur = y;
  }
  return 0;
}
```

Measured before the change: 1617.

## Use buffer loads in stride-2 depthwise bwd and extend cooperative dgrad to residual

Adds a buffer-resource variant of the fused stride-2 depthwise backward kernel for TT=3. It uses raw buffer loads and stores with out-of-bounds offsets in place of branches, which cuts per-lane bounds checks and 64-bit address math. It also extends the cooperative dgrad+wgrad pointwise kernel to the downsampling residual mode (res_mode 1) with strided residual indexing, and falls back to a separate wgrad launch if the kernel is unsupported. This moves more blocks onto the fused wgrad path, at the cost of extra per-row index stepping and new template variants.

Result: faster. 1636 (median of 6 runs) (+1.2%).

```diff
diff --git a/change3d_amd/csrc/dw_bwd_fused.hip b/change3d_amd/csrc/dw_bwd_fused.hip
--- a/change3d_amd/csrc/dw_bwd_fused.hip
+++ b/change3d_amd/csrc/dw_bwd_fused.hip
@@ -227,7 +227,14 @@
   }
 }
 
-template <typename T, int TT, int S>
+constexpr uint32_t FB_OOB = 0x80000000u;
+typedef uint32_t fb_u32x2_t __attribute__((ext_vector_type(2)));
+typedef uint32_t fb_u32x4_t __attribute__((ext_vector_type(4)));
+__device__ __forceinline__ __amdgpu_buffer_rsrc_t fb_rsrc(const void* p, uint32_t bytes) {
+  return __builtin_amdgcn_make_buffer_rsrc(const_cast<void*>(p), 0, (int)bytes, 0x00020000);
+}
+
+template <typename T, int TT, int S, bool BUF = false>
 __global__ FB_KATTR void dw_bwd_fused_kernel(
     const T* __restrict__ t1, const T* __restrict__ bb, const float* __restrict__ coefA,
     const float* __restrict__ coefB, const float* __restrict__ coefC, const float* __restrict__ w,
@@ -303,8 +310,30 @@
     yx[sl] = use_ ? (iy_ | (ix_ << 16)) : 0x7fff7fff;
   }
   const int orel = (S * py * g.W + S * px) * g.Cp + cb4, ofr = g.H * g.W * g.Cp;
+  const uint32_t in_bytes = BUF ? (uint32_t)g.T * (uint32_t)ofr * 2u : 0u, out_bytes = BUF ? (uint32_t)(g.T * g.Ho * g.Wo * g.Cp) * 2u : 0u;
+  const __amdgpu_buffer_rsrc_t rA = fb_rsrc(a + (BUF ? (int64_t)b * g.T * ofr : 0), in_bytes);
+  const __amdgpu_buffer_rsrc_t rT2 = fb_rsrc(t2 + (BUF ? (int64_t)b * g.T * ofr : 0), in_bytes);
+  const __amdgpu_buffer_rsrc_t rT1 = fb_rsrc(t1 + (BUF ? (int64_t)b * g.T * g.Ho * g.Wo * g.Cp : 0), out_bytes);
+  const __amdgpu_buffer_rsrc_t rBB = fb_rsrc(bb + (BUF ? (int64_t)b * g.T * g.Ho * g.Wo * g.Cp : 0), out_bytes);
 #define FB_ISSUE_RAW(TL)                                                                          \
-  {                                                                                               \
+  if constexpr (BUF) {                                                                            \
+    const int tx_ = (TL) % tiles_x, ty_ = (TL) / tiles_x;                                         \
+    const int dy0_ = ty_ * FB_TH - 1, dx0_ = tx_ * FB_TW - 1;                                     \
+    const int tbo_ = (dy0_ * g.Wo + dx0_) * g.Cp;                                                 \
+    const bool on_ = (TL) < tl1;                                                                  \
+    vmask = 0;                                                                                    \
+    _Pragma("unroll") for (int sl = 0; sl < SL; ++sl) {                                           \
+      const unsigned gy_ = (unsigned)(dy0_ + (yx[sl] & 0xffff));                                  \
+      const unsigned gx_ = (unsigned)(dx0_ + (yx[sl] >> 16));                                     \
+      const bool v_ = on_ && gy_ < (unsigned)g.Ho && gx_ < (unsigned)g.Wo;                        \
+      const uint32_t o_ = v_ ? (uint32_t)(rel[sl] + tbo_) * 2u : FB_OOB;                          \
+      const fb_u32x4_t q1_ = __builtin_amdgcn_raw_buffer_load_b128(rT1, o_, 0, 0);                \
+      const fb_u32x4_t q2_ = __builtin_amdgcn_raw_buffer_load_b128(rBB, o_, 0, 0);                \
+      r1[sl] = __builtin_bit_cast(typename R8::type, q1_);                                        \
+      r2[sl] = __builtin_bit_cast(typename R8::type, q2_);                                        \
+      vmask |= v_ ? 1u << sl : 0u;                                                                \
+    }                                                                                             \
+  } else {                                                                                        \
     const int tx_ = (TL) % tiles_x, ty_ = (TL) / tiles_x;                                         \
     const int dy0_ = ty_ * FB_TH - 1, dx0_ = tx_ * FB_TW - 1;                                     \
     const int64_t tb_ = ((((int64_t)b * g.T) * g.Ho + dy0_) * g.Wo + dx0_) * g.Cp;   \
@@ -322,7 +351,15 @@
     }                                                                                             \
   }
 #define FB_ISSUE_A(TL, CY, CX)                                                                    \
-  {                                                                                               \
+  if constexpr (BUF) {                                                                            \
+    const int tx_ = (TL) % tiles_x, ty_ = (TL) / tiles_x;                                         \
+    const bool v_ = (TL) < tl1 && c_ok && ty_ * FB_TH * S + S * py + (CY) < g.H && tx_ * FB_TW * S + S * px + (CX) < g.W; \
+    const uint32_t o_ = (uint32_t)(((ty_ * FB_TH * S + (CY)) * g.W + tx_ * FB_TW * S + (CX)) * g.Cp + orel) * 2u; \
+    _Pragma("unroll") for (int t = 0; t < TT; ++t) {                                              \
+      const fb_u32x2_t q_ = __builtin_amdgcn_raw_buffer_load_b64(rA, (v_ && t < g.T) ? o_ + (uint32_t)(t * ofr) * 2u : FB_OOB, 0, 0); \
+      ar[t] = __builtin_bit_cast(typename R4::type, q_);                                          \
+    }                                                                                             \
+  } else {                                                                                        \
     const int tx_ = (TL) % tiles_x, ty_ = (TL) / tiles_x;                                         \
     if (c_ok && ty_ * FB_TH * S + S * py + (CY) < g.H && tx_ * FB_TW * S + S * px + (CX) < g.W) { \
       const T* ab_ = a + ((((int64_t)b * g.T) * g.H + ty_ * FB_TH * S + (CY)) * g.W + tx_ * FB_TW * S + (CX)) * g.Cp; \
@@ -393,7 +430,30 @@
     }                                                                                                             \
   }
 #define FB_EPI(CY, CX)                                                                                            \
-  if (p_ok) {                                                                                                     \
+  if constexpr (BUF) {                                                                                            \
+    float o[TT][4];                                                                                               \
+    _Pragma("unroll") for (int t = 0; t < TT; ++t) { o[t][0] = 0.f; o[t][1] = 0.f; o[t][2] = 0.f; o[t][3] = 0.f; } \
+    if (p_ok) {                                        \
+      float ma[4], ra[4];                                                                                         \
+      lds4(cf + 5 * 32 + cv * 8 + h * 4, ma);                                                                     \
+      lds4(cf + 6 * 32 + cv * 8 + h * 4, ra);                                                                     \
+      _Pragma("unroll") for (int t = 0; t < TT; ++t) {                                                           \
+        if (t < g.T) {                                                                                            \
+          float av[4];                                                                                            \
+          R4::cvt(arc[t], av);                                                                                    \
+          _Pragma("unroll") for (int j = 0; j < 4; ++j) {                                                        \
+            const float d = round_as<T>(ain[t][j >> 1][j & 1] > 0.f ? acc[t][j >> 1][j & 1] : 0.f);               \
+            o[t][j] = d;                                                                                          \
+            S1[j] += d; S2[j] += d * ((av[j] - ma[j]) * ra[j]);                                                   \
+          }                                                                                                       \
+        }                                                                                                         \
+      }                                                                                                           \
+    }                                                                                                             \
+    const uint32_t so_ = (uint32_t)(((y0 + (CY)) * g.W + x0 + (CX)) * g.Cp + orel) * 2u;                          \
+    _Pragma("unroll") for (int t = 0; t < TT; ++t)                                                               \
+      __builtin_amdgcn_raw_buffer_store_b64(fb_u32x2_t{pack_bf16x2(o[t][0], o[t][1]), pack_bf16x2(o[t][2], o[t][3])}, rT2, \
+                                            (p_ok && t < g.T) ? so_ + (uint32_t)(t * ofr) * 2u : FB_OOB, 0, 0);   \
+  } else if (p_ok) {                                                                                              \
     float ma[4], ra[4];                                                                                           \
     lds4(cf + 5 * 32 + cv * 8 + h * 4, ma);                                                                       \
     lds4(cf + 6 * 32 + cv * 8 + h * 4, ra);                                                                       \
@@ -414,7 +474,7 @@
     FB_PRE(0, 0)
     if constexpr (S == 2) {
       FB_ISSUE_A(tl, 1, 0)
-      if (tl + 1 < tl1) FB_ISSUE_RAW(tl + 1)
+      if (BUF || tl + 1 < tl1) FB_ISSUE_RAW(tl + 1)
       FCLK(2)
       __syncthreads();
       FCLK(3)
@@ -439,7 +499,7 @@
       FB_EPI(0, 1)
       FCLK(5)
       FB_PRE(1, 1)
-      if (tl + 1 < tl1) FB_ISSUE_A(tl + 1, 0, 0)
+      if (BUF || tl + 1 < tl1) FB_ISSUE_A(tl + 1, 0, 0)
       FCLK(2)
       fb_taps_s2<TT, 1, 1>(tp, wlp, acc, dwa, ain);
       FCLK(4)
@@ -899,7 +959,7 @@
   return 0;
 }
 
-template <typename T, int TT, int S>
+template <typename T, int TT, int S, bool BUF = false>
 int launch_fused_t(const void* t1, const void* bb, const float* cA, const float* cB, const float* cC, const float* w,
                    const void* a, const float* ss_a, const float* mr_a, void* t2, double* dsums, float* dw,
                    const DwGeom& g, hipStream_t stream, const c3d_bn_fin& fin) {
@@ -909,7 +969,7 @@
   if (lds > 160 * 1024) return C3D_E_UNSUPPORTED;
   static bool attr_set = false;
   if (!attr_set) {
-    hipError_t e = hipFuncSetAttribute(reinterpret_cast<const void*>(&dw_bwd_fused_kernel<T, TT, S>),
+    hipError_t e = hipFuncSetAttribute(reinterpret_cast<const void*>(&dw_bwd_fused_kernel<T, TT, S, BUF>),
                                        hipFuncAttributeMaxDynamicSharedMemorySize, 160 * 1024);
     if (e != hipSuccess) return (int)e;
     attr_set = true;
@@ -924,7 +984,7 @@
   if (env_tpw > 0) tpw = env_tpw;
   if (tpw > ntiles) tpw = ntiles;
   dim3 grid(chunk_order_grid(chunks, (long)((ntiles + tpw - 1) / tpw) * g.B));
-  dw_bwd_fused_kernel<T, TT, S><<<grid, dim3(FB_NTHR), lds, stream>>>(
+  dw_bwd_fused_kernel<T, TT, S, BUF><<<grid, dim3(FB_NTHR), lds, stream>>>(
       reinterpret_cast<const T*>(t1), reinterpret_cast<const T*>(bb), cA, cB, cC, w, reinterpret_cast<const T*>(a),
       ss_a, mr_a, reinterpret_cast<T*>(t2), dsums, dw, g, tpw, fin);
   C3D_CHECK_LAUNCH();
@@ -960,6 +1020,8 @@
       return launch_ring_t<5, false>(t1, b, coefA, coefB, coefC, w, a, ss_a, mr_a, t2, dsums, dw, g, s, fin);
     }
     if (g.stride == 1) { FB_DISPATCH(bf16_t, 1) }
+    if (tt == 3 && !(c3d_option_dw_ring & 16) && (int64_t)g.T * g.H * g.W * g.Cp * 2 < ((int64_t)1 << 31))
+      return launch_fused_t<bf16_t, 3, 2, true>(t1, b, coefA, coefB, coefC, w, a, ss_a, mr_a, t2, dsums, dw, g, s, fin);
     FB_DISPATCH(bf16_t, 2)
   }
 #undef FB_DISPATCH
diff --git a/change3d_amd/csrc/launch_hints.h b/change3d_amd/csrc/launch_hints.h
--- a/change3d_amd/csrc/launch_hints.h
+++ b/change3d_amd/csrc/launch_hints.h
@@ -13,7 +13,7 @@
 extern int c3d_option_pw_cfwd;
 extern int c3d_option_pw_cdg;
 int c3d_detail_pw_cdg_a(const c3d_pw_args* args, void* stream);
-bool c3d_detail_pw_cdg_a_supported(int Kp, int Np, int64_t M);
+bool c3d_detail_pw_cdg_a_supported(int Kp, int Np, int64_t M, int res_mode, int H, int W);
 int c3d_detail_pw_cdg_c(const c3d_pw_args* args, void* stream);
 bool c3d_detail_pw_cdg_c_supported(int Kp, int Np, int64_t M, int64_t rows_per_sample);
 extern thread_local int c3d_cdg_defer_reduce, c3d_cdg_parts;
diff --git a/change3d_amd/csrc/pw_cdgrad.hip b/change3d_amd/csrc/pw_cdgrad.hip
--- a/change3d_amd/csrc/pw_cdgrad.hip
+++ b/change3d_amd/csrc/pw_cdgrad.hip
@@ -33,6 +33,7 @@
   int w_off, a_off, a_bytes, q_off, q_bytes;
   int os_off, os_wave;
   int par_off, dump_off;
+  int res_dw, res_dh, res_dbt;
 };
 
 typedef uint32_t cd_u32x4_t __attribute__((ext_vector_type(4)));
@@ -60,7 +61,7 @@
   f[0] = a.x; f[1] = a.y; f[2] = a.z; f[3] = a.w; f[4] = b.x; f[5] = b.y; f[6] = b.z; f[7] = b.w;
 }
 
-template <int KS, int NTW, int NPW, int NQW, int RP, int RQ, int K2>
+template <int KS, int NTW, int NPW, int NQW, int RP, int RQ, int K2, int RES>
 __global__ __launch_bounds__(CD_THREADS) void pw_cdg_a_kernel(const c3d_pw_args a, const CdPlan L) {
   extern __shared__ __attribute__((aligned(16))) unsigned char smem[];
   const int tid = threadIdx.x, lane = tid & 63;
@@ -81,7 +82,7 @@
   const __amdgpu_buffer_rsrc_t rX = cd_rsrc(a.x, row_hi * (uint32_t)Kp * 2u);
   const __amdgpu_buffer_rsrc_t rX2 = cd_rsrc(a.x2, row_hi * (uint32_t)Kp * 2u);
   const __amdgpu_buffer_rsrc_t rQ = cd_rsrc(a.wg_x3, row_hi * (uint32_t)Np * 2u);
-  const __amdgpu_buffer_rsrc_t rE1 = cd_rsrc(a.e1, (uint32_t)M32 * (uint32_t)Np * 2u);
+  const __amdgpu_buffer_rsrc_t rE1 = cd_rsrc(a.e1, (uint32_t)(RES ? M32 >> 2 : M32) * (uint32_t)Np * 2u);
   const __amdgpu_buffer_rsrc_t rC1 = cd_rsrc(a.add_sums ? a.add_c : nullptr, (uint32_t)M32 * (uint32_t)Np * 2u);
   const __amdgpu_buffer_rsrc_t rY = cd_rsrc(a.y, (uint32_t)M32 * (uint32_t)Np * 2u);
 
@@ -129,8 +130,38 @@
   uint4 e1r[NPASS], c1r[NPASS];
 #define CD_EOFF(TILE, P) ((act_o && (P) * RPO + rr_o < 16 && (TILE) * MT + wr * 16 + (P) * RPO + rr_o < M32)                        \
                               ? ((uint32_t)((TILE) * MT + wr * 16 + (P) * RPO + rr_o) * (uint32_t)Np + (uint32_t)cvec * 8u) * 2u : CD_OOB)
-#pragma unroll
-  for (int p = 0; p < NPASS; ++p) { const uint32_t o = t0 < t1 ? CD_EOFF(t0, p) : CD_OOB; e1r[p] = cd_load(rE1, o); c1r[p] = cd_load(rC1, o); }
+  int rw_[NPASS], rh_[NPASS], rf_[NPASS];
+  uint32_t e1on[NPASS];
+  const int Hh = a.H >> 1, Wh = a.W >> 1;
+#define CD_E1OFF(TILE, P) ((((rw_[P] | rh_[P]) & 1) == 0 && CD_EOFF(TILE, P) != CD_OOB)                                               \
+                               ? ((uint32_t)((rf_[P] * Hh + (rh_[P] >> 1)) * Wh + (rw_[P] >> 1)) * (uint32_t)Np + (uint32_t)cvec * 8u) * 2u : CD_OOB)
+#define CD_E1STEP(P)                                                                                                \
+  {                                                                                                                 \
+    rw_[P] += L.res_dw;                                                                                             \
+    const int cw_ = rw_[P] >= a.W ? 1 : 0;                                                                          \
+    rw_[P] -= cw_ ? a.W : 0;                                                                                        \
+    rh_[P] += L.res_dh + cw_;                                                                                       \
+    const int ch_ = rh_[P] >= a.H ? 1 : 0;                                                                          \
+    rh_[P] -= ch_ ? a.H : 0;                                                                                        \
+    rf_[P] += L.res_dbt + ch_;                                                                                      \
+  }
+#pragma unroll
+  for (int p = 0; p < NPASS; ++p) {
+    const uint32_t o = t0 < t1 ? CD_EOFF(t0, p) : CD_OOB;
+    if (RES) {
+      const uint32_t m0 = (uint32_t)(t0 * MT + wr * 16 + p * RPO + rr_o);
+      const uint32_t q0 = m0 / (uint32_t)a.W;
+      rw_[p] = (int)(m0 - q0 * (uint32_t)a.W);
+      rf_[p] = (int)(q0 / (uint32_t)a.H);
+      rh_[p] = (int)(q0 - (uint32_t)rf_[p] * (uint32_t)a.H);
+      const uint32_t oe = t0 < t1 ? CD_E1OFF(t0, p) : CD_OOB;
+      e1on[p] = oe != CD_OOB ? 0xffffffffu : 0u;
+      e1r[p] = cd_load(rE1, oe);
+    } else {
+      e1r[p] = cd_load(rE1, o);
+    }
+    c1r[p] = cd_load(rC1, o);
+  }
 
   {
     const int wbytes = (KS * 4) * L.img_rows * 16;
@@ -260,7 +291,8 @@
         const uint32_t hx = (xw[j >> 1] >> ((j & 1) * 16)) & 0xffffu;                                               \
               \
         const uint32_t pass = ((hx & 0x7fffu) != 0u && !(hx & 0x8000u)) ? 0xffffffffu : ~mask_on;                   \
-        const float d = __uint_as_float(__float_as_uint(f[j] + rv[j]) & pass);                                      \
+        const uint32_t sum_ = __float_as_uint(f[j] + rv[j]);                                                        \
+        const float d = __uint_as_float((RES ? (sum_ & e1on[p]) | (__float_as_uint(f[j]) & ~e1on[p]) : sum_) & pass); \
         f[j] = d;                                                                                                   \
         const float gq = __uint_as_float(__float_as_uint(round_as<bf16_t>(d)) & keep & sums_on);                    \
         s0[j] += gq; s1[j] = fmaf(gq, (cv[j] - eM[j]) * eR[j], s1[j]);                                              \
@@ -269,7 +301,15 @@
       __builtin_amdgcn_raw_buffer_store_b128(cd_u32x4_t{pk.x, pk.y, pk.z, pk.w}, rY,                                \
                                              ok ? ((uint32_t)m * (uint32_t)Np + (uint32_t)cvec * 8u) * 2u : CD_OOB, 0, 0); \
       const uint32_t no_ = (NEXT_ON) ? CD_EOFF((TILE) + 1, p) : CD_OOB;                                             \
-      e1r[p] = cd_load(rE1, no_); c1r[p] = cd_load(rC1, no_);                                                       \
+      if (RES) {                                                                                                    \
+        CD_E1STEP(p)                                                                                                \
+        const uint32_t ne_ = (NEXT_ON) ? CD_E1OFF((TILE) + 1, p) : CD_OOB;                                          \
+        e1on[p] = ne_ != CD_OOB ? 0xffffffffu : 0u;                                                                 \
+        e1r[p] = cd_load(rE1, ne_);                                                                                 \
+      } else {                                                                                                      \
+        e1r[p] = cd_load(rE1, no_);                                                                                 \
+      }                                                                                                             \
+      c1r[p] = cd_load(rC1, no_);                                                                                   \
     }                                                                                                               \
   }
 
@@ -315,6 +355,8 @@
 #undef CD_MULT
 #undef CD_WGRAD
 #undef CD_EPI
+#undef CD_E1STEP
+#undef CD_E1OFF
 #undef CD_EOFF
 
   {
@@ -353,37 +395,48 @@
   }
 }
 
-template <int KS, int NTW, int NPW, int NQW, int RP, int RQ, int K2>
+template <int KS, int NTW, int NPW, int NQW, int RP, int RQ, int K2, int RES>
 int cd_launch(const c3d_pw_args& a, const CdPlan& L, dim3 grid, size_t lds, hipStream_t s) {
   static bool attr_set = false;
   if (!attr_set) {
-    hipError_t e = hipFuncSetAttribute(reinterpret_cast<const void*>(&pw_cdg_a_kernel<KS, NTW, NPW, NQW, RP, RQ, K2>),
+    hipError_t e = hipFuncSetAttribute(reinterpret_cast<const void*>(&pw_cdg_a_kernel<KS, NTW, NPW, NQW, RP, RQ, K2, RES>),
                                        hipFuncAttributeMaxDynamicSharedMemorySize, 160 * 1024);
     if (e != hipSuccess) return (int)e;
     attr_set = true;
   }
-  pw_cdg_a_kernel<KS, NTW, NPW, NQW, RP, RQ, K2><<<grid, dim3(CD_THREADS), lds, s>>>(a, L);
+  pw_cdg_a_kernel<KS, NTW, NPW, NQW, RP, RQ, K2, RES><<<grid, dim3(CD_THREADS), lds, s>>>(a, L);
   return 0;
 }
 
-int cd_variant(int Kp, int Np) {
+int cd_variant(int Kp, int Np, int res_mode) {
   const int KS = (Kp + 31) / 32, ntn = (Np + 15) >> 4, ntp = (Kp + 15) >> 4;
-  if (KS == 7 && ntn >= 5 && ntn <= 6 && ntp <= 16) return 1;
-  if (KS == 4 && ntn == 3 && ntp <= 8) return 2;
+  if (res_mode == 0) {
+    if (KS == 7 && ntn >= 5 && ntn <= 6 && ntp <= 16) return 1;
+    if (KS == 4 && ntn == 3 && ntp <= 8) return 2;
+  } else if (res_mode == 1) {
+    if (KS == 4 && ntn == 2 && ntp <= 8) return 4;
+    if (KS == 7 && ntn == 3 && ntp <= 16) return 5;
+  } else {
+    return 0;
+  }
   if (KS == 2 && ntn == 2 && ntp <= 4) return 3;
   return 0;
 }
 
 int cd_plan(const c3d_pw_args& a, CdPlan& L, int64_t& blocks, size_t& lds) {
-  const int var = cd_variant(a.Kp, a.Np);
+  const int var = cd_variant(a.Kp, a.Np, a.res_mode);
   if (!var) return 0;
+  if (a.res_mode == 1 && (a.H < 2 || a.W < 2 || (a.H & 1) || (a.W & 1) || a.M % ((int64_t)a.H * a.W))) return 0;
   const int Kpad = (a.Kp + 31) / 32 * 32, KS = Kpad / 32, ntn = (a.Np + 15) >> 4;
   L.img_rows = (ntn <= 2 ? 2 : ntn <= 4 ? 4 : ntn <= 7 ? 7 : 14) * 16;
   int NTW;
   if (var == 1) { L.WR = 2; L.WC = 4; NTW = 2; L.QG = 2; }
   else if (var == 2) { L.WR = 8; L.WC = 1; NTW = 3; L.QG = 1; }
+  else if (var == 5) { L.WR = 4; L.WC = 2; NTW = 2; L.QG = 1; }
   else { L.WR = 8; L.WC = 1; NTW = 2; L.QG = 2; }
   L.MT = 16 * L.WR;
+  L.res_dw = L.res_dh = L.res_dbt = 0;
+  if (a.res_mode == 1) { L.res_dw = L.MT % a.W; L.res_dh = (L.MT / a.W) % a.H; L.res_dbt = (L.MT / a.W) / a.H; }
   L.KL = Kpad + 8;
   L.QL = ntn * 16 + 8;
   const int64_t tiles = (a.M + L.MT - 1) / L.MT;
@@ -768,12 +821,12 @@
 
 }
 
-__attribute__((visibility("hidden"))) bool c3d_detail_pw_cdg_a_supported(int Kp, int Np, int64_t M) {
+__attribute__((visibility("hidden"))) bool c3d_detail_pw_cdg_a_supported(int Kp, int Np, int64_t M, int res_mode, int H, int W) {
   if (Kp <= 0 || Np <= 0 || (Kp & 7) || (Np & 7)) return false;
   if (M < 1024 || (M + 512) * (int64_t)(Kp > Np ? Kp : Np) * 2 >= ((int64_t)1 << 31)) return false;
   c3d_pw_args a;
   std::memset(&a, 0, sizeof(a));
-  a.M = M; a.K = a.Kp = Kp; a.N = a.Np = Np;
+  a.M = M; a.K = a.Kp = Kp; a.N = a.Np = Np; a.res_mode = res_mode; a.H = H; a.W = W;
   CdPlan L;
   int64_t blocks = 0;
   size_t lds = 0;
@@ -783,8 +836,9 @@
 __attribute__((visibility("hidden"))) int c3d_detail_pw_cdg_a(const c3d_pw_args* args, void* stream) {
   const c3d_pw_args& a = *args;
   if (a.dtype != C3D_DT_BF16 || a.row_mode != C3D_ROWS_DENSE || a.pro_mode != C3D_PRO_AFFINE2 || a.epi_mode != C3D_EPI_ADD ||
-      a.wg_mode != C3D_WG_ROWS || a.res_mode != 0)
+      a.wg_mode != C3D_WG_ROWS || (a.res_mode != 0 && a.res_mode != 1))
     return C3D_E_UNSUPPORTED;
+  if (a.res_mode == 1 && ((c3d_option_pw_cdg & 4) || a.add_sums)) return C3D_E_UNSUPPORTED;
   if (!a.w_img || !a.x2 || !a.e1 || !a.wg_x3 || !a.wg_dw || !a.wg_ws || a.pro_out || a.bias || a.fin.ticket) return C3D_E_UNSUPPORTED;
   if (a.fin.sums ? (a.fin.training != 0 || !a.fin.mr || !a.fin.gamma) : !a.pro_p) return C3D_E_UNSUPPORTED;
   if (a.add_sums && (!a.add_c || !a.add_mr || !a.wg_mask_out)) return C3D_E_UNSUPPORTED;
@@ -797,9 +851,12 @@
   hipStream_t s = reinterpret_cast<hipStream_t>(stream);
   const dim3 grid((unsigned)blocks);
   int rc = C3D_E_UNSUPPORTED;
-  if (var == 1) rc = cd_launch<7, 2, 4, 3, 2, 1, 1>(a, L, grid, lds, s);
-  else if (var == 2) rc = cd_launch<4, 3, 1, 3, 4, 2, 4>(a, L, grid, lds, s);
-  else if (var == 3) rc = cd_launch<2, 2, 1, 1, 2, 1, 4>(a, L, grid, lds, s);
+  if (var == 1) rc = cd_launch<7, 2, 4, 3, 2, 1, 1, 0>(a, L, grid, lds, s);
+  else if (var == 2) rc = cd_launch<4, 3, 1, 3, 4, 2, 4, 0>(a, L, grid, lds, s);
+  else if (var == 3 && a.res_mode == 0) rc = cd_launch<2, 2, 1, 1, 2, 1, 4, 0>(a, L, grid, lds, s);
+  else if (var == 3) rc = cd_launch<2, 2, 1, 1, 2, 1, 4, 1>(a, L, grid, lds, s);
+  else if (var == 4) rc = cd_launch<4, 2, 2, 1, 4, 1, 4, 1>(a, L, grid, lds, s);
+  else if (var == 5) rc = cd_launch<7, 2, 2, 3, 4, 1, 2, 1>(a, L, grid, lds, s);
   if (rc != 0) return rc;
   C3D_CHECK_LAUNCH();
   if (c3d_cdg_defer_reduce) { c3d_cdg_parts = (int)blocks; return 0; }
diff --git a/change3d_amd/csrc/stage_driver.hip b/change3d_amd/csrc/stage_driver.hip
--- a/change3d_amd/csrc/stage_driver.hip
+++ b/change3d_amd/csrc/stage_driver.hip
@@ -167,7 +167,7 @@
     const BlkGeom& G = P.g[i];
     if (fuse_wgrad(d, G.Cop, G.Cip, C3D_WG_SWISH)) wsf_fused = std::max(wsf_fused, c3d_pw_gemm_wg_ws_floats(G.Co, G.Ci));
     if (fuse_wgrad(d, G.Cip, G.Cinp, C3D_WG_ROWS)) wsf_fused = std::max(wsf_fused, c3d_pw_gemm_wg_ws_floats(G.Ci, G.Cin));
-    if (d->dtype == C3D_DT_BF16 && c3d_detail_pw_cdg_a_supported(G.Cip, G.Cinp, G.M)) wsf_fused = std::max(wsf_fused, c3d_pw_gemm_wg_ws_floats(G.Ci, G.Cin));
+    if (d->dtype == C3D_DT_BF16 && c3d_detail_pw_cdg_a_supported(G.Cip, G.Cinp, G.M, G.sc_conv && G.s == 2 ? 1 : 0, G.H, G.W)) wsf_fused = std::max(wsf_fused, c3d_pw_gemm_wg_ws_floats(G.Ci, G.Cin));
     if (d->dtype == C3D_DT_BF16 && c3d_detail_pw_cdg_c_supported(G.Cop, G.Cip, G.Mo, (int64_t)d->T * G.Ho * G.Wo))
       wsf_fused = std::max(wsf_fused, c3d_pw_gemm_wg_ws_floats(G.Co, G.Ci));
     mx_g = std::max(mx_g, (size_t)G.Mo * G.Cop * e);
@@ -778,18 +778,21 @@
       res = dxs;
       res_mode = G.s == 2 ? 1 : 0;
     }
-    const bool coop_wa = (c3d_option_pw_cdg & 1) && dt == C3D_DT_BF16 && !(d->flags & C3D_STAGE_SEPARATE_WGRAD) && res_mode == 0 &&
-                         imgp(F.img_at) != nullptr && c3d_detail_pw_cdg_a_supported(G.Cip, G.Cinp, G.M);
+    const bool coop_wa = (c3d_option_pw_cdg & 1) && dt == C3D_DT_BF16 && !(d->flags & C3D_STAGE_SEPARATE_WGRAD) &&
+                         (res_mode == 0 || !(c3d_option_pw_cdg & 4)) && imgp(F.img_at) != nullptr &&
+                         c3d_detail_pw_cdg_a_supported(G.Cip, G.Cinp, G.M, res_mode, G.H, G.W);
     const bool fuse_wa = coop_wa || ((g_fuse_wgrad & 1) && fuse_wgrad(d, G.Cip, G.Cinp, C3D_WG_ROWS));
     bool mask_next = false, sums_next = false;
-    if (!fuse_wa)
-    RC(side_run(st, [&](hipStream_t s2) {
-      WgCall w(t2, xin, k.dw_a, wgws_ab[wg_n++ & 1], G.M, G.Cin, G.Ci, G.Cin, 1, dt);
-      w.a.chain = g_wgrad_chain;
-      w.a.p2 = a; w.a.p_coef = coef_a;
-      if (consb) w.a.p_fin = fin_coef_consume(dsums_a, k.bn_a, (double)G.M, mr_a, false);
-      return wg_launch(w.a, s2);
-    }));
+    auto wgrad_a = [&] {
+      return side_run(st, [&](hipStream_t s2) {
+        WgCall w(t2, xin, k.dw_a, wgws_ab[wg_n++ & 1], G.M, G.Cin, G.Ci, G.Cin, 1, dt);
+        w.a.chain = g_wgrad_chain;
+        w.a.p2 = a; w.a.p_coef = coef_a;
+        if (consb) w.a.p_fin = fin_coef_consume(dsums_a, k.bn_a, (double)G.M, mr_a, false);
+        return wg_launch(w.a, s2);
+      });
+    };
+    if (!fuse_wa) RC(wgrad_a());
     {
       PwCall p(t2, k.w_a, dx, G.M, G.Ci, G.Cin, 1, G.Cin, dt);
       if (fuse_wa) { p.a.wg_mode = C3D_WG_ROWS; p.a.wg_x3 = xin; p.a.wg_dw = k.dw_a; p.a.wg_ws = wgws_fused; }
@@ -807,17 +810,20 @@
       if (consb) p.a.fin = fin_coef_consume(dsums_a, k.bn_a, (double)G.M, mr_a, true);
       p.a.epi_mode = C3D_EPI_ADD; p.a.e1 = res; p.a.res_mode = res_mode; p.a.H = G.H; p.a.W = G.W;
       p.a.w_img = imgp(F.img_at);
-      if (coop_wa && side_enabled()) {
-        float* const wsk = wgws_fused + (size_t)(1 + cdg_n) * (P.wgrad_ws_fused_slot / 4);
-        p.a.wg_ws = wsk;
-        c3d_cdg_defer_reduce = 1; c3d_cdg_parts = 0;
-        const int rcl = pw_launch(p.a, st);
-        c3d_cdg_defer_reduce = 0;
-        RC(rcl);
-        if (c3d_cdg_parts > 0) { ++cdg_n; red_jobs.push_back({wsk, p.a.wg_dw, p.a.K, p.a.N, c3d_cdg_parts, p.a.w_sk, p.a.w_sn}); }
-      } else {
-        RC(pw_launch(p.a, st));
+      const bool defer = coop_wa && side_enabled();
+      float* const wsk = defer ? wgws_fused + (size_t)(1 + cdg_n) * (P.wgrad_ws_fused_slot / 4) : nullptr;
+      if (defer) { p.a.wg_ws = wsk; c3d_cdg_defer_reduce = 1; c3d_cdg_parts = 0; }
+      int rcl = pw_launch(p.a, st);
+      c3d_cdg_defer_reduce = 0;
+      if (rcl == C3D_E_UNSUPPORTED && coop_wa) {
+        mask_next = sums_next = false;
+        p.a.wg_mode = C3D_WG_NONE; p.a.wg_x3 = nullptr; p.a.wg_dw = nullptr; p.a.wg_ws = nullptr; p.a.wg_mask_out = 0;
+        p.a.add_c = nullptr; p.a.add_mr = nullptr; p.a.add_sums = nullptr;
+        RC(wgrad_a());
+        rcl = pw_launch(p.a, st);
       }
+      RC(rcl);
+      if (defer && c3d_cdg_parts > 0) { ++cdg_n; red_jobs.push_back({wsk, p.a.wg_dw, p.a.K, p.a.N, c3d_cdg_parts, p.a.w_sk, p.a.w_sn}); }
     }
     lag.push_back(side_mark());
     if ((int)lag.size() >= bwd_ring()) { RC(side_join(st, lag.front())); lag.pop_front(); }
@@ -849,11 +855,11 @@
     case C3D_OPT_FUSE_WGRAD: g_fuse_wgrad = value & 3; return 0;
     case C3D_OPT_FOLD_SE: g_fold_se = value ? 1 : 0; return 0;
     case C3D_OPT_MASK_IN_DGRAD: g_mask_in_dgrad = value & 3; return 0;
-    case C3D_OPT_DW_RING: c3d_option_dw_ring = value & 15; return 0;
+    case C3D_OPT_DW_RING: c3d_option_dw_ring = value & 31; return 0;
     case C3D_OPT_DW_FWD_HV: c3d_option_dw_fwd_hv = value & 7; return 0;
     case C3D_OPT_DW_T4: c3d_option_dw_t4 = value ? 1 : 0; return 0;
     case C3D_OPT_PW_CFWD: c3d_option_pw_cfwd = value & 3; return 0;
-    case C3D_OPT_PW_CDG: c3d_option_pw_cdg = value & 3; return 0;
+    case C3D_OPT_PW_CDG: c3d_option_pw_cdg = value & 7; return 0;
     case C3D_OPT_PW_WGRAD_V2: c3d_option_pw_wgrad_v2 = value & 1; g_wgrad_chain = (value & 2) ? 0 : 1; return 0;
     default: return C3D_E_BADARG;
   }
```
